# LukasHaas/PIGEON

Measured on AMD Instinct MI355X. Metric: images/sec end-to-end (ViT+head+refine), 4x336x336, higher is better.
Workload: dtype f16

## Files before the change

include/pigeon_hip.h:

```cpp
#ifndef PIGEON_HIP_H
#define PIGEON_HIP_H

#include <stddef.h>
#include <stdint.h>

#ifdef __cplusplus
extern "C" {
#endif

#define PG_OK            0
#define PG_EINVAL       -1
#define PG_ENOMEM       -2
#define PG_EHIP         -3
#define PG_ESTATE       -4

#define PG_DTYPE_F32     0
#define PG_DTYPE_BF16    1
#define PG_DTYPE_F16     2
#define PG_DTYPE_F64     3
#define PG_DTYPE_U8      4

#define PG_ABI_VERSION   7

const char* pg_last_error(void);
int pg_abi_version(void);
int pg_device_count(void);

typedef struct pg_vit pg_vit;

typedef struct pg_vit_cfg {
    int32_t layers;
    int32_t image_size;
    int32_t patch;
    int32_t hidden;
    int32_t heads;
    int32_t mlp;
    float   ln_eps;
    int32_t max_chunk;
    int32_t mma_dtype;
    int32_t precise;
} pg_vit_cfg;

int pg_vit_create(pg_vit** out, int device, const pg_vit_cfg* cfg);
int pg_vit_load_weight(pg_vit* h, const char* name, const void* data, int dtype,
                       const int64_t* shape, int ndim);
int pg_vit_finalize(pg_vit* h);
int pg_vit_workspace_bytes(const pg_vit* h, int n_images, size_t* bytes);
int pg_vit_forward(pg_vit* h, const void* pixels, int pix_dtype, int n_images, float* emb_out,
                   void* workspace, size_t workspace_bytes, void* stream);
int pg_vit_forward_hidden(pg_vit* h, const void* pixels, int pix_dtype, int n_images, float* emb_out,
                          float* hidden_out, void* workspace, size_t workspace_bytes, void* stream);
int pg_vit_precise_workspace_bytes(const pg_vit* h, int n_images, size_t* bytes);
int pg_vit_precise_plan(int n_images, int32_t out[8]);
int pg_vit_forward_precise(pg_vit* h, const void* pixels, int pix_dtype, int n_images, float* emb_out, float* hidden_out,
                           void* workspace, size_t workspace_bytes, void* stream);
int pg_vit_graph(pg_vit* h, int on, int64_t* replays, int64_t* captures);
int pg_vit_destroy(pg_vit* h);
int pg_vit_mma_dtype(const pg_vit* h);

int pg_fingerprint(const void* data, size_t bytes, uint64_t seed, uint64_t out[2], void* stream);
int pg_vit_fingerprint(const pg_vit* h, uint64_t out[2]);

#define PG_PROF_CLASSES 9
int pg_vit_profile_enable(pg_vit* h, int on);
int pg_vit_profile_read(pg_vit* h, int64_t* launches , double* ms );
int pg_vit_profile_reset(pg_vit* h);

int pg_tune_gemm_stagger(float fraction);
int pg_tune_gemm_tail_rows(int rows);
int pg_tune_gemm_tail_shape(int min_k, int min_n);
int pg_tune_gemm_raster(int gn);
int pg_tune_gemm_mid(int on);
int pg_gemm_plan(int variant, int epi, int M, int N, int K, int* kernel, int* rows_main, int* rest);
int pg_tune_exact_attention(int use_f32_mfma);
int pg_tune_exact_products(int n);
int pg_tune_exact_fusion(int on);
int pg_vit_saturation_check(pg_vit* h, int on);
int pg_vit_saturation_read(pg_vit* h, int64_t* count, int reset);
int pg_vit_range_alarm_read(pg_vit* h, int64_t* rows, int reset);

int pg_head_forward(const float* emb, int B, int P, const float* W, const float* bias,
                    const double* centroids, int C, int k, float* logits,
                    float* topk_val, int64_t* topk_idx, int64_t* argmax, double* pred_llh, void* stream);

int pg_head_margin(const float* logits, int B, int C, const float* emb, int P, const float* W, float* margin, float* sens,
                   int64_t* top2, void* stream);

int pg_head_certainty(const float* logits, int B, int C, const float* emb, int P, const float* W, const int64_t* topk_idx, int kx,
                      const float* beta, const float* wstats, float* tol, int32_t* code, float* margin, float* sens, void* stream);

int pg_aux_heads_forward(const float* emb, int B, int P, const float* W, const float* bias, int n_reg, int n_climate, int n_month,
                         const float* beta, float* preds, int64_t* cls, float* tol, int32_t* code, float* row_tol, void* stream);

typedef struct pg_bank {
    const float*   proto_emb;
    const int64_t* cell_off;
    const float*   proto_lnglat;
    const int32_t* proto_count;
    const int64_t* member_off;
    const int64_t* member_idx;
    const float*   train_emb;
    const float*   train_lnglat;
    int64_t num_cells;
    int64_t num_protos;
    int64_t num_train;
} pg_bank;

int pg_refine_forward(const pg_bank* bank, const float* q, int B, int P, const double* init_llh,
                      const int64_t* cand, const float* cand_prob, int k, int topk,
                      float temperature, double max_refine_km, float* scratch,
                      float* out_llh, int64_t* out_cell, int32_t* out_choice, void* stream);

int pg_refine_forward_ex(const pg_bank* bank, const float* q, int B, int P, const double* init_llh,
                         const int64_t* cand, const float* cand_prob, int k, int topk, int n_eval,
                         float temperature, double max_refine_km, float* scratch12,
                         float* out_llh, int64_t* out_cell, int32_t* out_choice, int32_t* out_refined, void* stream);

int pg_refine_certainty(const pg_bank* bank, const float* q, int B, int P, const int64_t* cand, const float* cand_prob, int k,
                        int topk, int n_eval, const float* scratch12, const float* W, int C, const float* beta,
                        const float* wstats, float temperature, const int32_t* refined, const int32_t* choice,
                        float* tol, int32_t* code, void* stream);

int pg_requeue_append(const float* head_tol, const float* refine_tol, const int32_t* refine_code, int B, float thr, int force_all,
                      int64_t dst_base, int64_t flushed, int64_t cap, int64_t* counters, int64_t* slot_dst, int32_t* row_slot,
                      uint8_t* certain, int32_t* cause, void* stream);
int pg_rows_to_slots(const void* src, int64_t row_bytes, const int32_t* row_slot, int B, void* dst, void* stream);
int pg_requeue_take(const int64_t* slot_dst, int64_t cap, int64_t head, int n_valid, int n_pad, int64_t* dst_out, void* stream);
int pg_scatter_rows(const void* src, int64_t row_bytes, const int64_t* dst_row, int n, void* dst, int64_t dst_rows,
                    int64_t remap_wb, int64_t remap_b, int64_t remap_off, void* stream);
// ... 37 lines not shown
int pg_allgather_many(void* comm, int count, const void* const* send, void* const* recv, const size_t* bytes_per_rank,
                      void* stream);
int pg_comm_destroy(void* comm);
int pg_comm_rccl_version(void);

int pg_proto_build(const float* train_emb, int panels, int64_t num_train, const int64_t* member_off,
                   const int64_t* member_idx, int64_t num_protos, float* proto_emb, void* stream);
int pg_haversine_matrix(const void* x, int x_dtype, const double* y, int N, int M, double* out, void* stream);
int pg_haversine_pairs(const double* x, const void* y, int y_dtype, int64_t N, double* out, void* stream);
int pg_smooth_labels(const double* distances, int N, int M, double constant, double* out, void* stream);

int pg_haversine_blocks(const double* pts, const int64_t* cell_off, const int64_t* mat_off, int C, double zero_as, double* out,
                        void* stream);
int pg_optics_graph(const double* dist, const int64_t* cell_off, const int64_t* mat_off, int C, int min_samples, int64_t* ordering,
                    double* core, double* reach, int64_t* pred, void* stream);
int pg_optics_plan(int64_t n, int min_samples, int32_t out[4]);
int pg_tune_optics_lds_points(int max_points);

typedef struct pg_region_bank {
    const int64_t* region_off;
    const int64_t* ring_off;
    const double*  xy;
    const double*  ring_bbox;
    const double*  region_bbox;
    const int64_t* region_off_host;
    const int64_t* ring_off_host;
    int64_t num_regions;
    int64_t num_rings;
    int64_t num_vertices;
} pg_region_bank;
#define PG_REGION_OUTSIDE   0
#define PG_REGION_INSIDE    1
#define PG_REGION_AMBIGUOUS 2
int pg_region_locate(const pg_region_bank* bank, const double* pts, const int32_t* start, int64_t N, int32_t* cover, uint8_t* state,
                     void* stream);
int pg_region_classify(const pg_region_bank* bank, const double* pts, const int32_t* region, int64_t N, uint8_t* state, void* stream);
int pg_region_nearest(const pg_region_bank* bank, const double* pts, int64_t N, int32_t* idx, double* dist, void* stream);
int pg_region_plan(const pg_region_bank* bank, int32_t out[4]);
int pg_tune_region_wave_edges(int max_edges);

int pg_op_gemm16(int dtype, const void* A, int64_t lda, const void* W, const float* bias, void* out, int64_t ldc,
                 int M, int N, int K, int epi, float qscale, int qcols, const float* aux,
                 int variant, void* stream);
int pg_op_gemm16_ld(int dtype, const void* A, int64_t lda, const void* W, int64_t ldw, const float* bias, void* out,
                    int64_t ldc, int M, int N, int K, int epi, float qscale, int qcols, const float* aux,
                    int variant, void* stream);
int pg_op_rowstat_cast(const float* x, void* x16, int dtype, float* rowstat, int64_t rows, float eps, void* stream);
int pg_op_gemm16_resid_stat(int dtype, const void* A, int64_t lda, const void* W, int64_t ldw, const float* bias, float* X,
                            int64_t ldc, void* x16, int64_t ldx, float* statpart, int M, int N, int K, int variant, void* stream);
int pg_op_rowstat_finalize(const float* statpart, int slots, float* rowstat, int64_t rows, float eps, void* stream);
int pg_op_gemm16_ln(int dtype, const void* A, int64_t lda, const void* W, int64_t ldw, const float* bias, const float* colsum,
                    const float* rowstat, void* out, int64_t ldc, int M, int N, int K, int epi, float qscale, int qcols,
                    int variant, void* stream);
int pg_op_layernorm(const float* x, const float* gamma, const float* beta, void* y, int out_dtype,
                    int64_t rows, float eps, void* stream);
int pg_op_attention(int dtype, const void* qkv, void* out, int n_images, void* stream);
int pg_op_im2col(const void* pixels, int pix_dtype, void* out, int out_dtype, int n_images, void* stream);
int pg_op_token_mean(const float* x, float* out, int n_images, void* stream);
int pg_op_cast_f32(const float* x, void* y, int out_dtype, int64_t n, void* stream);
int pg_op_preln(float* x, const float* cls, const float* pos0, const float* gamma, const float* beta, int64_t rows, float eps,
                void* x16, int x16_dtype, float* rowstat, void* stream);
int pg_op_gemm16_parts(int dtype, const void* A, int64_t lda, const void* W, int64_t ldw, const float* bias, float* parts,
                       int M, int N, int Kp, int S, void* stream);
int pg_op_x3_split(const float* x, void* y3, int64_t rows, int cols, int gelu, void* stream);
int pg_op_x3_layernorm(const float* x, const float* gamma, const float* beta, void* y3, int64_t rows, float eps, void* stream);
int pg_op_attention_f32(const float* qkv, float* out, int n_images, void* stream);
int pg_op_attention_x3(const float* qkv, void* out3, int n_images, void* stream);
int pg_op_x3_im2col(const void* pixels, int pix_dtype, void* out3, int n_images, void* stream);
int pg_op_sum_parts(const float* parts, int S, int64_t part_elems, float* dst, int64_t n, int resid, void* stream);

#ifdef __cplusplus
}
#endif
#endif
```

pigeon_amd/_lib.py:

```python
from __future__ import annotations

import ctypes as C
import os

_HERE = os.path.dirname(os.path.abspath(__file__))
LIB_PATH = os.environ.get("PIGEON_HIP_LIB") or os.path.join(_HERE, "libpigeon_hip.so")

PG_DTYPE_F32, PG_DTYPE_BF16, PG_DTYPE_F16, PG_DTYPE_F64, PG_DTYPE_U8 = 0, 1, 2, 3, 4
EPI_QKV, EPI_GELU, EPI_RESID, EPI_PATCH, EPI_F32, EPI_RESID_STAT, EPI_QKV_LN, EPI_GELU_LN, EPI_GELU_X3 = 0, 1, 2, 3, 4, 5, 6, 7, 8
PROF_CLASSES = ["gemm_qkv", "gemm_out", "gemm_fc1", "gemm_fc2", "gemm_patch", "attention", "layernorm",
                "im2col", "token_mean"]


class PigeonHipError(RuntimeError):
    pass


class VitCfg(C.Structure):
    _fields_ = [("layers", C.c_int32), ("image_size", C.c_int32), ("patch", C.c_int32), ("hidden", C.c_int32),
                ("heads", C.c_int32), ("mlp", C.c_int32), ("ln_eps", C.c_float), ("max_chunk", C.c_int32),
                ("mma_dtype", C.c_int32), ("precise", C.c_int32)]


class Bank(C.Structure):
    _fields_ = [("proto_emb", C.c_void_p), ("cell_off", C.c_void_p), ("proto_lnglat", C.c_void_p),
                ("proto_count", C.c_void_p), ("member_off", C.c_void_p), ("member_idx", C.c_void_p),
                ("train_emb", C.c_void_p), ("train_lnglat", C.c_void_p),
                ("num_cells", C.c_int64), ("num_protos", C.c_int64), ("num_train", C.c_int64)]


class RegionBankStruct(C.Structure):
    _fields_ = [("region_off", C.c_void_p), ("ring_off", C.c_void_p), ("xy", C.c_void_p), ("ring_bbox", C.c_void_p),
                ("region_bbox", C.c_void_p), ("region_off_host", C.c_void_p), ("ring_off_host", C.c_void_p),
                ("num_regions", C.c_int64), ("num_rings", C.c_int64), ("num_vertices", C.c_int64)]


class PrepItem(C.Structure):
    _fields_ = [("src_off", C.c_uint64), ("in_h", C.c_int32), ("in_w", C.c_int32), ("new_h", C.c_int32), ("new_w", C.c_int32),
                ("top", C.c_int32), ("left", C.c_int32), ("ksize_h", C.c_int32), ("ksize_v", C.c_int32), ("row0", C.c_int32),
                ("nrows", C.c_int32), ("tmp_row", C.c_int32), ("bounds_h_off", C.c_uint32), ("kk_h_off", C.c_uint32),
                ("bounds_v_off", C.c_uint32), ("kk_v_off", C.c_uint32), ("reserved", C.c_int32 * 3)]


PREP_ITEM_BYTES = 80
assert C.sizeof(PrepItem) == PREP_ITEM_BYTES


_P, _I, _I64, _F, _D, _SZ = C.c_void_p, C.c_int, C.c_int64, C.c_float, C.c_double, C.c_size_t
SIGNATURES = {
    "pg_last_error": (C.c_char_p, []),
    "pg_abi_version": (_I, []),
    "pg_device_count": (_I, []),
    "pg_vit_create": (_I, [C.POINTER(_P), _I, C.POINTER(VitCfg)]),
    "pg_vit_load_weight": (_I, [_P, C.c_char_p, _P, _I, C.POINTER(_I64), _I]),
    "pg_vit_finalize": (_I, [_P]),
    "pg_vit_workspace_bytes": (_I, [_P, _I, C.POINTER(_SZ)]),
    "pg_vit_forward": (_I, [_P, _P, _I, _I, _P, _P, _SZ, _P]),
    "pg_vit_forward_hidden": (_I, [_P, _P, _I, _I, _P, _P, _P, _SZ, _P]),
    "pg_vit_precise_workspace_bytes": (_I, [_P, _I, C.POINTER(_SZ)]),
    "pg_vit_forward_precise": (_I, [_P, _P, _I, _I, _P, _P, _P, _SZ, _P]),
    "pg_vit_graph": (_I, [_P, _I, C.POINTER(_I64), C.POINTER(_I64)]),
    "pg_vit_destroy": (_I, [_P]),
    "pg_vit_mma_dtype": (_I, [_P]),
    "pg_fingerprint": (_I, [_P, _SZ, C.c_uint64, C.POINTER(C.c_uint64), _P]),
    "pg_vit_fingerprint": (_I, [_P, C.POINTER(C.c_uint64)]),
    "pg_vit_profile_enable": (_I, [_P, _I]),
    "pg_vit_profile_read": (_I, [_P, C.POINTER(_I64), C.POINTER(_D)]),
    "pg_vit_profile_reset": (_I, [_P]),
    "pg_tune_gemm_stagger": (_I, [_F]),
    "pg_tune_gemm_tail_rows": (_I, [_I]),
    "pg_tune_gemm_tail_shape": (_I, [_I, _I]),
    "pg_tune_gemm_raster": (_I, [_I]),
    "pg_tune_gemm_mid": (_I, [_I]),
    "pg_tune_exact_attention": (_I, [_I]),
    "pg_tune_exact_products": (_I, [_I]),
    "pg_tune_exact_fusion": (_I, [_I]),
    "pg_gemm_plan": (_I, [_I, _I, _I, _I, _I, _P, _P, _P]),
    "pg_vit_saturation_check": (_I, [_P, _I]),
    "pg_vit_saturation_read": (_I, [_P, C.POINTER(_I64), _I]),
    "pg_vit_range_alarm_read": (_I, [_P, C.POINTER(_I64), _I]),
    "pg_comm_unique_id": (_I, [_P]),
    "pg_comm_init_rank": (_I, [C.POINTER(_P), _I, _P, _I]),
    "pg_comm_count": (_I, [_P, C.POINTER(_I)]),
    "pg_allgather": (_I, [_P, _P, _P, _SZ, _P]),
    "pg_allgather_many": (_I, [_P, _I, C.POINTER(_P), C.POINTER(_P), C.POINTER(_SZ), _P]),
    "pg_comm_destroy": (_I, [_P]),
    "pg_comm_rccl_version": (_I, []),
    "pg_prep_create": (_I, [C.POINTER(_P), _I, _I, _I]),
    "pg_prep_destroy": (_I, [_P]),
    "pg_prep_geometry": (_I, [_P, C.POINTER(C.c_int32)]),
    "pg_prep_workspace_bytes": (_I, [_P, _I, C.POINTER(_SZ)]),
    "pg_prep_norm_lut": (_I, [C.POINTER(_F)]),
    "pg_prep_forward": (_I, [_P, _P, _I, _P, _I, _P, _SZ, _P]),
    "pg_prep_ragged_plan": (_I, [_I, C.POINTER(C.c_int32), C.POINTER(PrepItem), C.POINTER(_SZ), C.POINTER(_SZ)]),
    "pg_prep_ragged_create": (_I, [C.POINTER(_P), _I]),
    "pg_prep_ragged_destroy": (_I, [_P]),
    "pg_prep_ragged_forward": (_I, [_P, _P, _SZ, C.POINTER(PrepItem), _I, _P, _I, _P, _SZ, _P]),
    "pg_proto_build": (_I, [_P, _I, _I64, _P, _P, _I64, _P, _P]),
    "pg_haversine_matrix": (_I, [_P, _I, _P, _I, _I, _P, _P]),
    "pg_haversine_pairs": (_I, [_P, _P, _I, _I64, _P, _P]),
    "pg_smooth_labels": (_I, [_P, _I, _I, _D, _P, _P]),
    "pg_haversine_blocks": (_I, [_P, _P, _P, _I, _D, _P, _P]),
    "pg_optics_graph": (_I, [_P, _P, _P, _I, _I, _P, _P, _P, _P, _P]),
    "pg_optics_plan": (_I, [_I64, _I, C.POINTER(C.c_int32)]),
    "pg_tune_optics_lds_points": (_I, [_I]),
    "pg_region_locate": (_I, [C.POINTER(RegionBankStruct), _P, _P, _I64, _P, _P, _P]),
    "pg_region_classify": (_I, [C.POINTER(RegionBankStruct), _P, _P, _I64, _P, _P]),
    "pg_region_nearest": (_I, [C.POINTER(RegionBankStruct), _P, _I64, _P, _P, _P]),
    "pg_region_plan": (_I, [C.POINTER(RegionBankStruct), C.POINTER(C.c_int32)]),
    "pg_tune_region_wave_edges": (_I, [_I]),
    "pg_head_forward": (_I, [_P, _I, _I, _P, _P, _P, _I, _I, _P, _P, _P, _P, _P, _P]),
    "pg_head_margin": (_I, [_P, _I, _I, _P, _I, _P, _P, _P, _P, _P]),
    "pg_head_certainty": (_I, [_P, _I, _I, _P, _I, _P, _P, _I, _P, _P, _P, _P, _P, _P, _P]),
    "pg_aux_heads_forward": (_I, [_P, _I, _I, _P, _P, _I, _I, _I, _P, _P, _P, _P, _P, _P, _P]),
    "pg_refine_forward": (_I, [C.POINTER(Bank), _P, _I, _I, _P, _P, _P, _I, _I, _F, _D, _P, _P, _P, _P, _P]),
    "pg_refine_forward_ex": (_I, [C.POINTER(Bank), _P, _I, _I, _P, _P, _P, _I, _I, _I, _F, _D, _P, _P, _P, _P, _P, _P]),
    "pg_refine_certainty": (_I, [C.POINTER(Bank), _P, _I, _I, _P, _P, _I, _I, _I, _P, _P, _I, _P, _P, _F, _P, _P, _P, _P, _P]),
    "pg_requeue_append": (_I, [_P, _P, _P, _I, _F, _I, _I64, _I64, _I64, _P, _P, _P, _P, _P, _P]),
    "pg_rows_to_slots": (_I, [_P, _I64, _P, _I, _P, _P]),
    "pg_requeue_take": (_I, [_P, _I64, _I64, _I, _I, _P, _P]),
    "pg_scatter_rows": (_I, [_P, _I64, _P, _I, _P, _I64, _I64, _I64, _I64, _P]),
    "pg_head_wstats": (_I, [_P, _I, _P, _P, _P]),
    "pg_embedding_debias": (_I, [_P, _I64, _I, _P, _P]),
    "pg_op_gemm16": (_I, [_I, _P, _I64, _P, _P, _P, _I64, _I, _I, _I, _I, _F, _I, _P, _I, _P]),
    "pg_op_gemm16_ld": (_I, [_I, _P, _I64, _P, _I64, _P, _P, _I64, _I, _I, _I, _I, _F, _I, _P, _I, _P]),
    "pg_op_rowstat_cast": (_I, [_P, _P, _I, _P, _I64, _F, _P]),
    "pg_op_gemm16_resid_stat": (_I, [_I, _P, _I64, _P, _I64, _P, _P, _I64, _P, _I64, _P, _I, _I, _I, _I, _P]),
    "pg_op_rowstat_finalize": (_I, [_P, _I, _P, _I64, _F, _P]),
    "pg_op_gemm16_ln": (_I, [_I, _P, _I64, _P, _I64, _P, _P, _P, _P, _I64, _I, _I, _I, _I, _F, _I, _I, _P]),
    "pg_op_layernorm": (_I, [_P, _P, _P, _P, _I, _I64, _F, _P]),
    "pg_op_attention": (_I, [_I, _P, _P, _I, _P]),
    "pg_op_im2col": (_I, [_P, _I, _P, _I, _I, _P]),
    "pg_op_token_mean": (_I, [_P, _P, _I, _P]),
    "pg_op_cast_f32": (_I, [_P, _P, _I, _I64, _P]),
    "pg_op_gemm16_parts": (_I, [_I, _P, _I64, _P, _I64, _P, _P, _I, _I, _I, _I, _P]),
    "pg_op_x3_split": (_I, [_P, _P, _I64, _I, _I, _P]),
    "pg_op_x3_layernorm": (_I, [_P, _P, _P, _P, _I64, _F, _P]),
    "pg_op_attention_f32": (_I, [_P, _P, _I, _P]),
    "pg_op_attention_x3": (_I, [_P, _P, _I, _P]),
    "pg_op_x3_im2col": (_I, [_P, _I, _P, _I, _P]),
    "pg_op_sum_parts": (_I, [_P, _I, _I64, _P, _I64, _I, _P]),
    "pg_op_preln": (_I, [_P, _P, _P, _P, _P, _I64, _F, _P, _I, _P, _P]),
    "pg_vit_precise_plan": (_I, [_I, C.POINTER(C.c_int32)]),
}

_lib = None


def load():
    global _lib
    if _lib is not None:
        return _lib
    if not os.path.exists(LIB_PATH):
        raise PigeonHipError(
            f"{LIB_PATH} not found: build it with `python -m pigeon_amd.build` (hipcc, gfx950). "
            "pigeon_amd has no CPU/PyTorch fallback for its hot path.")
    import torch
    lib = C.CDLL(LIB_PATH)
    for name, (res, args) in SIGNATURES.items():
        fn = getattr(lib, name)
        fn.restype = res
        fn.argtypes = args
    _lib = lib
    return lib


def check(rc: int, what: str = ""):
    if rc != 0:
        msg = load().pg_last_error()
        raise PigeonHipError(f"{what} failed (code {rc}): {msg.decode() if msg else ''}")


def require_gpu():
    lib = load()
    n = lib.pg_device_count()
    if n <= 0:
        raise PigeonHipError("pigeon_amd needs an AMD GPU (gfx950) visible to HIP; found none. "
                             "There is no CPU fallback for the hot path.")
    return n
```

pigeon_amd/csrc/abi.hip:

```cpp
#include "pigeon_internal.h"
#include <cstdarg>
#include <cstdio>

static thread_local char g_err[512] = "";

void pg_set_error(const char* fmt, ...) {
    va_list ap;
    va_start(ap, fmt);
    vsnprintf(g_err, sizeof(g_err), fmt, ap);
    va_end(ap);
}
int pg_check_launch(const char* what) {
    hipError_t e = hipGetLastError();
    if (e != hipSuccess) { pg_set_error("launch of %s failed: %s", what, hipGetErrorString(e)); return PG_EHIP; }
    return PG_OK;
}

extern "C" const char* pg_last_error(void) { return g_err; }
extern "C" int pg_abi_version(void) { return PG_ABI_VERSION; }
extern "C" int pg_device_count(void) {
    int n = 0;
    hipError_t e = hipGetDeviceCount(&n);
    if (e != hipSuccess) { pg_set_error("hipGetDeviceCount: %s", hipGetErrorString(e)); return PG_EHIP; }
    return n;
}

extern "C" int pg_op_gemm16(int dtype, const void* A, int64_t lda, const void* W, const float* bias, void* out, int64_t ldc,
                            int M, int N, int K, int epi, float qscale, int qcols, const float* aux, int variant,
                            void* stream) {
    if (!A || !W || !out) { pg_set_error("op_gemm16: null argument"); return PG_EINVAL; }
    return pg_gemm_launch(dtype, A, lda, W, K, bias, out, ldc, M, N, K, epi, qscale, qcols, aux, variant, (hipStream_t)stream);
}
extern "C" int pg_op_gemm16_ld(int dtype, const void* A, int64_t lda, const void* W, int64_t ldw, const float* bias, void* out,
                               int64_t ldc, int M, int N, int K, int epi, float qscale, int qcols, const float* aux,
                               int variant, void* stream) {
    if (!A || !W || !out) { pg_set_error("op_gemm16_ld: null argument"); return PG_EINVAL; }
    return pg_gemm_launch(dtype, A, lda, W, ldw, bias, out, ldc, M, N, K, epi, qscale, qcols, aux, variant, (hipStream_t)stream);
}
extern "C" int pg_op_rowstat_cast(const float* x, void* x16, int dtype, float* rowstat, int64_t rows, float eps, void* stream) {
    if (!x || !x16 || !rowstat) { pg_set_error("op_rowstat_cast: null argument"); return PG_EINVAL; }
    return pg_rowstat_cast_launch(x, x16, dtype, rowstat, rows, eps, (hipStream_t)stream);
}
extern "C" int pg_op_rowstat_finalize(const float* statpart, int slots, float* rowstat, int64_t rows, float eps, void* stream) {
    if (!statpart || !rowstat || slots <= 0) { pg_set_error("op_rowstat_finalize: bad argument"); return PG_EINVAL; }
    return pg_rowstat_finalize_launch(statpart, slots, rowstat, rows, eps, (hipStream_t)stream);
}
extern "C" int pg_op_gemm16_resid_stat(int dtype, const void* A, int64_t lda, const void* W, int64_t ldw, const float* bias, float* X,
                                       int64_t ldc, void* x16, int64_t ldx, float* statpart, int M, int N, int K, int variant,
                                       void* stream) {
    if (!A || !W || !X || !x16 || !statpart) { pg_set_error("op_gemm16_resid_stat: null argument"); return PG_EINVAL; }
    PgGemmExtra ex; ex.x16 = x16; ex.ldx = ldx; ex.statpart = statpart;
    return pg_gemm_launch(dtype, A, lda, W, ldw, bias, X, ldc, M, N, K, EPI_RESID_STAT, 1.f, 0, nullptr, variant ? variant : PG_GEMM_V_PP,
                          (hipStream_t)stream, &ex);
}
extern "C" int pg_op_gemm16_ln(int dtype, const void* A, int64_t lda, const void* W, int64_t ldw, const float* bias,
                               const float* colsum, const float* rowstat, void* out, int64_t ldc, int M, int N, int K, int epi,
                               float qscale, int qcols, int variant, void* stream) {
    if (!A || !W || !out || !colsum || !rowstat) { pg_set_error("op_gemm16_ln: null argument"); return PG_EINVAL; }
    if (epi != EPI_QKV_LN && epi != EPI_GELU_LN) { pg_set_error("op_gemm16_ln: epi must be 6 or 7"); return PG_EINVAL; }
    PgGemmExtra ex; ex.colsum = colsum; ex.rowstat = rowstat;
    return pg_gemm_launch(dtype, A, lda, W, ldw, bias, out, ldc, M, N, K, epi, qscale, qcols, nullptr, variant ? variant : PG_GEMM_V_PP,
                          (hipStream_t)stream, &ex);
}
extern "C" int pg_op_layernorm(const float* x, const float* gamma, const float* beta, void* y, int out_dtype,
                               int64_t rows, float eps, void* stream) {
    if (!x || !gamma || !beta || !y) { pg_set_error("op_layernorm: null argument"); return PG_EINVAL; }
    return pg_layernorm_launch(x, gamma, beta, y, out_dtype, rows, eps, (hipStream_t)stream);
}
extern "C" int pg_op_attention(int dtype, const void* qkv, void* out, int n_images, void* stream) {
    if (!qkv || !out) { pg_set_error("op_attention: null argument"); return PG_EINVAL; }
    return pg_attention_launch(dtype, qkv, out, n_images, (hipStream_t)stream);
}
extern "C" int pg_op_im2col(const void* pixels, int pix_dtype, void* out, int out_dtype, int n_images, void* stream) {
    if (!pixels || !out) { pg_set_error("op_im2col: null argument"); return PG_EINVAL; }
    if (out_dtype == PG_DTYPE_U8) { pg_set_error("op_im2col: PG_DTYPE_U8 is a pixel dtype, not an output dtype"); return PG_EINVAL; }
    const float* lut = nullptr;
    if (pix_dtype == PG_DTYPE_U8 && n_images > 0) { const int rc = pg_norm_lut_device(&lut); if (rc) return rc; }
    return pg_im2col_launch(pixels, pix_dtype, out, out_dtype, n_images, (hipStream_t)stream, lut);
}
extern "C" int pg_op_token_mean(const float* x, float* out, int n_images, void* stream) {
    if (!x || !out) { pg_set_error("op_token_mean: null argument"); return PG_EINVAL; }
    return pg_token_mean_launch(x, out, n_images, (hipStream_t)stream);
}
extern "C" int pg_op_cast_f32(const float* x, void* y, int out_dtype, int64_t n, void* stream) {
    if (!x || !y) { pg_set_error("op_cast_f32: null argument"); return PG_EINVAL; }
    return pg_cast_f32_launch(x, y, out_dtype, n, (hipStream_t)stream);
}

extern "C" int pg_op_gemm16_parts(int dtype, const void* A, int64_t lda, const void* W, int64_t ldw, const float* bias, float* parts,
                                  int M, int N, int Kp, int S, void* stream) {
    if (!A || !W || !parts) { pg_set_error("op_gemm16_parts: null argument"); return PG_EINVAL; }
    if (S < 1 || S > 8) { pg_set_error("op_gemm16_parts: 1 <= S <= 8"); return PG_EINVAL; }
    PgGemmExtra ex;
    ex.parts = S; ex.a_part = Kp; ex.w_part = Kp; ex.c_part = (int64_t)M * N;
    return pg_gemm_launch(dtype, A, lda, W, ldw, bias, parts, N, M, N, Kp, EPI_F32, 1.f, 0, nullptr, PG_GEMM_V_PP, (hipStream_t)stream, &ex);
}

extern "C" int pg_op_x3_split(const float* x, void* y3, int64_t rows, int cols, int gelu, void* stream) {
    if (!x || !y3) { pg_set_error("op_x3_split: null argument"); return PG_EINVAL; }
    return pg_x3_split_launch(x, y3, rows, cols, gelu, (hipStream_t)stream);
}
extern "C" int pg_op_x3_layernorm(const float* x, const float* gamma, const float* beta, void* y3, int64_t rows, float eps, void* stream) {
    if (!x || !gamma || !beta || !y3) { pg_set_error("op_x3_layernorm: null argument"); return PG_EINVAL; }
    return pg_x3_ln_launch(x, gamma, beta, y3, rows, eps, (hipStream_t)stream);
}
extern "C" int pg_op_attention_f32(const float* qkv, float* out, int n_images, void* stream) {
    if (!qkv || !out) { pg_set_error("op_attention_f32: null argument"); return PG_EINVAL; }
    return pg_attention_f32_launch(qkv, out, n_images, (hipStream_t)stream);
}
extern "C" int pg_op_x3_im2col(const void* pixels, int pix_dtype, void* out3, int n_images, void* stream) {
    if (!pixels || !out3 || n_images < 0) { pg_set_error("op_x3_im2col: bad argument"); return PG_EINVAL; }
    const float* lut = nullptr;
    if (pix_dtype == PG_DTYPE_U8 && n_images > 0) { const int rc = pg_norm_lut_device(&lut); if (rc) return rc; }
// ... 18 lines not shown
```

pigeon_amd/csrc/gemm_epi.h:

```cpp
#pragma once
#include "gemm_device.h"

__device__ __forceinline__ float quick_gelu(float v) {
    const float e = __builtin_amdgcn_exp2f(-2.4554669595930157f * v);
    return v * __builtin_amdgcn_rcpf(1.0f + e);
}

typedef float f32x2 __attribute__((ext_vector_type(2)));
__device__ __forceinline__ f32x2 pk_fma(f32x2 a, f32x2 b, f32x2 c) { return __builtin_elementwise_fma(a, b, c); }
__device__ __forceinline__ f32x2 quick_gelu2(f32x2 v) {
    const f32x2 t = v * -2.4554669595930157f;
    f32x2 e = {__builtin_amdgcn_exp2f(t[0]), __builtin_amdgcn_exp2f(t[1])};
    e = 1.0f + e;
    const f32x2 r = {__builtin_amdgcn_rcpf(e[0]), __builtin_amdgcn_rcpf(e[1])};
    return v * r;
}
__device__ __forceinline__ f32x4 ln_fold4(f32x4 acc, float rstd, float mrs, const f32x4& colsum, const f32x4& c) {
    const f32x2 r2 = {rstd, rstd}, m2 = {-mrs, -mrs};
    const f32x2 a0 = pk_fma(f32x2{acc[0], acc[1]}, r2, pk_fma(m2, f32x2{colsum[0], colsum[1]}, f32x2{c[0], c[1]}));
    const f32x2 a1 = pk_fma(f32x2{acc[2], acc[3]}, r2, pk_fma(m2, f32x2{colsum[2], colsum[3]}, f32x2{c[2], c[3]}));
    return f32x4{a0[0], a0[1], a1[0], a1[1]};
}
__device__ __forceinline__ f32x4 quick_gelu4(f32x4 v) {
    const f32x2 a0 = quick_gelu2(f32x2{v[0], v[1]}), a1 = quick_gelu2(f32x2{v[2], v[3]});
    return f32x4{a0[0], a0[1], a1[0], a1[1]};
}


template <typename T, int EPI>
__device__ __forceinline__ u32x4 epi16_finish(f32x4 lo, f32x4 hi, const f32x4& b_lo, const f32x4& b_hi, const f32x4& s_lo,
                                              const f32x4& s_hi, float rstd, float mrs, bool q_strip, float qsc) {
    if constexpr (epi_is_ln(EPI)) {
        lo = ln_fold4(lo, rstd, mrs, s_lo, b_lo);
        hi = ln_fold4(hi, rstd, mrs, s_hi, b_hi);
    } else {
        lo += b_lo; hi += b_hi;
    }
    if constexpr (epi_is_qkv(EPI)) {
        if (q_strip) { lo *= qsc; hi *= qsc; }
    } else {
        lo = quick_gelu4(lo); hi = quick_gelu4(hi);
    }
    u32x4 pk;
    pk[0] = pack16x2<T>(lo[0], lo[1]); pk[1] = pack16x2<T>(lo[2], lo[3]);
    pk[2] = pack16x2<T>(hi[0], hi[1]); pk[3] = pack16x2<T>(hi[2], hi[3]);
    return pk;
}

__device__ __forceinline__ f32x4 epi_resid4(f32x4 x, const f32x4& acc, const f32x4& b) {
    x += acc + b;
    return x;
}
template <typename T>
__device__ __forceinline__ u32x2 epi_copy16x4(const f32x4& x) {
    u32x2 h;
    h[0] = pack16x2<T>(x[0], x[1]); h[1] = pack16x2<T>(x[2], x[3]);
    return h;
}
__device__ __forceinline__ void epi_stat8(const f32x4& x, const f32x4& y, float& s1, float& s2) {
    s1 = ((x[0] + x[1]) + (x[2] + x[3])) + ((y[0] + y[1]) + (y[2] + y[3]));
    s2 = ((x[0] * x[0] + x[1] * x[1]) + (x[2] * x[2] + x[3] * x[3])) + ((y[0] * y[0] + y[1] * y[1]) + (y[2] * y[2] + y[3] * y[3]));
}
template <int CTRL>
__device__ __forceinline__ float epi_dpp_mov(float v) {
    return __builtin_bit_cast(float, __builtin_amdgcn_update_dpp(0, __builtin_bit_cast(int, v), CTRL, 0xF, 0xF, true));
}
__device__ __forceinline__ float row8_sum(float v) {
    v += epi_dpp_mov<0xB1>(v);
    v += epi_dpp_mov<0x4E>(v);
    v += epi_dpp_mov<0x141>(v);
    return v;
}

template <int EPI>
__device__ __forceinline__ void epi_store_f32x4(const GemmArgs& g, int row, int col, f32x4 v, const f32x4& b4) {
    if (EPI == EPI_RESID) {
        float* p = (float*)g.out + (int64_t)row * g.ldc + col;
        f32x4 x = *(const f32x4*)p;
        x += v + b4;
        *(f32x4*)p = x;
    } else if (EPI == EPI_PATCH) {
        const int img = row / VIT_PATCHES, p = row - img * VIT_PATCHES;
        float* o = (float*)g.out + ((int64_t)img * VIT_TOKENS + 1 + p) * g.ldc + col;
        const f32x4 pos = *(const f32x4*)(g.aux + (int64_t)(1 + p) * g.N + col);
        *(f32x4*)o = v + pos;
    } else {
        *(f32x4*)((float*)g.out + (int64_t)row * g.ldc + col) = v + b4;
    }
}

template <typename T, int EPI>
__device__ __forceinline__ void epi_store_bf16x8(const GemmArgs& g, int row, int col, f32x4 lo, f32x4 hi,
                                                 const f32x4& b_lo, const f32x4& b_hi) {
    lo += b_lo; hi += b_hi;
    if (EPI == EPI_QKV) {
        if (col < g.qcols) { lo *= g.qscale; hi *= g.qscale; }
    } else {
#pragma unroll
        for (int e = 0; e < 4; ++e) { lo[e] = quick_gelu(lo[e]); hi[e] = quick_gelu(hi[e]); }
    }
    u32x4 pk;
    pk[0] = pack16x2<T>(lo[0], lo[1]); pk[1] = pack16x2<T>(lo[2], lo[3]);
    pk[2] = pack16x2<T>(hi[0], hi[1]); pk[3] = pack16x2<T>(hi[2], hi[3]);
    *(u32x4*)((uint16_t*)g.out + (int64_t)row * g.ldc + col) = pk;
}

constexpr int EPI_SLAB_ROWPF = 64 + 4;
template <typename T, int EPI>
__device__ __forceinline__ void epi_slab32(const GemmArgs& g, float* slab, int lane, int row0, int col0, const f32x4 (&acc0)[4],
                                           const f32x4 (&acc1)[4]) {
    constexpr bool OUT16 = epi_is_out16(EPI);
    constexpr bool LN = epi_is_ln(EPI);
    constexpr bool STAT = (EPI == EPI_RESID_STAT);
    constexpr bool RESID = epi_is_resid(EPI);
    constexpr int ROWPF = EPI_SLAB_ROWPF;
    const int l15 = lane & 15, lq = lane >> 4;
#pragma unroll
    for (int ib = 0; ib < 2; ++ib)
#pragma unroll
        for (int j = 0; j < 4; ++j) *(f32x4*)(slab + (ib * 16 + l15) * ROWPF + j * 16 + 4 * lq) = (ib ? acc1 : acc0)[j];
    wave_lds_fence();

    constexpr int HOFF = STAT ? 32 : 4;
    const int rr = lane >> 3, cc = STAT ? (lane & 7) * 4 : (lane & 7) * 8;
    const int col = col0 + cc;
    const f32x4 zero4 = {0.f, 0.f, 0.f, 0.f};
    f32x4 b_lo = zero4, b_hi = zero4, s_lo = zero4, s_hi = zero4;
    if (g.bias) { b_lo = *(const f32x4*)(g.bias + col); b_hi = *(const f32x4*)(g.bias + col + HOFF); }
    if constexpr (LN) { s_lo = *(const f32x4*)(g.ex.colsum + col); s_hi = *(const f32x4*)(g.ex.colsum + col + 4); }
    const float qsc = (epi_is_qkv(EPI) && col < g.qcols) ? g.qscale : 1.f;

#pragma unroll
    for (int it = 0; it < 4; ++it) {
        const int r = it * 8 + rr;
        const int row = row0 + r;
        if (row >= g.M) continue;
        f32x4 lo = *(const f32x4*)(slab + r * ROWPF + cc);
        f32x4 hi = *(const f32x4*)(slab + r * ROWPF + cc + HOFF);
        if constexpr (OUT16) {
            float rstd = 0.f, mrs = 0.f;
            if constexpr (LN) {
                const u32x2 rs = *(const u32x2*)(g.ex.rowstat + (int64_t)row * 2);
                asm("v_mov_b32 %0, %1" : "=v"(rstd) : "v"(rs[0]));
                asm("v_mov_b32 %0, %1" : "=v"(mrs) : "v"(rs[1]));
            }
            *(u32x4*)((uint16_t*)g.out + (int64_t)row * g.ldc + col) =
                epi16_finish<T, EPI>(lo, hi, b_lo, b_hi, s_lo, s_hi, rstd, mrs, col0 < g.qcols, qsc);
        } else if constexpr (RESID) {
            float* p = (float*)g.out + (int64_t)row * g.ldc + col;
            const f32x4 x = epi_resid4(*(const f32x4*)p, lo, b_lo);
            const f32x4 y = epi_resid4(*(const f32x4*)(p + HOFF), hi, b_hi);
            *(f32x4*)p = x;
            *(f32x4*)(p + HOFF) = y;
            if constexpr (STAT) {
                uint16_t* p16 = (uint16_t*)g.ex.x16 + (int64_t)row * g.ldc + col;
                *(u32x2*)p16 = epi_copy16x4<T>(x);
                *(u32x2*)(p16 + HOFF) = epi_copy16x4<T>(y);
                float s1, s2;
                epi_stat8(x, y, s1, s2);
                s1 = row8_sum(s1);
                s2 = row8_sum(s2);
                if ((lane & 7) == 0) {
                    float* sp = g.ex.statpart + ((int64_t)(col0 / 64) * g.ex.stat_rows + row) * 2;
                    sp[0] = s1; sp[1] = s2;
                }
            }
        } else {
            float* p = (float*)g.out + (int64_t)row * g.ldc + col;
            *(f32x4*)p = lo + b_lo;
            *(f32x4*)(p + 4) = hi + b_hi;
        }
    }
}
```

pigeon_amd/csrc/gemm_mid.hip:

```cpp
#include "gemm_epi.h"

namespace {

constexpr int MD_BM = 128, MD_BN = 128;
#ifndef PG_MID_STAGES
#define PG_MID_STAGES 3
#endif
constexpr int MD_STAGES = PG_MID_STAGES;
#ifndef PG_MID_PRODUCER
#define PG_MID_PRODUCER 1
#endif
constexpr bool MD_PROD = PG_MID_PRODUCER != 0;
constexpr int MD_THREADS = MD_PROD ? 320 : 256;
constexpr int MD_STAGE = (MD_BM + MD_BN) * ROWB;
constexpr int MD_W_OFF = MD_BM * ROWB;
constexpr int MD_NDMA = (MD_BM + MD_BN) / 8 / 4;
constexpr int MD_LDS = MD_STAGES * MD_STAGE;
constexpr int MD_SLAB_BYTES = 32 * EPI_SLAB_ROWPF * 4;

__device__ __forceinline__ void md_issue(__amdgpu_buffer_rsrc_t ra, __amdgpu_buffer_rsrc_t rw, char* stage, int wave,
                                         const int (&voffA)[4], const int (&voffW)[4], int soff) {
#pragma unroll
    for (int d = 0; d < 4; ++d) dma16(ra, stage + (wave + 4 * d) * 8 * ROWB, voffA[d], soff);
#pragma unroll
// ... 17 lines not shown
    int voffA[4], voffW[4];
#pragma unroll
    for (int d = 0; d < 4; ++d) {
        const int r = (wave + 4 * d) * 8 + (lane >> 3);
        const int c = (lane & 7) ^ ((r >> 1) & 7);
        voffA[d] = r * (int)g.lda * 2 + c * 16;
        voffW[d] = r * (int)g.ldw * 2 + c * 16;
    }
    const int nt = g.K / BK;
    if constexpr (MD_PROD) {
        static_assert(!MD_PROD || MD_STAGES == 3, "the producer form is written for the three-stage ring");
        if (wave == 4) {
            int pvA[2], pvW[2];
#pragma unroll
            for (int d = 0; d < 2; ++d) {
                const int r = d * 8 + (lane >> 3);
                const int c = (lane & 7) ^ ((r >> 1) & 7);
                pvA[d] = r * (int)g.lda * 2 + c * 16;
                pvW[d] = r * (int)g.ldw * 2 + c * 16;
            }
            const int stepA = 16 * (int)g.lda * 2, stepW = 16 * (int)g.ldw * 2;
            auto issue = [&](int t, char* stage) {
#pragma unroll
                for (int gr = 0; gr < 16; ++gr) dma16(ra, stage + gr * 8 * ROWB, pvA[gr & 1] + (gr >> 1) * stepA, t * BK * 2);
#pragma unroll
                for (int gr = 0; gr < 16; ++gr) dma16(rw, stage + MD_W_OFF + gr * 8 * ROWB, pvW[gr & 1] + (gr >> 1) * stepW, t * BK * 2);
            };
            issue(0, smem);
            if (nt > 1) issue(1, smem + MD_STAGE);
            int freed = 2 * MD_STAGE;
            for (int t = 0; t < nt; ++t) {
                if (t + 1 < nt) asm volatile("s_waitcnt vmcnt(32)" ::: "memory");
                else asm volatile("s_waitcnt vmcnt(0)" ::: "memory");
                __builtin_amdgcn_sched_barrier(0);
                __builtin_amdgcn_s_barrier();
                __builtin_amdgcn_sched_barrier(0);
                if (t + 2 < nt) issue(t + 2, smem + freed);
                freed += MD_STAGE;
                if (freed >= MD_LDS) freed = 0;
            }
            __builtin_amdgcn_s_barrier();
            return;
        }
    } else {
#pragma unroll
        for (int t = 0; t < MD_STAGES - 1; ++t)
            if (t < nt) md_issue(ra, rw, smem + t * MD_STAGE, wave, voffA, voffW, t * BK * 2);
    }

    const int l15 = lane & 15, lq = lane >> 4;
    const int sw = (lane >> 1) & 7;
    const uint32_t lds0 = (uint32_t)(uintptr_t)(__attribute__((address_space(3))) char*)smem;
    const uint32_t a_base = lds0 + (wm * 64 + l15) * ROWB, b_base = lds0 + MD_W_OFF + (wn * 64 + l15) * ROWB;
    f32x4 acc[4][4];
#pragma unroll
    for (int i = 0; i < 4; ++i)
#pragma unroll
        for (int j = 0; j < 4; ++j) acc[i][j] = f32x4{0.f, 0.f, 0.f, 0.f};

    int cur = 0;
    for (int kt = 0; kt < nt; ++kt) {
        static_assert(MD_STAGES >= 3 && MD_STAGES <= 5, "the vmcnt ladder below covers 3 .. 5 stages");
        if constexpr (!MD_PROD) {
            const int ahead = min(MD_STAGES - 2, nt - 1 - kt);
            if (MD_STAGES >= 5 && ahead == 3) asm volatile("s_waitcnt vmcnt(%0)" ::"n"(3 * MD_NDMA) : "memory");
            else if (MD_STAGES >= 4 && ahead == 2) asm volatile("s_waitcnt vmcnt(%0)" ::"n"(2 * MD_NDMA) : "memory");
            else if (ahead == 1) asm volatile("s_waitcnt vmcnt(%0)" ::"n"(MD_NDMA) : "memory");
            else asm volatile("s_waitcnt vmcnt(0)" ::: "memory");
        }
        __builtin_amdgcn_sched_barrier(0);
        __builtin_amdgcn_s_barrier();
        __builtin_amdgcn_sched_barrier(0);
        if (!MD_PROD && kt + MD_STAGES - 1 < nt) {
            int nxt = cur - MD_STAGE;
            if (nxt < 0) nxt += MD_LDS;
            md_issue(ra, rw, smem + nxt, wave, voffA, voffW, (kt + MD_STAGES - 1) * BK * 2);
        }
#pragma unroll
        for (int ks = 0; ks < 2; ++ks) {
            const uint32_t xo = (uint32_t)(((ks * 4 + lq) ^ sw) << 4) + (uint32_t)cur;
            const uint32_t aa = a_base + xo, ab = b_base + xo;
            typename T::v8 a[4], b[4];
            lds_read_b128<0 * 16 * ROWB>(a[0], aa); lds_read_b128<1 * 16 * ROWB>(a[1], aa);
            lds_read_b128<2 * 16 * ROWB>(a[2], aa); lds_read_b128<3 * 16 * ROWB>(a[3], aa);
            lds_read_b128<0 * 16 * ROWB>(b[0], ab); lds_read_b128<1 * 16 * ROWB>(b[1], ab);
            lds_read_b128<2 * 16 * ROWB>(b[2], ab); lds_read_b128<3 * 16 * ROWB>(b[3], ab);
            wait_lgkm0();
#pragma unroll
            for (int i = 0; i < 4; ++i)
#pragma unroll
                for (int j = 0; j < 4; ++j) acc[i][j] = T::mfma16(b[j], a[i], acc[i][j]);
        }
        cur += MD_STAGE;
        if (cur >= MD_LDS) cur = 0;
    }
    if constexpr (MD_PROD) {
        asm volatile("s_waitcnt lgkmcnt(0)" ::: "memory");
        __builtin_amdgcn_s_barrier();
    } else {
        __syncthreads();
    }
    float* slab = (float*)(smem + wave * MD_SLAB_BYTES);
    const int row0 = m0 + wm * 64, col0 = n0 + wn * 64;
    epi_slab32<T, EPI>(g, slab, lane, row0, col0, acc[0], acc[1]);
    wave_lds_fence();
    epi_slab32<T, EPI>(g, slab, lane, row0 + 32, col0, acc[2], acc[3]);
    wave_lds_fence();
}

template <typename T, int EPI>
int launch_mid(const GemmArgs& g, int nblk, hipStream_t s) {
    static bool attr_set = false;
    return launch_kernel(gemm_mid_kernel<T, EPI>, attr_set, MD_LDS, dim3(nblk), dim3(MD_THREADS), g, s, "gemm_mid", "gemm_mid: set LDS attr");
}

template <typename T>
int dispatch_mid(const GemmArgs& g, int epi, int nblk, hipStream_t s) {
    switch (epi) {
        case EPI_QKV: return launch_mid<T, EPI_QKV>(g, nblk, s);
        case EPI_GELU: return launch_mid<T, EPI_GELU>(g, nblk, s);
        case EPI_RESID: return launch_mid<T, EPI_RESID>(g, nblk, s);
        case EPI_F32: return launch_mid<T, EPI_F32>(g, nblk, s);
        case EPI_RESID_STAT: return launch_mid<T, EPI_RESID_STAT>(g, nblk, s);
        case EPI_QKV_LN: return launch_mid<T, EPI_QKV_LN>(g, nblk, s);
        case EPI_GELU_LN: return launch_mid<T, EPI_GELU_LN>(g, nblk, s);
        default: pg_set_error("gemm_mid: epilogue %d not supported", epi); return PG_EINVAL;
    }
}

}

bool pg_gemm_mid_supported(int epi, int N, int K) {
    return epi != EPI_PATCH && epi >= EPI_QKV && epi <= EPI_GELU_LN && N % MD_BN == 0 && K % BK == 0 && K >= BK;
}

int pg_gemm_mid_launch(int dtype, GemmArgs g, int epi, hipStream_t s, int m_begin) {
    if (!pg_gemm_mid_supported(epi, g.N, g.K)) { pg_set_error("gemm_mid: unsupported epilogue / shape (epi=%d N=%d K=%d)", epi, g.N, g.K); return PG_EINVAL; }
    if (g.ex.parts > 1) { pg_set_error("gemm_mid: several products in one launch exist in gemm_pp.hip only"); return PG_EINVAL; }
    if (m_begin < 0 || m_begin >= g.M) return m_begin == g.M ? PG_OK : (pg_set_error("gemm_mid: m_begin = %d outside [0, %d)", m_begin, g.M), PG_EINVAL);
    if (m_begin > 0) {
        if (g.ex.stat_rows <= 0) g.ex.stat_rows = g.M;
        g.A += (int64_t)m_begin * g.lda;
        g.out = (char*)g.out + (int64_t)m_begin * g.ldc * (epi_is_out16(epi) ? 2 : 4);
        if (g.ex.rowstat) g.ex.rowstat += (int64_t)m_begin * 2;
        if (g.ex.x16) g.ex.x16 = (uint16_t*)g.ex.x16 + (int64_t)m_begin * g.ldc;
        if (g.ex.statpart) g.ex.statpart += (int64_t)m_begin * 2;
        g.M -= m_begin;
    }
    if (int rc = pg_gemm_panel_check("gemm_mid", g.lda, g.ldw, MD_BM, MD_BN)) return rc;
    g.tilesM = (g.M + MD_BM - 1) / MD_BM;
    g.tilesN = g.N / MD_BN;
    g.ntiles = g.tilesM * g.tilesN;
    g.gn = g.M >= g.N ? 1 : 0;
    if (dtype == PG_DTYPE_F16) return dispatch_mid<T_F16>(g, epi, g.ntiles, s);
    if (dtype == PG_DTYPE_BF16) return dispatch_mid<T_BF16>(g, epi, g.ntiles, s);
    pg_set_error("gemm_mid: operand dtype must be PG_DTYPE_F16 or PG_DTYPE_BF16 (got %d)", dtype);
    return PG_EINVAL;
}
```

pigeon_amd/csrc/gemm_plan.hip:

```cpp
#include "common.h"
#include "pigeon_internal.h"

#include "gemm_epi.h"

#include <cmath>
#include <cstdlib>
#include <type_traits>

#ifndef PG_DEFAULT_GEMM_STAGGER
#define PG_DEFAULT_GEMM_STAGGER 0.0f
#endif
#define PG_DEFAULT_GEMM_TAIL_ROWS 768
#define PG_DEFAULT_GEMM_TAIL_MIN_K 2048
#define PG_DEFAULT_GEMM_TAIL_MIN_N 4096
#ifndef PG_DEFAULT_GEMM_RESID6
#define PG_DEFAULT_GEMM_RESID6 1
#endif
#define PG_ROUTE_MAX_ROWS 40000
#ifndef PG_EXACT_MID_US_KT
#define PG_EXACT_MID_US_KT 0.6
#endif

static unsigned long long g_tune_epoch = 1;
unsigned long long pg_tune_epoch() { return g_tune_epoch; }
// ... 21 lines not shown
    return v;
}
static int route_max_rows() {
    static int v = -1;
    if (v < 0) { v = env_knob("PIGEON_GEMM_ROUTE_MAX_ROWS", PG_ROUTE_MAX_ROWS); if (v < 0) v = 0; }
    return v;
}
static bool resid6_enabled(int K) {
    static int mask = -1;
    if (mask < 0) { mask = env_knob("PIGEON_GEMM_RESID6", PG_DEFAULT_GEMM_RESID6); if (mask < 0) mask = 0; }
    return (mask & (K >= 2048 ? 1 : 2)) != 0;
}
static double precise_mid_us_kt() {
    static double v = -1.0;
    if (v < 0.0) { v = env_knob("PIGEON_EXACT_MID_US", PG_EXACT_MID_US_KT); if (!(v > 0.0)) v = PG_EXACT_MID_US_KT; }
    return v;
}

static int g_raster_gn = -2;
int pg_gemm_raster_gn() {
    if (g_raster_gn == -2) { g_raster_gn = env_knob("PIGEON_GEMM_RASTER_GN", 0); if (g_raster_gn < -1) g_raster_gn = 0; }
    return g_raster_gn;
}
extern "C" int pg_tune_gemm_raster(int gn) {
    if (gn < -1 || gn > 64) { pg_set_error("tune_gemm_raster: gn must be -1 (all N tiles), 0 (default) or 1..64"); return PG_EINVAL; }
    g_raster_gn = gn; ++g_tune_epoch;
    return PG_OK;
}

static int g_tail_rows = -1, g_tail_min_k = -1, g_tail_min_n = -1;
static int env_count(const char* name, int dflt) { const int v = env_knob(name, dflt); return v < 0 ? 0 : v; }
static int tail_rows() { if (g_tail_rows < 0) g_tail_rows = env_count("PIGEON_GEMM_TAIL_ROWS", PG_DEFAULT_GEMM_TAIL_ROWS); return g_tail_rows; }
static int tail_min_k() { if (g_tail_min_k < 0) g_tail_min_k = env_count("PIGEON_GEMM_TAIL_MIN_K", PG_DEFAULT_GEMM_TAIL_MIN_K); return g_tail_min_k; }
static int tail_min_n() { if (g_tail_min_n < 0) g_tail_min_n = env_count("PIGEON_GEMM_TAIL_MIN_N", PG_DEFAULT_GEMM_TAIL_MIN_N); return g_tail_min_n; }
extern "C" int pg_tune_gemm_tail_rows(int rows) {
    if (rows < 0 || rows > (1 << 20)) { pg_set_error("tune_gemm_tail_rows: rows must be in [0, 2^20]"); return PG_EINVAL; }
    g_tail_rows = rows; ++g_tune_epoch;
    return PG_OK;
}
extern "C" int pg_tune_gemm_tail_shape(int min_k, int min_n) {
    if (min_k < 0 || min_n < 0) { pg_set_error("tune_gemm_tail_shape: negative threshold"); return PG_EINVAL; }
    g_tail_min_k = min_k; g_tail_min_n = min_n; ++g_tune_epoch;
    return PG_OK;
}

static int g_gemm_mid = -1;
static bool mid_on() {
    if (g_gemm_mid < 0) { const char* e = env_knob<const char*>("PIGEON_GEMM_MID", "1"); g_gemm_mid = e[0] == '0' ? 0 : (e[0] == '2' ? 2 : 1); }
    return g_gemm_mid != 0;
}
static bool route_pp256() { return mid_on() && g_gemm_mid != 2; }
extern "C" int pg_tune_gemm_mid(int on) {
    g_gemm_mid = on == 2 ? 2 : (on ? 1 : 0); ++g_tune_epoch;
    return PG_OK;
}

static float g_stagger = -1.f;
static float stagger_fraction() {
    if (g_stagger < 0.f) {
        g_stagger = env_knob("PIGEON_GEMM_STAGGER", PG_DEFAULT_GEMM_STAGGER);
        if (!(g_stagger >= 0.f && g_stagger <= 4.f)) g_stagger = 0.f;
    }
    return g_stagger;
}
extern "C" int pg_tune_gemm_stagger(float fraction) {
    if (!(fraction >= 0.f && fraction <= 4.f)) { pg_set_error("tune_gemm_stagger: fraction must be in [0, 4]"); return PG_EINVAL; }
    g_stagger = fraction; ++g_tune_epoch;
    return PG_OK;
}

static int num_cus() {
    static int n = 0;
    if (n == 0) {
        int dev = 0;
        hipDeviceProp_t p;
        if (hipGetDevice(&dev) == hipSuccess && hipGetDeviceProperties(&p, dev) == hipSuccess) n = p.multiProcessorCount;
        if (n <= 0) n = 256;
    }
    return n;
}
int pg_gemm_grid_cus() {
    const int ncu = num_cus(), cap = block_cap();
    return cap > 0 && cap < ncu ? cap : ncu;
}


struct PersistentFit { double ci, cf, e1_resid, e1_gelu, e1_other, e2; };
constexpr PersistentFit SMALL_PP6 = {1.6, 3.0, 7.0, 9.0, 6.0, 3.0};
constexpr PersistentFit SMALL_PP = {1.1, 1.8, 12.0, 9.0, 7.0, 6.0};
constexpr double SMALL_MID_US_KT = 0.44;
constexpr double SMALL_MID_EPI_RESID = 8.0, SMALL_MID_EPI = 5.5;
constexpr double SMALL_PP_MARGIN = 0.90;

static double gemm_model_us(int kernel, int M, int N, int K, int epi, int ncu) {
    const bool resid = epi == EPI_RESID || epi == EPI_RESID_STAT;
    const bool gelu = epi == EPI_GELU || epi == EPI_GELU_LN;
    const double kt = K / 64;
    if (kernel == PG_GK_MID) {
        const int64_t tiles = (int64_t)((M + 127) / 128) * (N / 128);
        return (double)((tiles + ncu - 1) / ncu) * (kt * SMALL_MID_US_KT + (resid ? SMALL_MID_EPI_RESID : SMALL_MID_EPI));
    }
    const PersistentFit& c = kernel == PG_GK_PP6 ? SMALL_PP6 : SMALL_PP;
    const int bm = kernel == PG_GK_PP6 ? 384 : 256;
    const double e1 = resid ? c.e1_resid : (gelu ? c.e1_gelu : c.e1_other);
    const int64_t tiles = (int64_t)((M + bm - 1) / bm) * (N / 256);
    const int64_t full = tiles / ncu;
// ... 93 lines not shown
    if (!by_mid && !by_tail) return false;
    p.rows = (int)m_main;
    p.rest = by_mid ? PG_GK_MID : PG_GK_TAIL;
    return true;
}

static int stagger_ticks(bool six, int epi, int M, int K) {
    const float f = stagger_fraction();
    if (!(f > 0.f && M >= 256 * 64)) return 0;
    const float period_us = six ? ((epi == EPI_GELU || epi == EPI_GELU_LN ? STAGGER_PP6_EPI_GELU : STAGGER_PP6_EPI) + STAGGER_PP6_US_KT * (K / 64))
                                : ((epi == EPI_RESID || epi == EPI_RESID_STAT ? STAGGER_PP_EPI_RESID : STAGGER_PP_EPI) + STAGGER_PP_US_KT * (K / 64));
    return (int)(f * period_us * TICKS_PER_US);
}

static int gemm_plan(int variant, int epi, int M, int N, int K, GemmPlan& p) {
    if (epi < EPI_QKV || epi > EPI_GELU_X3) { pg_set_error("gemm: bad epilogue %d", epi); return PG_EINVAL; }
    if (variant == 0) variant = pg_default_gemm_variant();
    const bool six = use_pp6(variant, epi, N, K);
    const bool pp = !six && (variant == PG_GEMM_V_PP6 || is_pp_variant(variant)) && N % 256 == 0 && K % 128 == 0;
    const int own = six ? PG_GK_PP6 : PG_GK_PP;
    const int pp_variant = variant == PG_GEMM_V_PP6 ? PG_GEMM_V_PP : variant;
    p = GemmPlan{own, pp_variant, M, PG_GK_NONE, stagger_ticks(six, epi, M, K)};
    if (variant == PG_GEMM_V_MID || variant == PG_GEMM_V_TAIL) {
        const bool mid = variant == PG_GEMM_V_MID;
        if (!(mid ? pg_gemm_mid_supported(epi, N, K) : pg_gemm_tail_supported(epi, N, K))) {
            pg_set_error("gemm: variant %d (%s) does not support epi=%d N=%d K=%d", variant, mid ? "gemm_mid" : "gemm_tail", epi, N, K);
            return PG_EINVAL;
        }
        p.kernel = mid ? PG_GK_MID : PG_GK_TAIL;
        return PG_OK;
    }
    if (six || pp) {
        const int kind = small_batch_route(own, epi, M, N, K);
        if (kind != own) {
            p.kernel = kind;
            p.variant = PG_GEMM_V_PP;
            return PG_OK;
        }
        tail_split(own, epi, M, N, K, p);
        return PG_OK;
    }
    if (epi >= EPI_RESID_STAT) { pg_set_error("gemm: epilogue %d exists only in the persistent kernels (variants 33, 36, 56, N %% 256 == 0, K %% 128 == 0)", epi); return PG_EINVAL; }
    p.kernel = PG_GK_ONE_TILE;
    p.variant = (variant == PG_GEMM_V_PP6 || is_pp_variant(variant)) ? PG_GEMM_V_ONE_TILE : variant;
    const int bn = pg_gemm_one_tile_bn(p.variant);
    if (bn == 0) {
        pg_set_error("gemm: variant %d does not exist (variants: 8, 33, 36, 56, 70, 71)", p.variant);
        return PG_EINVAL;
    }
    if (N % bn != 0 || K % BK != 0) { pg_set_error("gemm: N %% %d or K %% 64 != 0 (N=%d K=%d)", bn, N, K); return PG_EINVAL; }
    return PG_OK;
}

extern "C" int pg_gemm_plan(int variant, int epi, int M, int N, int K, int* kernel, int* rows_main, int* rest) {
    if (!kernel || !rows_main || !rest || M <= 0 || N <= 0 || K <= 0) { pg_set_error("gemm_plan: bad argument"); return PG_EINVAL; }
    GemmPlan p;
    const int rc = gemm_plan(variant, epi, M, N, K, p);
    if (rc != PG_OK) return rc;
    *kernel = p.kernel; *rows_main = p.rows; *rest = p.rest;
    return PG_OK;
}

#ifdef PIGEON_PROBES
static void* g_dbg_ts = nullptr;
extern "C" int pg_dbg_timestamps(void* buf) { g_dbg_ts = buf; return PG_OK; }
#endif

static int launch_one(int kernel, int variant, int dtype, const GemmArgs& g, int epi, int m_begin, hipStream_t s) {
    switch (kernel) {
        case PG_GK_PP6: return pg_gemm_pp6_launch(dtype, g, epi, s);
        case PG_GK_PP: return pg_gemm_pp_launch(dtype, g, epi, variant, s);
        case PG_GK_MID: return pg_gemm_mid_launch(dtype, g, epi, s, m_begin);
        case PG_GK_TAIL: return pg_gemm_tail_launch(dtype, g, epi, m_begin, s);
        default: return pg_gemm_one_tile_launch(dtype, g, epi, variant, s);
    }
}

int pg_gemm_launch(int dtype, const void* A, int64_t lda, const void* W, int64_t ldw, const float* bias, void* out, int64_t ldc,
                   int M, int N, int K, int epi, float qscale, int qcols, const float* aux, int variant,
                   hipStream_t s, const PgGemmExtra* extra) {
    if (M <= 0) return PG_OK;
    GemmArgs g;
    g.A = (const uint16_t*)A; g.lda = lda; g.W = (const uint16_t*)W; g.ldw = ldw > 0 ? ldw : K; g.bias = bias; g.out = out; g.ldc = ldc;
    g.M = M; g.N = N; g.K = K; g.qscale = qscale; g.qcols = qcols; g.aux = aux;
    g.tilesM = 0; g.tilesN = 0; g.ntiles = 0; g.part_tiles = 0; g.gn = 0; g.stagger = 0; g.xcd_stagger_ticks = 0;
    if (extra) g.ex = *extra;
    if (g.ex.parts > 1) {
        if (epi != EPI_F32 || N % 256 != 0 || K % 128 != 0) { pg_set_error("gemm: parts > 1 needs EPI_F32, N %% 256 == 0, K %% 128 == 0"); return PG_EINVAL; }
        return pg_gemm_pp_launch(dtype, g, epi, PG_GEMM_V_PP, s);
    }
    if ((epi == EPI_GELU || epi == EPI_RESID || epi >= EPI_RESID_STAT) && !bias) { pg_set_error("gemm: epilogue %d needs a bias", epi); return PG_EINVAL; }
    if (epi == EPI_RESID_STAT && (!g.ex.x16 || !g.ex.statpart || g.ex.ldx != ldc)) { pg_set_error("gemm: EPI_RESID_STAT needs x16 / statpart and ldx == ldc"); return PG_EINVAL; }
    if (epi_is_ln(epi) && (!g.ex.colsum || !g.ex.rowstat)) { pg_set_error("gemm: LN epilogue needs colsum / rowstat"); return PG_EINVAL; }
    if (epi == EPI_PATCH && !aux) { pg_set_error("gemm: patch epilogue needs aux"); return PG_EINVAL; }
    if (epi == EPI_GELU_X3 && (ldc != 3 * (int64_t)N || dtype != PG_DTYPE_F16 || N % 256 != 0 || K % 128 != 0)) {
        pg_set_error("gemm: EPI_GELU_X3 writes the fp16 triple [M][3N]: ldc == 3 N, fp16 operands, N %% 256 == 0, K %% 128 == 0 (ldc=%lld N=%d K=%d)",
                     (long long)ldc, N, K);
        return PG_EINVAL;
    }
    if ((lda % 8) || (ldc % 8) || (qcols % 8) || (g.ldw % 8) || g.ldw < K) { pg_set_error("gemm: lda/ldw/ldc/qcols must be multiples of 8, ldw >= K"); return PG_EINVAL; }
    GemmPlan p;
    const int rc = gemm_plan(variant, epi, M, N, K, p);
    if (rc != PG_OK) return rc;
    g.xcd_stagger_ticks = p.stagger_ticks;
    if (g.ex.stat_rows <= 0) g.ex.stat_rows = M;
#ifdef PIGEON_PROBES
    if (g_dbg_ts && epi != EPI_PATCH) { g.aux = (const float*)g_dbg_ts; g.stagger = -7; }
#endif
    GemmArgs gm = g;
    gm.M = p.rows;
    const int rc_main = launch_one(p.kernel, p.variant, dtype, gm, epi, 0, s);
    if (rc_main != PG_OK || p.rest == PG_GK_NONE) return rc_main;
    return launch_one(p.rest, 0, dtype, g, epi, p.rows, s);
}
```

pigeon_amd/csrc/gemm_pp.hip:

```cpp
#include "gemm_epi.h"
#include "x3.h"
#include <type_traits>

namespace {

constexpr int PP_BM = 256, PP_BN = 256;
constexpr int PP_STAGE = (PP_BM + PP_BN) * ROWB;
constexpr int PP_W_OFF = PP_BM * ROWB;
constexpr int PP_SLAB_OFF = PP_STAGE;
constexpr int PP_SLAB_ROWF = 64 + 4;
constexpr int PP_SLAB_BYTES = 32 * PP_SLAB_ROWF * 4;
constexpr int PP_LDS = 160 * 1024;

struct TileCtx {
    __amdgpu_buffer_rsrc_t ra, rw;
    int m0, n0;
    int part;
};

template <bool PARTS = false>
__device__ __forceinline__ TileCtx make_tile(const GemmArgs& g, int L) {
    TileCtx c;
    c.part = 0;
    const uint16_t* Ab = g.A;
    const uint16_t* Wb = g.W;
    if constexpr (PARTS) {
        c.part = L / g.part_tiles;
        L -= c.part * g.part_tiles;
        Ab += (int64_t)c.part * g.ex.a_part;
        Wb += (int64_t)c.part * g.ex.w_part;
    }
    const int gmax = g.gn >= 32 ? 1 : 32 / g.gn;
    const int band_sz = gmax * g.tilesN;
    const int band = L / band_sz, rem = L - band * band_sz;
    const int gm = min(gmax, g.tilesM - band * gmax);
    const int sup = rem / (gm * g.gn), rem2 = rem - sup * gm * g.gn;
    const int im = rem2 / g.gn, in = rem2 - im * g.gn;
    const int tm = band * gmax + im, tn = sup * g.gn + in;
    c.m0 = tm * PP_BM; c.n0 = tn * PP_BN;
    const int rows = min(PP_BM, g.M - c.m0);
    c.ra = make_rsrc(Ab + (int64_t)c.m0 * g.lda, (uint32_t)rows * (uint32_t)g.lda * 2u);
    c.rw = make_rsrc(Wb + (int64_t)c.n0 * g.ldw, (uint32_t)PP_BN * (uint32_t)g.ldw * 2u);
    return c;
}

template <int FROM, int CNT>
__device__ __forceinline__ void issue_dma(const TileCtx& c, char* stage, int wave, const int (&voffA)[4], const int (&voffW)[4],
                                          int soff) {
#pragma unroll
    for (int d = 0; d < 8; ++d) {
        if (d < FROM || d >= FROM + CNT) continue;
        if (d < 4) dma16(c.ra, stage + (wave + 8 * d) * 8 * ROWB, voffA[d], soff);
        else dma16(c.rw, stage + PP_W_OFF + (wave + 8 * (d - 4)) * 8 * ROWB, voffW[d - 4], soff);
    }
}

typedef f32x4 AccPP[8][4];
template <typename T> struct Frag { typename T::v8 a[4], b[4]; };

template <typename T, bool WITH_B>
__device__ __forceinline__ void load_frag(Frag<T>& f, const char* sa, const char* sb, int xo) {
#pragma unroll
    for (int i = 0; i < 4; ++i) f.a[i] = *(const typename T::v8*)(sa + i * 16 * ROWB + xo);
    if constexpr (WITH_B) {
#pragma unroll
// ... 214 lines not shown
                const int r = it * RPI + rr;
                f32x4 lo = *(const f32x4*)(slab + r * ROWPF + cc);
                f32x4 hi = lo;
                if constexpr (WIDE) hi = *(const f32x4*)(slab + r * ROWPF + cc + HOFF);
                const int ooff = voff + (i * sstep + it * rstep);
                if constexpr (OUT16) {
                    float rstd = 0.f, mrs = 0.f;
                    if constexpr (LN) {
                        asm("v_mov_b32 %0, %1" : "=v"(rstd) : "v"(rs[i][it][0]));
                        asm("v_mov_b32 %0, %1" : "=v"(mrs) : "v"(rs[i][it][1]));
                    }
                    const u32x4 pk = epi16_finish<T, EPI>(lo, hi, bias.lo, bias.hi, bias.slo, bias.shi, rstd, mrs, col0 < g.qcols, qsc);
                    __builtin_amdgcn_raw_buffer_store_b128(pk, ro, ooff, 0, 0);
                } else if constexpr (RESID) {
                    const f32x4 x = epi_resid4(__builtin_bit_cast(f32x4, XEARLY == 1 ? xq[i][it] : xr[i & 1][it][0]), lo, bias.lo);
                    __builtin_amdgcn_raw_buffer_store_b128(__builtin_bit_cast(u32x4, x), ro, ooff, 0, 0);
                    if constexpr (STAT) {
                        const f32x4 y = epi_resid4(__builtin_bit_cast(f32x4, xr[i & 1][it][1]), hi, bias.hi);
                        __builtin_amdgcn_raw_buffer_store_b128(__builtin_bit_cast(u32x4, y), ro, ooff + HOFF * 4, 0, 0);
                        __builtin_amdgcn_raw_buffer_store_b64(epi_copy16x4<T>(x), rx16, ooff >> 1, 0, 0);
                        __builtin_amdgcn_raw_buffer_store_b64(epi_copy16x4<T>(y), rx16, (ooff >> 1) + HOFF * 2, 0, 0);
                        float s1, s2;
                        epi_stat8(x, y, s1, s2);
                        s1 = row8_sum(s1);
                        s2 = row8_sum(s2);
                        if ((lane & 7) == 0) { slab[r * ROWPF + 64] = s1; slab[r * ROWPF + 65] = s2; }
                    }
                } else if constexpr (X3) {
                    f32x4 v = lo + bias.lo;
#pragma unroll
                    for (int e = 0; e < 4; ++e) v[e] = x3_quick_gelu(v[e]);
                    u32x2 ph, pl, ps;
                    x3_pack4(v, ph, pl, ps);
                    const int nb = g.N * 2;
                    __builtin_amdgcn_raw_buffer_store_b64(ph, ro, ooff, 0, 0);
                    __builtin_amdgcn_raw_buffer_store_b64(pl, ro, ooff + nb, 0, 0);
                    __builtin_amdgcn_raw_buffer_store_b64(ps, ro, ooff + 2 * nb, 0, 0);
                } else {
                    __builtin_amdgcn_raw_buffer_store_b128(__builtin_bit_cast(u32x4, lo + bias.lo), ro, ooff, 0, 0);
                }
            }
            wave_lds_fence();
            if constexpr (STAT) {
                if (lane < 32 && i * 32 + lane < rv)
                    *(u32x2*)(stat_base + (i * 32 + lane) * 2) = *(const u32x2*)(slab + lane * ROWPF + 64);
                wave_lds_fence();
            }
            PG_TS(g, dbg_iter, wave, 3 + i);
            if constexpr (LN) { if (i == 0) prefetch_next(); }
        }
    }
}

template <typename T, int EPI>
__global__ __launch_bounds__(512) void gemm_pp_kernel(GemmArgs g) {
    extern __shared__ __attribute__((aligned(16))) char smem[];
    const int tid = threadIdx.x;
    const int lane = tid & 63;
    const int wave = __builtin_amdgcn_readfirstlane(tid >> 6);
    const int wm = wave >> 2, wn = wave & 3;
    const bool follower = (wm == 1);

    int voffA[4], voffW[4];
#pragma unroll
    for (int i = 0; i < 4; ++i) {
        const int r = (wave + 8 * i) * 8 + (lane >> 3);
        const int c = (lane & 7) ^ ((r >> 1) & 7);
        voffA[i] = r * (int)g.lda * 2 + c * 16;
        voffW[i] = r * (int)g.ldw * 2 + c * 16;
    }
    const int l15 = lane & 15, lq = lane >> 4;
    const int sw = (lane >> 1) & 7;
    int xoff[2];
#pragma unroll
    for (int ks = 0; ks < 2; ++ks) xoff[ks] = ((ks * 4 + lq) ^ sw) << 4;
    const int a_base = (wm * 128 + l15) * ROWB;
    const int b_base = PP_W_OFF + (wn * 64 + l15) * ROWB;

    constexpr int ECPL = epi_wide<EPI>() ? 8 : 4;
    const int ecc = EPI == EPI_RESID_STAT ? (lane & 7) * 4 : (lane % (64 / ECPL)) * ECPL;
    const int nt = g.K / BK;
    const int nblk = gridDim.x;
    constexpr bool PARTS = (EPI == EPI_F32);
    int L = xcd_remap(blockIdx.x, nblk);
    if (L >= g.ntiles) return;
    xcd_stagger_wait(g.xcd_stagger_ticks);
    if (g.stagger > 0) {
        const int slot = (blockIdx.x >> 3) & 31;
        const long long until = (long long)__builtin_readcyclecounter() + (long long)g.stagger * slot / 32;
        while ((long long)__builtin_readcyclecounter() < until) __builtin_amdgcn_s_sleep(8);
    }
    TileCtx c = make_tile<PARTS>(g, L);
    issue_dma<0, 8>(c, smem, wave, voffA, voffW, 0);
    EpiBias<EPI> bias;
    const int err = lane / (64 / ECPL);
    load_bias<EPI>(bias, g, c.n0 + wn * 64 + ecc);
    if constexpr (PARTS) { if (c.part > 0) zero_bias<EPI>(bias); }
    pin_bias<EPI>(bias);
    constexpr int NST = (EPI == EPI_PATCH) ? 0 : (EPI == EPI_F32 ? 32 : (EPI == EPI_GELU_X3 ? 63 : (epi_is_ln(EPI) ? 12 : 16)));
    bool first = true;
    int dbg_iter = 0;

    while (true) {
        AccPP acc;

        if (first || NST == 0) {
            wait_vm0();
        } else {
            asm volatile("s_waitcnt vmcnt(%0)" ::"n"(NST) : "memory");
            __builtin_amdgcn_sched_barrier(0);
        }
        wait_lgkm0();
        raw_barrier();
        PG_TS(g, dbg_iter, wave, 0);
        u32x2 rs[4][4];
        if constexpr (epi_is_ln(EPI)) load_rowstat<EPI>(rs, g, c.m0 + wm * 128, err);
        constexpr int XEARLY = EPI == EPI_RESID ? 1 : (EPI == EPI_RESID_STAT ? 2 : 0);
        XCtx xc;
        u32x4 xq[4][8];
        if (follower) raw_barrier();
        int t0 = 0;
        if (nt > 2) {
            ktile_pp<T, 0, true>(acc, smem, smem + PP_STAGE, a_base, b_base, xoff, c, wave, voffA, voffW, ROWB, true, false, xc, xq);
            ktile_pp<T, 0>(acc, smem + PP_STAGE, smem, a_base, b_base, xoff, c, wave, voffA, voffW, 2 * ROWB, true, false, xc, xq);
            t0 = 2;
        } else {
#pragma unroll
            for (int i = 0; i < 8; ++i)
#pragma unroll
                for (int j = 0; j < 4; ++j)
#pragma unroll
                    for (int r = 0; r < 4; ++r) acc[i][j][r] = 0.f;
        }
        for (int t = t0; t < nt; t += 2) {
            const bool xf = XEARLY != 0 && (t + 2 == nt);
            if (XEARLY != 0 && xf) xc = make_xctx<XEARLY == 2>(g, c.m0 + wm * 128, c.n0 + wn * 64, lane);
            ktile_pp<T, XEARLY>(acc, smem, smem + PP_STAGE, a_base, b_base, xoff, c, wave, voffA, voffW, (t + 1) * ROWB, true, xf, xc, xq);
            ktile_pp<T, 0>(acc, smem + PP_STAGE, smem, a_base, b_base, xoff, c, wave, voffA, voffW, (t + 2) * ROWB, t + 2 < nt, false,
                           xc, xq);
        }
        PG_TS(g, dbg_iter, wave, 1);
        if (!follower) raw_barrier();

        asm volatile("s_nop 7\n\ts_nop 7" ::: "memory");
        PG_TS(g, dbg_iter, wave, 2);
        const int row0 = c.m0 + wm * 128, col0 = c.n0 + wn * 64;
        const int part_now = c.part;
        L += nblk;
        const bool more = L < g.ntiles;
        EpiBias<EPI> bias_next = bias;
        auto prefetch_next = [&]() {
            c = make_tile<PARTS>(g, more ? L : L - nblk);
            issue_dma<0, 8>(c, smem, wave, voffA, voffW, 0);
            load_bias<EPI>(bias_next, g, c.n0 + wn * 64 + ecc);
            if constexpr (PARTS) { if (c.part > 0) zero_bias<EPI>(bias_next); }
        };
        if constexpr (PARTS) {
            GemmArgs ge = g;
            ge.out = (float*)g.out + (int64_t)part_now * g.ex.c_part;
            pp_epilogue<T, EPI, XEARLY>(acc, ge, smem, wave, lane, row0, col0, bias, rs, prefetch_next, xc, xq, dbg_iter);
        } else {
            pp_epilogue<T, EPI, XEARLY>(acc, g, smem, wave, lane, row0, col0, bias, rs, prefetch_next, xc, xq, dbg_iter);
        }
        PG_TS(g, dbg_iter, wave, 9);
        ++dbg_iter;
        if (!more) break;
        pin_bias<EPI>(bias_next);
        bias = bias_next;
        first = false;
    }
}

template <typename T, int EPI>
int launch_pp(const GemmArgs& g, int nblk, hipStream_t s) {
    static bool attr_set = false;
    return launch_kernel(gemm_pp_kernel<T, EPI>, attr_set, PP_LDS, dim3(nblk), dim3(512), g, s, "gemm_pp", "gemm_pp: set LDS attr");
}

template <typename T>
int launch_pp_epi(const GemmArgs& g, int epi, int nblk, hipStream_t s) {
    switch (epi) {
        case EPI_QKV: return launch_pp<T, EPI_QKV>(g, nblk, s);
        case EPI_GELU: return launch_pp<T, EPI_GELU>(g, nblk, s);
        case EPI_RESID: return launch_pp<T, EPI_RESID>(g, nblk, s);
        case EPI_PATCH: return launch_pp<T, EPI_PATCH>(g, nblk, s);
        case EPI_F32: return launch_pp<T, EPI_F32>(g, nblk, s);
        case EPI_RESID_STAT: return launch_pp<T, EPI_RESID_STAT>(g, nblk, s);
        case EPI_QKV_LN: return launch_pp<T, EPI_QKV_LN>(g, nblk, s);
        case EPI_GELU_LN: return launch_pp<T, EPI_GELU_LN>(g, nblk, s);
        case EPI_GELU_X3:
            if constexpr (std::is_same<T, T_F16>::value) return launch_pp<T, EPI_GELU_X3>(g, nblk, s);
            else { pg_set_error("gemm_pp: EPI_GELU_X3 exists for fp16 operands only (the exact mode)"); return PG_EINVAL; }
        default: pg_set_error("gemm_pp: bad epilogue %d", epi); return PG_EINVAL;
    }
}

template <typename T>
int dispatch_pp(GemmArgs& g, int epi, int variant, int nblk, hipStream_t s) {
    g.gn = g.tilesN;
    switch (variant) {
        case 33: return launch_pp_epi<T>(g, epi, nblk, s);
        case 36: if (g.tilesN % 4 == 0) g.gn = 4; return launch_pp_epi<T>(g, epi, nblk, s);
        default: pg_set_error("gemm_pp: variant %d is not a persistent schedule (33, 36)", variant); return PG_EINVAL;
    }
}

}

int pg_gemm_pp_launch(int dtype, GemmArgs g, int epi, int variant, hipStream_t s) {
    if (g.N % PP_BN != 0 || g.K % (2 * BK) != 0) {
        pg_set_error("gemm_pp: N %% 256 or K %% 128 != 0 (N=%d K=%d)", g.N, g.K);
        return PG_EINVAL;
    }
    if (int rc = pg_gemm_panel_check("gemm_pp", g.lda, g.ldw, PP_BM, PP_BN)) return rc;
    g.tilesM = (g.M + PP_BM - 1) / PP_BM;
    g.tilesN = g.N / PP_BN;
    g.part_tiles = g.tilesM * g.tilesN;
    if (g.ex.parts < 1) g.ex.parts = 1;
    if (g.ex.parts > 1 && epi != EPI_F32) { pg_set_error("gemm_pp: parts > 1 exists for EPI_F32 only (epi = %d)", epi); return PG_EINVAL; }
    if ((int64_t)g.part_tiles * g.ex.parts >= (1ll << 30)) { pg_set_error("gemm_pp: too many tiles"); return PG_EINVAL; }
    g.ntiles = g.part_tiles * g.ex.parts;
    const int cap = pg_gemm_grid_cus();
    const int nblk = g.ntiles < cap ? g.ntiles : cap;
    if (dtype == PG_DTYPE_F16) return dispatch_pp<T_F16>(g, epi, variant, nblk, s);
    if (dtype == PG_DTYPE_BF16) return dispatch_pp<T_BF16>(g, epi, variant, nblk, s);
    pg_set_error("gemm_pp: operand dtype must be PG_DTYPE_F16 or PG_DTYPE_BF16 (got %d)", dtype);
    return PG_EINVAL;
}
```

pigeon_amd/csrc/gemm_pp6.hip:

```cpp
#include "gemm_epi.h"

namespace {

constexpr int P6_TM = 6;
constexpr int P6_BM = 2 * P6_TM * 32, P6_BN = 256;
constexpr int P6_STAGE = (P6_BM + P6_BN) * ROWB;
constexpr int P6_W_OFF = P6_BM * ROWB;
constexpr int P6_SLAB_OFF = P6_STAGE;
constexpr int P6_SLAB_ROWF = 64 + 4;
constexpr int P6_SLAB_BYTES = 32 * P6_SLAB_ROWF * 4;
constexpr int P6_LDS = 2 * P6_STAGE;
constexpr int P6_NDMA = P6_TM + 4;
static_assert(8 * P6_SLAB_BYTES <= P6_STAGE, "slabs must fit into stage 1");

struct Tile6 {
    __amdgpu_buffer_rsrc_t ra, rw;
    int m0, n0;
    int sa, sw;
};

__device__ __forceinline__ Tile6 make_tile6(const GemmArgs& g, int L) {
    Tile6 c;
    const int gmax = g.gn >= 32 ? 1 : 32 / g.gn;
    const int band_sz = gmax * g.tilesN;
    const int band = L / band_sz, rem = L - band * band_sz;
    const int gm = min(gmax, g.tilesM - band * gmax);
    const int sup = rem / (gm * g.gn), rem2 = rem - sup * gm * g.gn;
    const int im = rem2 / g.gn, in = rem2 - im * g.gn;
    const int tm = band * gmax + im, tn = sup * g.gn + in;
    c.m0 = tm * P6_BM; c.n0 = tn * P6_BN;
    const int rows = min(P6_BM, g.M - c.m0);
    c.ra = make_rsrc(g.A + (int64_t)c.m0 * g.lda, (uint32_t)rows * (uint32_t)g.lda * 2u);
    c.rw = make_rsrc(g.W + (int64_t)c.n0 * g.ldw, (uint32_t)P6_BN * (uint32_t)g.ldw * 2u);
    c.sa = 64 * (int)g.lda * 2; c.sw = 64 * (int)g.ldw * 2;
    return c;
}

template <int FROM, int CNT>
__device__ __forceinline__ void issue_dma6(const Tile6& c, char* stage, int wave, int voffA, int voffW, int soff) {
    asm volatile("" : "+s"(soff));
#pragma unroll
    for (int d = 0; d < P6_NDMA; ++d) {
        if (d < FROM || d >= FROM + CNT) continue;
        if (d < P6_TM) dma16(c.ra, stage + (wave + 8 * d) * 8 * ROWB, voffA + (soff + d * c.sa), 0);
        else dma16(c.rw, stage + P6_W_OFF + (wave + 8 * (d - P6_TM)) * 8 * ROWB, voffW + (soff + (d - P6_TM) * c.sw), 0);
    }
}

constexpr int P6_RB = 2 * P6_TM;
typedef f32x4 Acc6[P6_RB][4];
template <typename T> struct Frag6 { typename T::v8 a[P6_TM], b[4]; };

template <typename T, bool WITH_B>
__device__ __forceinline__ void load_frag6(Frag6<T>& f, uint32_t aA, uint32_t aB) {
    lds_read_b128<0 * 16 * ROWB>(f.a[0], aA); lds_read_b128<1 * 16 * ROWB>(f.a[1], aA); lds_read_b128<2 * 16 * ROWB>(f.a[2], aA);
    lds_read_b128<3 * 16 * ROWB>(f.a[3], aA); lds_read_b128<4 * 16 * ROWB>(f.a[4], aA);
    if constexpr (P6_TM > 5) lds_read_b128<5 * 16 * ROWB>(f.a[P6_TM > 5 ? 5 : 0], aA);
    if constexpr (WITH_B) {
        lds_read_b128<0 * 16 * ROWB>(f.b[0], aB); lds_read_b128<1 * 16 * ROWB>(f.b[1], aB);
        lds_read_b128<2 * 16 * ROWB>(f.b[2], aB); lds_read_b128<3 * 16 * ROWB>(f.b[3], aB);
    }
}

template <typename T, bool ZERO, int HALF>
__device__ __forceinline__ void mma24(Acc6& acc, const Frag6<T>& f) {
#pragma unroll
// ... 64 lines not shown
        wait_lgkm0();
#ifdef PIGEON_PROBES
        if (probe) t1 = __builtin_amdgcn_s_memrealtime();
#endif
        raw_barrier();
#ifdef PIGEON_PROBES
        if (probe) t2 = __builtin_amdgcn_s_memrealtime();
#endif
        __builtin_amdgcn_s_setprio(1);
        if (kk == 0) mma24<T, ZERO, 0>(acc, f);
        if (kk == 1) mma24<T, ZERO, 1>(acc, f);
        if (kk == 2) mma24<T, false, 0>(acc, f);
        if (kk == 3) mma24<T, false, 1>(acc, f);
        __builtin_amdgcn_s_setprio(0);
#ifdef PIGEON_PROBES
        if (probe) t3 = __builtin_amdgcn_s_memrealtime();
#endif
        raw_barrier();
#ifdef PIGEON_PROBES
        if (probe && (threadIdx.x & 63) == 0) {
            const unsigned long long t4 = __builtin_amdgcn_s_memrealtime();
            unsigned long long* d = pg_dbg_phase[wave >> 2];
            d[0] += t1 - t0; d[1] += t2 - t1; d[2] += t3 - t2; d[3] += t4 - t3; d[4] += 1;
        }
#endif
    }
}

struct Bias6 { f32x4 lo, hi; };

template <int HOFF = 4>
__device__ __forceinline__ void load_bias6(Bias6& b, const GemmArgs& g, int col) {
    const f32x4 z = {0.f, 0.f, 0.f, 0.f};
    b.lo = z; b.hi = z;
    if (g.bias) {
        b.lo = *(const f32x4*)(g.bias + col);
        b.hi = *(const f32x4*)(g.bias + col + HOFF);
    }
}
__device__ __forceinline__ void pin_bias6(Bias6& b) { asm volatile("" : "+v"(b.lo), "+v"(b.hi)); }

__device__ __forceinline__ __amdgpu_buffer_rsrc_t rowstat_rsrc6(const GemmArgs& g, int row0) {
    const int rvs = wave_valid_rows(g.M - row0, P6_TM * 32);
    return make_rsrc((const char*)g.ex.rowstat + (int64_t)row0 * 8, (uint32_t)rvs * 8u);
}

constexpr int P6_P16_ROWB = 128 + 16;
static_assert(32 * P6_P16_ROWB <= P6_SLAB_BYTES, "16-bit slab must fit into the wave's slab");
struct RowStatP { u32x2 v[2]; };
__device__ __forceinline__ void load_rowstat_p(RowStatP& rs, __amdgpu_buffer_rsrc_t rrs, int l15, int slab) {
    rs.v[0] = __builtin_amdgcn_raw_buffer_load_b64(rrs, (slab * 32 + l15) * 8, 0, 0);
    rs.v[1] = __builtin_amdgcn_raw_buffer_load_b64(rrs, (slab * 32 + 16 + l15) * 8, 0, 0);
}
template <typename T, int EPI, typename PREFETCH_DMA, typename PREFETCH_BIAS>
__device__ __forceinline__ void epilogue6_park16(Acc6& acc, const GemmArgs& g, char* smem, int wave, int lane, int row0, int col0,
                                                 const Bias6& b01, const Bias6& b23, const Bias6& s01, const Bias6& s23,
                                                 const RowStatP& rs0, __amdgpu_buffer_rsrc_t rrs,
                                                 PREFETCH_DMA&& prefetch_dma, PREFETCH_BIAS&& prefetch_bias, int dbg_iter = 0) {
    constexpr bool LN = epi_is_ln(EPI);
    const int l15 = lane & 15, lq = lane >> 4;
    char* slab = smem + P6_SLAB_OFF + wave * P6_SLAB_BYTES;
    const int rr = lane >> 3, c8 = lane & 7;
    const bool q_strip = col0 < g.qcols;
    const float qsc = (epi_is_qkv(EPI) && q_strip) ? g.qscale : 1.f;
    const int rv = wave_valid_rows(g.M - row0, P6_TM * 32);
    const uint32_t nbytes = rv > 0 ? (uint32_t)(((int64_t)(rv - 1) * g.ldc + 64) * 2) : 0u;
    __amdgpu_buffer_rsrc_t ro = make_rsrc((const char*)g.out + ((int64_t)row0 * g.ldc + col0) * 2, nbytes);
    const int voff = (rr * (int)g.ldc + c8 * 8) * 2;
    int rstep = 8 * (int)g.ldc * 2;
    int sstep = 32 * (int)g.ldc * 2;
    asm volatile("" : "+s"(rstep), "+s"(sstep));
    prefetch_dma();
    RowStatP rs[2];
    rs[0] = rs0;
    char* wr = slab + l15 * P6_P16_ROWB + 8 * lq;
#pragma unroll
    for (int i = 0; i < P6_TM; ++i) {
        if constexpr (LN) { if (i + 1 < P6_TM) load_rowstat_p(rs[(i + 1) & 1], rrs, l15, i + 1); }
#pragma unroll
        for (int ib = 0; ib < 2; ++ib) {
            float rstd = 0.f, mrs = 0.f;
            if constexpr (LN) {
                asm("v_mov_b32 %0, %1" : "=v"(rstd) : "v"(rs[i & 1].v[ib][0]));
                asm("v_mov_b32 %0, %1" : "=v"(mrs) : "v"(rs[i & 1].v[ib][1]));
            }
#pragma unroll
            for (int jp = 0; jp < 2; ++jp) {
                const Bias6& bb = jp ? b23 : b01;
                const Bias6& ss = jp ? s23 : s01;
                const u32x4 pk = epi16_finish<T, EPI>(acc[2 * i + ib][2 * jp], acc[2 * i + ib][2 * jp + 1], bb.lo, bb.hi, ss.lo, ss.hi,
                                                      rstd, mrs, q_strip, qsc);
                u32x2 h0, h1;
                h0[0] = pk[0]; h0[1] = pk[1]; h1[0] = pk[2]; h1[1] = pk[3];
                *(u32x2*)(wr + ib * 16 * P6_P16_ROWB + (2 * jp) * 32) = h0;
                *(u32x2*)(wr + ib * 16 * P6_P16_ROWB + (2 * jp + 1) * 32) = h1;
            }
        }
        wave_lds_fence();
#pragma unroll
        for (int it = 0; it < 4; ++it) {
            const u32x4 v = *(const u32x4*)(slab + (it * 8 + rr) * P6_P16_ROWB + c8 * 16);
            __builtin_amdgcn_raw_buffer_store_b128(v, ro, voff + (i * sstep + it * rstep), 0, 0);
        }
        wave_lds_fence();
        PG_TS(g, dbg_iter, wave, 3 + i);
        if (i == 0) prefetch_bias();
    }
}

struct XRows6 { u32x4 v[4][2]; };
template <int IT0 = 0, int IT1 = 4>
__device__ __forceinline__ void fetch_xrows6(XRows6& x, __amdgpu_buffer_rsrc_t ro, int voff, int slab_off, int rstep) {
#pragma unroll
    for (int it = IT0; it < IT1; ++it)
#pragma unroll
        for (int h = 0; h < 2; ++h)
            x.v[it][h] =
                __builtin_amdgcn_raw_buffer_load_b128(ro, voff + 128 * h, __builtin_amdgcn_readfirstlane(slab_off + it * rstep), 0);
}
constexpr int P6_X0_EARLY = 2;
struct ResidCtx6 {
    __amdgpu_buffer_rsrc_t ro, rx16, rstat;
    int voff;
};
__device__ __forceinline__ ResidCtx6 make_resid6(const GemmArgs& g, int row0, int col0, int lane) {
    ResidCtx6 r;
    const int rv = wave_valid_rows(g.M - row0, P6_TM * 32);
    const uint32_t nel = rv > 0 ? (uint32_t)((int64_t)(rv - 1) * g.ldc + 64) : 0u;
    r.ro = make_rsrc((const char*)g.out + ((int64_t)row0 * g.ldc + col0) * 4, nel * 4u);
    r.rx16 = make_rsrc((const char*)g.ex.x16 + ((int64_t)row0 * g.ldc + col0) * 2, nel * 2u);
    r.rstat = make_rsrc((const char*)(g.ex.statpart + ((int64_t)(col0 / 64) * g.ex.stat_rows + row0) * 2), (uint32_t)rv * 8u);
    r.voff = ((lane >> 3) * (int)g.ldc + (lane & 7) * 4) * 4;
    return r;
}
template <typename T, typename PREFETCH_DMA, typename PREFETCH_BIAS>
__device__ __forceinline__ void epilogue6_resid(Acc6& acc, const GemmArgs& g, char* smem, int wave, int lane, int row0, int col0,
                                                const Bias6& bias, const XRows6& x0, const ResidCtx6& rc,
                                                PREFETCH_DMA&& prefetch_dma, PREFETCH_BIAS&& prefetch_bias, int dbg_iter = 0) {
    constexpr int ROWPF = P6_SLAB_ROWF;
    const int l15 = lane & 15, lq = lane >> 4;
    float* slab = (float*)(smem + P6_SLAB_OFF + wave * P6_SLAB_BYTES);
    const int rr = lane >> 3, cc = (lane & 7) * 4;
    int rstep = 8 * (int)g.ldc * 4;
    int sstep = 32 * (int)g.ldc * 4;
    asm volatile("" : "+s"(rstep), "+s"(sstep));
    prefetch_dma();
    XRows6 xr[2];
#pragma unroll
    for (int it = 0; it < P6_X0_EARLY; ++it) { xr[0].v[it][0] = x0.v[it][0]; xr[0].v[it][1] = x0.v[it][1]; }
    auto process = [&](int i, int it) {
        const int r = it * 8 + rr;
        const f32x4 lo = *(const f32x4*)(slab + r * ROWPF + cc);
        const f32x4 hi = *(const f32x4*)(slab + r * ROWPF + cc + 32);
        const int ooff = rc.voff + (i * sstep + it * rstep);
        const f32x4 x = epi_resid4(__builtin_bit_cast(f32x4, xr[i & 1].v[it][0]), lo, bias.lo);
        const f32x4 y = epi_resid4(__builtin_bit_cast(f32x4, xr[i & 1].v[it][1]), hi, bias.hi);
        __builtin_amdgcn_raw_buffer_store_b128(__builtin_bit_cast(u32x4, x), rc.ro, ooff, 0, 0);
        __builtin_amdgcn_raw_buffer_store_b128(__builtin_bit_cast(u32x4, y), rc.ro, ooff + 128, 0, 0);
        __builtin_amdgcn_raw_buffer_store_b64(epi_copy16x4<T>(x), rc.rx16, ooff >> 1, 0, 0);
        __builtin_amdgcn_raw_buffer_store_b64(epi_copy16x4<T>(y), rc.rx16, (ooff >> 1) + 64, 0, 0);
        float s1, s2;
        epi_stat8(x, y, s1, s2);
        s1 = row8_sum(s1);
        s2 = row8_sum(s2);
        if ((lane & 7) == 0) { slab[r * ROWPF + 64] = s1; slab[r * ROWPF + 65] = s2; }
    };
#pragma unroll
    for (int i = 0; i < P6_TM; ++i) {
#pragma unroll
        for (int ib = 0; ib < 2; ++ib)
#pragma unroll
            for (int j = 0; j < 4; ++j) *(f32x4*)(slab + (ib * 16 + l15) * ROWPF + j * 16 + 4 * lq) = acc[2 * i + ib][j];
        if (i == 0) fetch_xrows6<P6_X0_EARLY, 4>(xr[0], rc.ro, rc.voff, 0, rstep);
        if (i + 1 < P6_TM) fetch_xrows6<0, 2>(xr[(i + 1) & 1], rc.ro, rc.voff, (i + 1) * sstep, rstep);
        wave_lds_fence();
        process(i, 0);
        process(i, 1);
        if (i + 1 < P6_TM) fetch_xrows6<2, 4>(xr[(i + 1) & 1], rc.ro, rc.voff, (i + 1) * sstep, rstep);
        process(i, 2);
        process(i, 3);
        wave_lds_fence();
        if (lane < 32)
            __builtin_amdgcn_raw_buffer_store_b64(*(const u32x2*)(slab + lane * ROWPF + 64), rc.rstat, lane * 8 + i * 256, 0, 0);
        wave_lds_fence();
        PG_TS(g, dbg_iter, wave, 3 + i);
        if (i == 0) prefetch_bias();
    }
}

template <typename T, int EPI>
__global__ __launch_bounds__(512) void gemm_pp6_kernel(GemmArgs g) {
    extern __shared__ __attribute__((aligned(16))) char smem[];
    const int tid = threadIdx.x;
    const int lane = tid & 63;
    const int wave = __builtin_amdgcn_readfirstlane(tid >> 6);
    const int wm = wave >> 2, wn = wave & 3;
    const bool follower = (wm == 1);

    const int r0 = wave * 8 + (lane >> 3);
    const int ch = (lane & 7) ^ ((r0 >> 1) & 7);
    const int voffA = r0 * (int)g.lda * 2 + ch * 16;
    const int voffW = r0 * (int)g.ldw * 2 + ch * 16;
    const int l15 = lane & 15;
    const int xo0 = ((lane >> 4) ^ ((lane >> 1) & 7)) << 4;
    const uint32_t smem0 = (uint32_t)(uintptr_t)(__attribute__((address_space(3))) char*)smem;
    const uint32_t baseA = smem0 + (wm * (P6_TM * 32) + l15) * ROWB + xo0;
    const uint32_t baseB = smem0 + P6_W_OFF + (wn * 64 + l15) * ROWB + xo0;
    constexpr bool RSTAT = (EPI == EPI_RESID_STAT);
    constexpr int BHOFF = RSTAT ? 32 : 16;
    const int ecc = RSTAT ? (lane & 7) * 4 : (lane >> 4) * 4;

    const int nt = g.K / BK;
    const int nblk = gridDim.x;
    int L = xcd_remap(blockIdx.x, nblk);
    if (L >= g.ntiles) return;
    xcd_stagger_wait(g.xcd_stagger_ticks);
    Tile6 c = make_tile6(g, L);
    issue_dma6<0, P6_NDMA>(c, smem, wave, voffA, voffW, 0);
    Bias6 bias;
    load_bias6<BHOFF>(bias, g, c.n0 + wn * 64 + ecc);
    pin_bias6(bias);
    constexpr int NST = (P6_TM - 1) * 4;
    bool first = true;
    int dbg_iter = 0;

    while (true) {
        Acc6 acc;
        if (first) {
            wait_vm0();
        } else {
            asm volatile("s_waitcnt vmcnt(%0)" ::"n"(NST) : "memory");
            __builtin_amdgcn_sched_barrier(0);
        }
        wait_lgkm0();
        raw_barrier();
        PG_TS(g, dbg_iter, wave, 0);
        if (follower) raw_barrier();
        ktile6<T, true, 0>(acc, smem, baseA, baseB, c, wave, voffA, voffW, ROWB, true);
        ktile6<T, false, 1>(acc, smem, baseA, baseB, c, wave, voffA, voffW, 2 * ROWB, true);
        for (int t = 2; t < nt; t += 2) {
            ktile6<T, false, 0>(acc, smem, baseA, baseB, c, wave, voffA, voffW, (t + 1) * ROWB, true);
            ktile6<T, false, 1>(acc, smem, baseA, baseB, c, wave, voffA, voffW, (t + 2) * ROWB, t + 2 < nt);
        }
        PG_TS(g, dbg_iter, wave, 1);
        const int row0 = c.m0 + wm * (P6_TM * 32), col0 = c.n0 + wn * 64;
        Bias6 cs;
        Bias6 b23, cs23;
        RowStatP rsp;
        __amdgpu_buffer_rsrc_t rrs = c.ra;
        if constexpr (!RSTAT) load_bias6<16>(b23, g, col0 + 32 + ecc);
        if constexpr (epi_is_ln(EPI)) {
            cs.lo = *(const f32x4*)(g.ex.colsum + col0 + ecc);
            cs.hi = *(const f32x4*)(g.ex.colsum + col0 + ecc + BHOFF);
            rrs = rowstat_rsrc6(g, row0);
            cs23.lo = *(const f32x4*)(g.ex.colsum + col0 + 32 + ecc);
            cs23.hi = *(const f32x4*)(g.ex.colsum + col0 + 48 + ecc);
            load_rowstat_p(rsp, rrs, l15, 0);
        }
        ResidCtx6 rc;
        XRows6 x0;
        if constexpr (RSTAT) {
            rc = make_resid6(g, row0, col0, lane);
            fetch_xrows6<0, P6_X0_EARLY>(x0, rc.ro, rc.voff, 0, 8 * (int)g.ldc * 4);
        }
        if (!follower) raw_barrier();
        asm volatile("s_nop 7\n\ts_nop 7" ::: "memory");
        PG_TS(g, dbg_iter, wave, 2);

        L += nblk;
        const bool more = L < g.ntiles;
        Bias6 bias_next = bias;
        auto prefetch_dma = [&]() {
            c = make_tile6(g, more ? L : L - nblk);
            issue_dma6<0, P6_NDMA>(c, smem, wave, voffA, voffW, 0);
        };
        auto prefetch_bias = [&]() { load_bias6<BHOFF>(bias_next, g, c.n0 + wn * 64 + ecc); };
        if constexpr (RSTAT) epilogue6_resid<T>(acc, g, smem, wave, lane, row0, col0, bias, x0, rc, prefetch_dma, prefetch_bias, dbg_iter);
        else epilogue6_park16<T, EPI>(acc, g, smem, wave, lane, row0, col0, bias, b23, cs, cs23, rsp, rrs, prefetch_dma, prefetch_bias, dbg_iter);
        PG_TS(g, dbg_iter, wave, 9);
        ++dbg_iter;
        if (!more) break;
        pin_bias6(bias_next);
        bias = bias_next;
        first = false;
    }
}

template <typename T, int EPI>
int launch_pp6(const GemmArgs& g, int nblk, hipStream_t s) {
    static bool attr_set = false;
    return launch_kernel(gemm_pp6_kernel<T, EPI>, attr_set, P6_LDS, dim3(nblk), dim3(512), g, s, "gemm_pp6", "gemm_pp6: set LDS attr");
}

}

bool pg_gemm_pp6_supported(int epi, int N, int K) {
    return (epi_is_out16(epi) || epi == EPI_RESID_STAT) && N % P6_BN == 0 &&
           K % (2 * BK) == 0 && K >= 4 * BK;
}

int pg_gemm_pp6_launch(int dtype, GemmArgs g, int epi, hipStream_t s) {
    if (!pg_gemm_pp6_supported(epi, g.N, g.K)) { pg_set_error("gemm_pp6: unsupported epilogue / shape (epi=%d N=%d K=%d)", epi, g.N, g.K); return PG_EINVAL; }
    if (int rc = pg_gemm_panel_check("gemm_pp6", g.lda, g.ldw, P6_BM, P6_BN)) return rc;
    g.tilesM = (g.M + P6_BM - 1) / P6_BM;
    g.tilesN = g.N / P6_BN;
    g.ntiles = g.tilesM * g.tilesN;
    g.gn = (g.tilesN % 4 == 0) ? 4 : g.tilesN;
    {
        const int rg = pg_gemm_raster_gn();
        if (rg == -1 || rg >= g.tilesN) g.gn = g.tilesN;
        else if (rg > 0 && g.tilesN % rg == 0) g.gn = rg;
    }
    const int cap = pg_gemm_grid_cus();
    const int nblk = g.ntiles < cap ? g.ntiles : cap;
    if (epi_is_ln(epi) && (!g.ex.colsum || !g.ex.rowstat)) { pg_set_error("gemm_pp6: LN epilogue needs colsum / rowstat"); return PG_EINVAL; }
    if (epi == EPI_RESID_STAT && (!g.ex.x16 || !g.ex.statpart || g.ex.ldx != g.ldc || !g.bias)) { pg_set_error("gemm_pp6: EPI_RESID_STAT needs bias, x16 / statpart and ldx == ldc"); return PG_EINVAL; }
#define P6_DISPATCH(TT)                                                          \
    switch (epi) {                                                               \
        case EPI_QKV: return launch_pp6<TT, EPI_QKV>(g, nblk, s);                \
        case EPI_GELU: return launch_pp6<TT, EPI_GELU>(g, nblk, s);              \
        case EPI_QKV_LN: return launch_pp6<TT, EPI_QKV_LN>(g, nblk, s);          \
        case EPI_RESID_STAT: return launch_pp6<TT, EPI_RESID_STAT>(g, nblk, s);  \
        default: return launch_pp6<TT, EPI_GELU_LN>(g, nblk, s);                 \
    }
    if (dtype == PG_DTYPE_F16) { P6_DISPATCH(T_F16) }
    if (dtype == PG_DTYPE_BF16) { P6_DISPATCH(T_BF16) }
#undef P6_DISPATCH
    pg_set_error("gemm_pp6: operand dtype must be PG_DTYPE_F16 or PG_DTYPE_BF16 (got %d)", dtype);
    return PG_EINVAL;
}
```

pigeon_amd/csrc/gemm_tail.hip:

```cpp
#include "gemm_epi.h"

namespace {

constexpr int TL_BM = 32, TL_BN = 64;
constexpr int TL_DEPTH = 8;

template <typename T> struct FragTL { typename T::v8 a[2], b[4]; };

template <typename T>
__device__ __forceinline__ void load_frag_tl(FragTL<T>& f, __amdgpu_buffer_rsrc_t ra, __amdgpu_buffer_rsrc_t rw,
                                             const int (&va)[2], const int (&vw)[4], int kbytes) {
#pragma unroll
    for (int i = 0; i < 2; ++i) f.a[i] = __builtin_bit_cast(typename T::v8, __builtin_amdgcn_raw_buffer_load_b128(ra, va[i], kbytes, 0));
#pragma unroll
    for (int j = 0; j < 4; ++j) f.b[j] = __builtin_bit_cast(typename T::v8, __builtin_amdgcn_raw_buffer_load_b128(rw, vw[j], kbytes, 0));
}

template <typename T, int EPI>
__global__ __launch_bounds__(64) void gemm_tail_kernel(GemmArgs g, int m_begin) {
    __shared__ __attribute__((aligned(16))) float slab[TL_BM * EPI_SLAB_ROWPF];
    const int lane = threadIdx.x;
    int tn, tm;
    if (g.tilesN % 8 == 0) {
        const int xcd = blockIdx.x & 7, idx = blockIdx.x >> 3, per = g.tilesN >> 3;
        tn = xcd + 8 * (idx % per); tm = idx / per;
    } else {
        tn = blockIdx.x % g.tilesN; tm = blockIdx.x / g.tilesN;
    }
    const int row0 = m_begin + tm * TL_BM, col0 = tn * TL_BN;
    const int l15 = lane & 15, lq = lane >> 4;
    const int rows = min(TL_BM, g.M - row0);
    const __amdgpu_buffer_rsrc_t ra = make_rsrc(g.A + (int64_t)row0 * g.lda, (uint32_t)rows * (uint32_t)g.lda * 2u);
    const __amdgpu_buffer_rsrc_t rw = make_rsrc(g.W + (int64_t)col0 * g.ldw, (uint32_t)TL_BN * (uint32_t)g.ldw * 2u);
    int va[2], vw[4];
#pragma unroll
    for (int i = 0; i < 2; ++i) va[i] = (i * 16 + l15) * (int)g.lda * 2 + lq * 16;
#pragma unroll
    for (int j = 0; j < 4; ++j) vw[j] = (j * 16 + l15) * (int)g.ldw * 2 + lq * 16;

    const int nks = g.K / 32;
    FragTL<T> fr[TL_DEPTH];
#pragma unroll
    for (int d = 0; d < TL_DEPTH; ++d) {
        load_frag_tl<T>(fr[d], ra, rw, va, vw, d * 64);
        __builtin_amdgcn_sched_barrier(0);
    }
    f32x4 acc[2][4];
#pragma unroll
    for (int i = 0; i < 2; ++i)
#pragma unroll
        for (int j = 0; j < 4; ++j) acc[i][j] = f32x4{0.f, 0.f, 0.f, 0.f};
    for (int ks = 0; ks < nks; ks += TL_DEPTH) {
#pragma unroll
        for (int d = 0; d < TL_DEPTH; ++d) {
#pragma unroll
            for (int i = 0; i < 2; ++i)
#pragma unroll
                for (int j = 0; j < 4; ++j) acc[i][j] = T::mfma16(fr[d].b[j], fr[d].a[i], acc[i][j]);
            const int kn = min(ks + d + TL_DEPTH, nks - 1);
            load_frag_tl<T>(fr[d], ra, rw, va, vw, kn * 64);
            __builtin_amdgcn_sched_barrier(0);
        }
    }

    constexpr bool OUT16 = epi_is_out16(EPI);
    constexpr bool LN = epi_is_ln(EPI);
    constexpr bool STAT = (EPI == EPI_RESID_STAT);
    constexpr bool RESID = epi_is_resid(EPI);
#pragma unroll
    for (int ib = 0; ib < 2; ++ib)
#pragma unroll
        for (int j = 0; j < 4; ++j) *(f32x4*)(slab + (ib * 16 + l15) * EPI_SLAB_ROWPF + j * 16 + 4 * lq) = acc[ib][j];
    wave_lds_fence();

    constexpr int HOFF = STAT ? 32 : 4;
    const int rr = lane >> 3, cc = STAT ? (lane & 7) * 4 : (lane & 7) * 8;
    const int col = col0 + cc;
    const f32x4 zero4 = {0.f, 0.f, 0.f, 0.f};
    f32x4 b_lo = zero4, b_hi = zero4, s_lo = zero4, s_hi = zero4;
    if (g.bias) { b_lo = *(const f32x4*)(g.bias + col); b_hi = *(const f32x4*)(g.bias + col + HOFF); }
    if constexpr (LN) { s_lo = *(const f32x4*)(g.ex.colsum + col); s_hi = *(const f32x4*)(g.ex.colsum + col + 4); }
    const float qsc = (epi_is_qkv(EPI) && col < g.qcols) ? g.qscale : 1.f;

#pragma unroll
    for (int it = 0; it < 4; ++it) {
        const int r = it * 8 + rr;
        const int row = row0 + r;
        if (row >= g.M) continue;
        f32x4 lo = *(const f32x4*)(slab + r * EPI_SLAB_ROWPF + cc);
        f32x4 hi = *(const f32x4*)(slab + r * EPI_SLAB_ROWPF + cc + HOFF);
        if constexpr (OUT16) {
            float rstd = 0.f, mrs = 0.f;
            if constexpr (LN) {
                const u32x2 rs = *(const u32x2*)(g.ex.rowstat + (int64_t)row * 2);
                asm("v_mov_b32 %0, %1" : "=v"(rstd) : "v"(rs[0]));
                asm("v_mov_b32 %0, %1" : "=v"(mrs) : "v"(rs[1]));
            }
            *(u32x4*)((uint16_t*)g.out + (int64_t)row * g.ldc + col) =
                epi16_finish<T, EPI>(lo, hi, b_lo, b_hi, s_lo, s_hi, rstd, mrs, col0 < g.qcols, qsc);
        } else if constexpr (RESID) {
            float* p = (float*)g.out + (int64_t)row * g.ldc + col;
            const f32x4 x = epi_resid4(*(const f32x4*)p, lo, b_lo);
            const f32x4 y = epi_resid4(*(const f32x4*)(p + HOFF), hi, b_hi);
            *(f32x4*)p = x;
            *(f32x4*)(p + HOFF) = y;
            if constexpr (STAT) {
                uint16_t* p16 = (uint16_t*)g.ex.x16 + (int64_t)row * g.ldc + col;
                *(u32x2*)p16 = epi_copy16x4<T>(x);
                *(u32x2*)(p16 + HOFF) = epi_copy16x4<T>(y);
                float s1, s2;
                epi_stat8(x, y, s1, s2);
                s1 = row8_sum(s1);
                s2 = row8_sum(s2);
                if ((lane & 7) == 0) {
                    float* sp = g.ex.statpart + ((int64_t)(col0 / 64) * g.ex.stat_rows + row) * 2;
                    sp[0] = s1; sp[1] = s2;
                }
            }
        } else {
            float* p = (float*)g.out + (int64_t)row * g.ldc + col;
            *(f32x4*)p = lo + b_lo;
            *(f32x4*)(p + 4) = hi + b_hi;
        }
    }
}

template <typename T, int EPI>
int launch_tail(const GemmArgs& g, int m_begin, int nblk, hipStream_t s) {
    hipLaunchKernelGGL((gemm_tail_kernel<T, EPI>), dim3(nblk), dim3(64), 0, s, g, m_begin);
    return pg_check_launch("gemm_tail");
}

template <typename T>
int dispatch_tail(const GemmArgs& g, int epi, int m_begin, int nblk, hipStream_t s) {
    switch (epi) {
        case EPI_QKV: return launch_tail<T, EPI_QKV>(g, m_begin, nblk, s);
        case EPI_GELU: return launch_tail<T, EPI_GELU>(g, m_begin, nblk, s);
        case EPI_RESID: return launch_tail<T, EPI_RESID>(g, m_begin, nblk, s);
        case EPI_F32: return launch_tail<T, EPI_F32>(g, m_begin, nblk, s);
        case EPI_RESID_STAT: return launch_tail<T, EPI_RESID_STAT>(g, m_begin, nblk, s);
        case EPI_QKV_LN: return launch_tail<T, EPI_QKV_LN>(g, m_begin, nblk, s);
        case EPI_GELU_LN: return launch_tail<T, EPI_GELU_LN>(g, m_begin, nblk, s);
        default: pg_set_error("gemm_tail: epilogue %d not supported", epi); return PG_EINVAL;
    }
}

}
// ... 18 lines not shown
```

pigeon_amd/csrc/pigeon_internal.h:

```cpp
#pragma once
#include <hip/hip_runtime.h>
#include <stdint.h>
#include "../../include/pigeon_hip.h"

enum { EPI_QKV = 0, EPI_GELU = 1, EPI_RESID = 2, EPI_PATCH = 3, EPI_F32 = 4, EPI_RESID_STAT = 5, EPI_QKV_LN = 6, EPI_GELU_LN = 7,
       EPI_GELU_X3 = 8 };

struct PgGemmExtra {
    const float* colsum = nullptr;
    const float* rowstat = nullptr;
    void* x16 = nullptr;
    int64_t ldx = 0;
    float* statpart = nullptr;
    int64_t stat_rows = 0;
    int parts = 1;
    int64_t a_part = 0, w_part = 0, c_part = 0;
};

void pg_set_error(const char* fmt, ...) __attribute__((format(printf, 1, 2)));
int pg_check_launch(const char* what);
int pg_default_gemm_variant();
int pg_gemm_grid_cus();
int pg_gemm_raster_gn();
unsigned long long pg_tune_epoch();
int pg_gemm_precise_route(int M, int N, int Ktot, bool resid, const int* cand, int ncand);

enum { PG_GEMM_V_ONE_TILE = 8, PG_GEMM_V_PP = 36, PG_GEMM_V_PP6 = 56, PG_GEMM_V_TAIL = 70, PG_GEMM_V_MID = 71 };
enum PgGemmKernel { PG_GK_NONE = -1, PG_GK_PP6 = 0, PG_GK_PP = 1, PG_GK_MID = 2, PG_GK_TAIL = 3, PG_GK_ONE_TILE = 4 };

#define PG_HIP(call)                                                                          \
    do {                                                                                      \
        hipError_t e__ = (call);                                                              \
        if (e__ != hipSuccess) {                                                              \
            pg_set_error("%s failed: %s (%s:%d)", #call, hipGetErrorString(e__), __FILE__, __LINE__); \
            return PG_EHIP;                                                                   \
        }                                                                                     \
    } while (0)

struct PgFpBuf { const void* data; size_t bytes; uint64_t seed; };
int pg_fingerprint_many(const PgFpBuf* bufs, int n, uint64_t* out, hipStream_t stream);
void pg_fingerprint_host(const void* data, size_t bytes, uint64_t seed, uint64_t out[2]);

#define PG_NORM_LUT_SIZE (3 * 256)
void pg_norm_lut_fill(float* lut);
int pg_norm_lut_device(const float** lut);

int pg_gemm_launch(int dtype, const void* A, int64_t lda, const void* W, int64_t ldw, const float* bias, void* out, int64_t ldc,
                   int M, int N, int K, int epi, float qscale, int qcols, const float* aux, int variant,
                   hipStream_t s, const PgGemmExtra* extra = nullptr);
int pg_layernorm_launch(const float* x, const float* gamma, const float* beta, void* y, int out_dtype,
                        int64_t rows, float eps, hipStream_t s);
int pg_preln_launch(float* x, const float* cls, const float* pos0, const float* gamma, const float* beta,
                    int64_t rows, float eps, hipStream_t s, void* x16 = nullptr, int x16_dtype = 0, float* rowstat = nullptr);
int pg_im2col_launch(const void* pixels, int pix_dtype, void* out, int out_dtype, int n_images, hipStream_t s, const float* norm_lut = nullptr);
int pg_token_mean_launch(const float* x, float* out, int n_images, hipStream_t s);
int pg_cast_f32_launch(const float* x, void* y, int out_dtype, int64_t n, hipStream_t s);
int pg_rowstat_cast_launch(const float* x, void* x16, int out_dtype, float* rowstat, int64_t rows, float eps, hipStream_t s);
int pg_rowstat_finalize_launch(const float* statpart, int slots, float* rowstat, int64_t rows, float eps, hipStream_t s,
                               unsigned long long* alarm = nullptr, float alarm_sumsq = 0.f);
int pg_count_sat16_launch(const void* buf, int64_t rows, int cols, int64_t ld, int dtype, unsigned long long* counter, hipStream_t s);
int pg_attention_launch(int dtype, const void* qkv, void* out, int n_images, hipStream_t s);
int pg_x3_ln_launch(const float* x, const float* gamma, const float* beta, void* y3, int64_t rows, float eps, hipStream_t s);
int pg_x3_split_launch(const float* x, void* y3, int64_t rows, int C, int gelu, hipStream_t s);
int pg_x3_im2col_launch(const void* pixels, int pix_dtype, void* out3, int n_images, hipStream_t s, const float* norm_lut = nullptr);
int pg_attention_f32_launch(const float* qkv, float* out, int n_images, hipStream_t s);
bool pg_attention_x3out_available();
int pg_attention_x3out_launch(const float* qkv, void* out3, int n_images, hipStream_t s);
int pg_sum_parts_launch(const float* parts, int S, int64_t part_elems, float* dst, int64_t n, int resid, hipStream_t s);
```

pigeon_amd/csrc/rowops.hip:

```cpp
#include "common.h"
#include "pigeon_internal.h"

template <int OUT>
__global__ __launch_bounds__(256) void layernorm_kernel(const float* __restrict__ x, const float* __restrict__ gamma,
                                                        const float* __restrict__ beta, void* __restrict__ y,
                                                        int64_t rows, float eps) {
    const int lane = threadIdx.x & 63;
    const int64_t row = (int64_t)blockIdx.x * 4 + (threadIdx.x >> 6);
    if (row >= rows) return;
    const float* xr = x + row * VIT_HIDDEN;
    f32x4 v[4];
#pragma unroll
    for (int i = 0; i < 4; ++i) v[i] = *(const f32x4*)(xr + i * 256 + lane * 4);
    float s = 0.f;
#pragma unroll
    for (int i = 0; i < 4; ++i) s += (v[i][0] + v[i][1]) + (v[i][2] + v[i][3]);
    const float mean = wave_sum(s) * (1.0f / VIT_HIDDEN);
    float q = 0.f;
#pragma unroll
    for (int i = 0; i < 4; ++i)
#pragma unroll
        for (int e = 0; e < 4; ++e) { const float d = v[i][e] - mean; q += d * d; }
    const float var = wave_sum(q) * (1.0f / VIT_HIDDEN);
    const float rstd = 1.0f / sqrtf(var + eps);
#pragma unroll
    for (int i = 0; i < 4; ++i) {
        const int c = i * 256 + lane * 4;
        const f32x4 g4 = *(const f32x4*)(gamma + c);
        const f32x4 b4 = *(const f32x4*)(beta + c);
        f32x4 o;
#pragma unroll
        for (int e = 0; e < 4; ++e) o[e] = (v[i][e] - mean) * rstd * g4[e] + b4[e];
        if (OUT != 0) {
            u32x2 pk;
            if (OUT == 1) { pk[0] = pack16x2<T_BF16>(o[0], o[1]); pk[1] = pack16x2<T_BF16>(o[2], o[3]); }
            else { pk[0] = pack16x2<T_F16>(o[0], o[1]); pk[1] = pack16x2<T_F16>(o[2], o[3]); }
            *(u32x2*)((uint16_t*)y + row * VIT_HIDDEN + c) = pk;
        } else {
            *(f32x4*)((float*)y + row * VIT_HIDDEN + c) = o;
        }
    }
}

int pg_layernorm_launch(const float* x, const float* gamma, const float* beta, void* y, int out_dtype,
                        int64_t rows, float eps, hipStream_t s) {
    if (rows <= 0) return PG_OK;
    dim3 grid((unsigned)((rows + 3) / 4)), block(256);
    if (out_dtype == PG_DTYPE_BF16) hipLaunchKernelGGL(layernorm_kernel<1>, grid, block, 0, s, x, gamma, beta, y, rows, eps);
    else if (out_dtype == PG_DTYPE_F16) hipLaunchKernelGGL(layernorm_kernel<2>, grid, block, 0, s, x, gamma, beta, y, rows, eps);
    else if (out_dtype == PG_DTYPE_F32) hipLaunchKernelGGL(layernorm_kernel<0>, grid, block, 0, s, x, gamma, beta, y, rows, eps);
    else { pg_set_error("layernorm: bad output dtype %d", out_dtype); return PG_EINVAL; }
    return pg_check_launch("layernorm");
}

// ... 62 lines not shown
    dim3 grid((unsigned)((rows + 3) / 4)), block(256);
    if (!x16) hipLaunchKernelGGL((preln_kernel<T_F16, false>), grid, block, 0, s, x, cls, pos0, gamma, beta, rows, eps, nullptr, nullptr);
    else if (!rowstat) { pg_set_error("pre_layernorm: x16 without rowstat"); return PG_EINVAL; }
    else if (x16_dtype == PG_DTYPE_F16) hipLaunchKernelGGL((preln_kernel<T_F16, true>), grid, block, 0, s, x, cls, pos0, gamma, beta, rows, eps, (uint16_t*)x16, rowstat);
    else if (x16_dtype == PG_DTYPE_BF16) hipLaunchKernelGGL((preln_kernel<T_BF16, true>), grid, block, 0, s, x, cls, pos0, gamma, beta, rows, eps, (uint16_t*)x16, rowstat);
    else { pg_set_error("pre_layernorm: bad 16-bit dtype %d", x16_dtype); return PG_EINVAL; }
    return pg_check_launch("pre_layernorm");
}

template <typename T>
__global__ __launch_bounds__(256) void rowstat_cast_kernel(const float* __restrict__ x, uint16_t* __restrict__ x16,
                                                           float* __restrict__ rowstat, int64_t rows, float eps) {
    const int lane = threadIdx.x & 63;
    const int64_t row = (int64_t)blockIdx.x * 4 + (threadIdx.x >> 6);
    if (row >= rows) return;
    const float* xr = x + row * VIT_HIDDEN;
    f32x4 v[4];
#pragma unroll
    for (int i = 0; i < 4; ++i) v[i] = *(const f32x4*)(xr + i * 256 + lane * 4);
    float s = 0.f;
#pragma unroll
    for (int i = 0; i < 4; ++i) s += (v[i][0] + v[i][1]) + (v[i][2] + v[i][3]);
    const float mean = wave_sum(s) * (1.0f / VIT_HIDDEN);
    float q = 0.f;
#pragma unroll
    for (int i = 0; i < 4; ++i)
#pragma unroll
        for (int e = 0; e < 4; ++e) { const float d = v[i][e] - mean; q += d * d; }
    const float rstd = 1.0f / sqrtf(wave_sum(q) * (1.0f / VIT_HIDDEN) + eps);
#pragma unroll
    for (int i = 0; i < 4; ++i) {
        u32x2 pk;
        pk[0] = pack16x2<T>(v[i][0], v[i][1]); pk[1] = pack16x2<T>(v[i][2], v[i][3]);
        *(u32x2*)(x16 + row * VIT_HIDDEN + i * 256 + lane * 4) = pk;
    }
    if (lane == 0) { rowstat[2 * row] = rstd; rowstat[2 * row + 1] = mean * rstd; }
}

int pg_rowstat_cast_launch(const float* x, void* x16, int out_dtype, float* rowstat, int64_t rows, float eps, hipStream_t s) {
    if (rows <= 0) return PG_OK;
    dim3 grid((unsigned)((rows + 3) / 4)), block(256);
    if (out_dtype == PG_DTYPE_F16) hipLaunchKernelGGL(rowstat_cast_kernel<T_F16>, grid, block, 0, s, x, (uint16_t*)x16, rowstat, rows, eps);
    else if (out_dtype == PG_DTYPE_BF16) hipLaunchKernelGGL(rowstat_cast_kernel<T_BF16>, grid, block, 0, s, x, (uint16_t*)x16, rowstat, rows, eps);
    else { pg_set_error("rowstat_cast: bad dtype %d", out_dtype); return PG_EINVAL; }
    return pg_check_launch("rowstat_cast");
}

__global__ __launch_bounds__(256) void rowstat_finalize_kernel(const float* __restrict__ part, int slots, float* __restrict__ rowstat,
                                                               int64_t rows, float eps, unsigned long long* __restrict__ alarm,
                                                               float alarm_sumsq) {
    const int64_t row = (int64_t)blockIdx.x * 256 + threadIdx.x;
    if (row >= rows) return;
    float s1 = 0.f, s2 = 0.f;
    for (int i = 0; i < slots; ++i) {
        const f32x2 v = *(const f32x2*)(part + ((int64_t)i * rows + row) * 2);
        s1 += v[0]; s2 += v[1];
    }
    const float mean = s1 * (1.0f / VIT_HIDDEN);
    const float var = fmaxf(s2 * (1.0f / VIT_HIDDEN) - mean * mean, 0.f);
    const float rstd = 1.0f / sqrtf(var + eps);
    rowstat[2 * row] = rstd;
    rowstat[2 * row + 1] = mean * rstd;
    if (alarm && !(s2 < alarm_sumsq)) atomicAdd(alarm, 1ull);
}

int pg_rowstat_finalize_launch(const float* statpart, int slots, float* rowstat, int64_t rows, float eps, hipStream_t s,
                               unsigned long long* alarm, float alarm_sumsq) {
    if (rows <= 0) return PG_OK;
    hipLaunchKernelGGL(rowstat_finalize_kernel, dim3((unsigned)((rows + 255) / 256)), dim3(256), 0, s, statpart, slots, rowstat, rows, eps,
                       alarm, alarm_sumsq);
    return pg_check_launch("rowstat_finalize");
}

template <typename PIX, typename T, bool PIX_F16 = false>
__global__ __launch_bounds__(256) void im2col_kernel(const PIX* __restrict__ pix, uint16_t* __restrict__ out) {
    const int img = blockIdx.x / 24, py = blockIdx.x % 24;
    const PIX* src = pix + (int64_t)img * 3 * VIT_IMG * VIT_IMG;
    uint16_t* dst = out + ((int64_t)img * VIT_PATCHES + py * 24) * VIT_PATCH_KPAD;
    for (int idx = threadIdx.x; idx < 42 * VIT_IMG; idx += 256) {
        const int line = idx / VIT_IMG, xcol = idx - line * VIT_IMG;
        const int c = line / 14, ky = line - c * 14;
        const int px = xcol / 14, kx = xcol - px * 14;
        float v;
        if (sizeof(PIX) == 4) v = (float)src[((int64_t)c * VIT_IMG + py * 14 + ky) * VIT_IMG + xcol];
        else if (PIX_F16) v = f16_bits_to_f32((uint16_t)src[((int64_t)c * VIT_IMG + py * 14 + ky) * VIT_IMG + xcol]);
        else v = bf16_bits_to_f32((uint16_t)src[((int64_t)c * VIT_IMG + py * 14 + ky) * VIT_IMG + xcol]);
        dst[px * VIT_PATCH_KPAD + c * 196 + ky * 14 + kx] = T::bits(v);
    }
    for (int idx = threadIdx.x; idx < 24 * (VIT_PATCH_KPAD - VIT_PATCH_K); idx += 256) {
        const int px = idx / (VIT_PATCH_KPAD - VIT_PATCH_K), k = idx % (VIT_PATCH_KPAD - VIT_PATCH_K);
        dst[px * VIT_PATCH_KPAD + VIT_PATCH_K + k] = 0;
    }
}

template <typename T>
__global__ __launch_bounds__(256) void im2col_u8_kernel(const uint8_t* __restrict__ pix, uint16_t* __restrict__ out,
                                                        const float* __restrict__ lut) {
    __shared__ float slut[PG_NORM_LUT_SIZE];
    for (int i = threadIdx.x; i < PG_NORM_LUT_SIZE; i += 256) slut[i] = lut[i];
    __syncthreads();
    const int img = blockIdx.x / 24, py = blockIdx.x % 24;
    const uint8_t* src = pix + (int64_t)img * 3 * VIT_IMG * VIT_IMG;
    uint16_t* dst = out + ((int64_t)img * VIT_PATCHES + py * 24) * VIT_PATCH_KPAD;
    constexpr int WORDS = VIT_IMG / 4;
    static_assert(VIT_IMG % 4 == 0, "a pixel line is a whole number of 4-byte words");
    for (int idx = threadIdx.x; idx < 42 * WORDS; idx += 256) {
        const int line = idx / WORDS, w = idx - line * WORDS;
        const int c = line / 14, ky = line - c * 14;
        const uint32_t word = *(const uint32_t*)(src + ((int64_t)c * VIT_IMG + py * 14 + ky) * VIT_IMG + w * 4);
#pragma unroll
        for (int b = 0; b < 4; b += 2) {
            const int xcol = w * 4 + b;
            const int px = xcol / 14, kx = xcol - px * 14;
            const uint32_t lo = T::bits(slut[c * 256 + ((word >> (8 * b)) & 0xffu)]);
            const uint32_t hi = T::bits(slut[c * 256 + ((word >> (8 * b + 8)) & 0xffu)]);
            *(uint32_t*)(dst + px * VIT_PATCH_KPAD + c * 196 + ky * 14 + kx) = lo | (hi << 16);
// ... 113 lines not shown
```

pigeon_amd/csrc/vit.hip:

```cpp
#include "vit_handle.h"

static const float kQScale = 0.125f * 1.4426950408889634f;
static size_t ws_bytes_for(int chunk, bool ln_fold) { return fast_ws((size_t)chunk * VIT_TOKENS, ln_fold).total; }
static size_t part_ws_bytes(const pg_vit* h, int n_images, int* parts) {
    *parts = (h->streams > 1 && n_images >= 32 * h->streams) ? h->streams : 1;
    const int per = (n_images + *parts - 1) / *parts;
    const int chunk = per < h->cfg.max_chunk ? per : h->cfg.max_chunk;
    return align_up(ws_bytes_for(chunk > 0 ? chunk : 1, h->ln_fold), 256);
}
extern "C" int pg_vit_workspace_bytes(const pg_vit* h, int n_images, size_t* bytes) {
    if (!h || !bytes || n_images < 0) { pg_set_error("vit_workspace_bytes: bad argument"); return PG_EINVAL; }
    int parts = 1;
    const size_t per_part = part_ws_bytes(h, n_images, &parts);
    *bytes = (size_t)parts * per_part;
    return PG_OK;
}
#define SAT(buf, rows, cols, ld) do { if (h->sat_check) RC(pg_count_sat16_launch((buf), (rows), (cols), (ld), dt, h->sat_counter, s)); } while (0)

static int vit_forward_body(pg_vit* h, int n, char* ws, hipStream_t s) {
    const int64_t M = (int64_t)n * VIT_TOKENS;
    const FastWs w = fast_ws((size_t)M, h->ln_fold);
    float* X = (float*)(ws + w.X);
    uint16_t *Xn = (uint16_t*)(ws + w.Xn), *big = (uint16_t*)(ws + w.big);
    const float eps = h->cfg.ln_eps;
    const int dt = h->cfg.mma_dtype, D = VIT_HIDDEN, F = VIT_MLP;
    auto gemm = [&](const void* A, const uint16_t* W, const float* bias, void* out, int N, int K, int epi, const PgGemmExtra* ex = nullptr) -> int {
        const bool qkv = epi == EPI_QKV || epi == EPI_QKV_LN;
        return pg_gemm_launch(dt, A, K, W, K, bias, out, N, (int)M, N, K, epi, qkv ? kQScale : 1.f, qkv ? D : 0, nullptr, 0, s, ex);
    };
    SAT(big, (int64_t)n * VIT_PATCHES, VIT_PATCH_KPAD, VIT_PATCH_KPAD);
    { ProfScope p(h, s, PROF_GEMM_PATCH);
      RC(pg_gemm_launch(dt, big, VIT_PATCH_KPAD, h->wpatch, VIT_PATCH_KPAD, nullptr, X, VIT_HIDDEN, n * VIT_PATCHES, VIT_HIDDEN, VIT_PATCH_KPAD,
                        EPI_PATCH, 1.f, 0, h->pos, 0, s)); }
    if (!h->ln_fold) { ProfScope p(h, s, PROF_LAYERNORM); RC(pg_preln_launch(X, h->cls, h->pos, h->preg, h->preb, M, eps, s)); }
    if (h->ln_fold) {
        uint16_t* Xn2 = (uint16_t*)(ws + w.Xn2);
        float *statpart = (float*)(ws + w.statpart), *rsA = (float*)(ws + w.rsA), *rsB = (float*)(ws + w.rsB);
        const int slots = VIT_HIDDEN / 64;
        { ProfScope p(h, s, PROF_LAYERNORM); RC(pg_preln_launch(X, h->cls, h->pos, h->preg, h->preb, M, eps, s, Xn, dt, rsA)); }
        SAT(Xn, M, VIT_HIDDEN, VIT_HIDDEN);
        for (int l = 0; l < h->cfg.layers; ++l) {
            const LayerW& L = h->layers[l];
            const bool last = l + 1 == h->cfg.layers;
            PgGemmExtra ex;
            { ProfScope p(h, s, PROF_GEMM_QKV); ex = PgGemmExtra(); ex.colsum = L.sqkv; ex.rowstat = rsA;
              RC(gemm(Xn, L.wqkv, L.bqkv, big, 3 * D, D, EPI_QKV_LN, &ex)); }
            SAT(big, M, 3 * VIT_HIDDEN, 3 * VIT_HIDDEN);
            { ProfScope p(h, s, PROF_ATTENTION); RC(pg_attention_launch(dt, big, Xn, n, s)); }
            SAT(Xn, M, VIT_HIDDEN, VIT_HIDDEN);
            { ProfScope p(h, s, PROF_GEMM_OUT); ex = PgGemmExtra(); ex.x16 = Xn2; ex.ldx = VIT_HIDDEN; ex.statpart = statpart;
              RC(gemm(Xn, L.wo, L.bo, X, D, D, EPI_RESID_STAT, &ex)); }
            SAT(Xn2, M, VIT_HIDDEN, VIT_HIDDEN);
            { ProfScope p(h, s, PROF_LAYERNORM); RC(pg_rowstat_finalize_launch(statpart, slots, rsB, M, eps, s, h->range_alarm, h->range_alarm_sumsq)); }
            { ProfScope p(h, s, PROF_GEMM_FC1); ex = PgGemmExtra(); ex.colsum = L.s1; ex.rowstat = rsB;
              RC(gemm(Xn2, L.w1, L.b1, big, F, D, EPI_GELU_LN, &ex)); }
            SAT(big, M, VIT_MLP, VIT_MLP);
            { ProfScope p(h, s, PROF_GEMM_FC2);
              if (last) RC(gemm(big, L.w2, L.b2, X, D, F, EPI_RESID));
              else { ex = PgGemmExtra(); ex.x16 = Xn; ex.ldx = VIT_HIDDEN; ex.statpart = statpart;
                     RC(gemm(big, L.w2, L.b2, X, D, F, EPI_RESID_STAT, &ex)); } }
            if (!last) SAT(Xn, M, VIT_HIDDEN, VIT_HIDDEN);
            if (!last) { ProfScope p(h, s, PROF_LAYERNORM); RC(pg_rowstat_finalize_launch(statpart, slots, rsA, M, eps, s, h->range_alarm, h->range_alarm_sumsq)); }
        }
    } else
    for (int l = 0; l < h->cfg.layers; ++l) {
        const LayerW& L = h->layers[l];
        { ProfScope p(h, s, PROF_LAYERNORM); RC(pg_layernorm_launch(X, L.ln1g, L.ln1b, Xn, dt, M, eps, s)); }
        SAT(Xn, M, VIT_HIDDEN, VIT_HIDDEN);
        { ProfScope p(h, s, PROF_GEMM_QKV); RC(gemm(Xn, L.wqkv, L.bqkv, big, 3 * D, D, EPI_QKV)); }
        SAT(big, M, 3 * VIT_HIDDEN, 3 * VIT_HIDDEN);
        { ProfScope p(h, s, PROF_ATTENTION); RC(pg_attention_launch(dt, big, Xn, n, s)); }
        SAT(Xn, M, VIT_HIDDEN, VIT_HIDDEN);
        { ProfScope p(h, s, PROF_GEMM_OUT); RC(gemm(Xn, L.wo, L.bo, X, D, D, EPI_RESID)); }
        { ProfScope p(h, s, PROF_LAYERNORM); RC(pg_layernorm_launch(X, L.ln2g, L.ln2b, Xn, dt, M, eps, s)); }
        SAT(Xn, M, VIT_HIDDEN, VIT_HIDDEN);
        { ProfScope p(h, s, PROF_GEMM_FC1); RC(gemm(Xn, L.w1, L.b1, big, F, D, EPI_GELU)); }
        SAT(big, M, VIT_MLP, VIT_MLP);
        { ProfScope p(h, s, PROF_GEMM_FC2); RC(gemm(big, L.w2, L.b2, X, D, F, EPI_RESID)); }
    }
    return PG_OK;
}

void vit_graph_entry_free(pg_vit::GraphEntry& e) {
    if (e.done) { (void)hipEventSynchronize(e.done); (void)hipEventDestroy(e.done); }
    if (e.exec) (void)hipGraphExecDestroy(e.exec);
    if (e.graph) (void)hipGraphDestroy(e.graph);
    e.exec = nullptr; e.graph = nullptr; e.done = nullptr;
}
static int graph_replay(pg_vit* h, pg_vit::GraphEntry* ent, hipStream_t s) {
    PG_HIP(hipGraphLaunch(ent->exec, s));
    if (ent->done) (void)hipEventRecord(ent->done, s);
    ++h->graph_replays;
    return PG_OK;
}
static int vit_forward_body_graphed(pg_vit* h, int n, char* ws, hipStream_t s) {
    const bool ok = h->use_graph && !h->prof && !h->sat_check && h->streams == 1;
    if (!ok) return vit_forward_body(h, n, ws, s);
    pg_vit::GraphEntry* ent = nullptr;
    for (auto& e : h->graphs) if (e.ws == ws && e.n == n) { ent = &e; break; }
    if (!ent) {
        if (h->graphs.size() >= 8) {
            size_t lru = 0;
            for (size_t i = 1; i < h->graphs.size(); ++i) if (h->graphs[i].last_use < h->graphs[lru].last_use) lru = i;
            vit_graph_entry_free(h->graphs[lru]);
            h->graphs.erase(h->graphs.begin() + lru);
        }
        h->graphs.push_back({ws, n, 0, nullptr, nullptr, 0, pg_tune_epoch(), nullptr});
        ent = &h->graphs.back();
    }
    ent->last_use = ++h->graph_clock;
    if (ent->exec && ent->epoch != pg_tune_epoch()) {
        vit_graph_entry_free(*ent);
        ent->seen = 1;
    }
    if (ent->exec) return graph_replay(h, ent, s);
// ... 144 lines not shown
```

pigeon_amd/hip_ops.py:

```python
from __future__ import annotations

import ctypes as C
from typing import Dict, Optional

import torch

from . import _lib
from ._lib import Bank, VitCfg, check, load

TOKENS, HIDDEN, MLP, PATCHES, KPAD = 577, 1024, 4096, 576, 640


def _p(t: Optional[torch.Tensor]):
    return C.c_void_p(0) if t is None else C.c_void_p(t.data_ptr())


def _stream():
    return C.c_void_p(torch.cuda.current_stream().cuda_stream)


_T16 = {torch.float16: _lib.PG_DTYPE_F16, torch.bfloat16: _lib.PG_DTYPE_BF16}
_PIXDT = {torch.float32: _lib.PG_DTYPE_F32, torch.float16: _lib.PG_DTYPE_F16, torch.bfloat16: _lib.PG_DTYPE_BF16}
_PIXIN = {**_PIXDT, torch.uint8: _lib.PG_DTYPE_U8}
_PREP_OUT = {torch.float32: _lib.PG_DTYPE_F32, torch.float16: _lib.PG_DTYPE_F16, torch.uint8: _lib.PG_DTYPE_U8}
# ... 46 lines not shown
        out.copy_(dst)
    return out


def tune_gemm_tail_rows(rows: int) -> None:
    check(load().pg_tune_gemm_tail_rows(int(rows)), "pg_tune_gemm_tail_rows")


def tune_gemm_tail_shape(min_k: int, min_n: int) -> None:
    check(load().pg_tune_gemm_tail_shape(int(min_k), int(min_n)), "pg_tune_gemm_tail_shape")


def rowstat_cast(x: torch.Tensor, out_dtype: torch.dtype = torch.float16, eps: float = 1e-5):
    _dev(x, torch.float32)
    rows = x.numel() // HIDDEN
    x16 = torch.empty(x.shape, dtype=out_dtype, device=x.device)
    rs = torch.empty((rows, 2), dtype=torch.float32, device=x.device)
    check(load().pg_op_rowstat_cast(_p(x), _p(x16), _dt16(x16), _p(rs), rows, float(eps), _stream()), "pg_op_rowstat_cast")
    return x16, rs


def gemm16_resid_stat(A: torch.Tensor, W: torch.Tensor, bias: torch.Tensor, X: torch.Tensor, variant: int = 0):
    M, K = A.shape
    N = W.shape[0]
    x16 = torch.empty((M, N), dtype=A.dtype, device=A.device)
    part = torch.empty((N // 64, M, 2), dtype=torch.float32, device=A.device)
    have = X.untyped_storage().nbytes() - X.storage_offset() * X.element_size()
    Xr = X
    if have < (M + 384) * X.stride(0) * X.element_size():
        Xr = torch.zeros((M + 384, N), dtype=X.dtype, device=X.device)[:M]
        Xr.copy_(X)
    check(load().pg_op_gemm16_resid_stat(_dt16(A), _p(A), A.stride(0), _p(W), W.stride(0), _p(bias), _p(Xr), Xr.stride(0), _p(x16),
                                         x16.stride(0), _p(part), M, N, K, variant, _stream()), "pg_op_gemm16_resid_stat")
    if Xr is not X:
        X.copy_(Xr)
    return x16, part


def rowstat_finalize(part: torch.Tensor, eps: float = 1e-5) -> torch.Tensor:
    slots, rows = part.shape[0], part.shape[1]
    rs = torch.empty((rows, 2), dtype=torch.float32, device=part.device)
    check(load().pg_op_rowstat_finalize(_p(part), slots, _p(rs), rows, float(eps), _stream()), "pg_op_rowstat_finalize")
    return rs


def gemm16_ln(A: torch.Tensor, W: torch.Tensor, bias: torch.Tensor, colsum: torch.Tensor, rowstat: torch.Tensor, epi: int,
              qscale: float = 1.0, qcols: int = 0, variant: int = 0) -> torch.Tensor:
    M, K = A.shape
    N = W.shape[0]
    out = torch.empty((M, N), dtype=A.dtype, device=A.device)
    check(load().pg_op_gemm16_ln(_dt16(A), _p(A), A.stride(0), _p(W), W.stride(0), _p(bias), _p(colsum), _p(rowstat), _p(out),
                                 out.stride(0), M, N, K, epi, float(qscale), int(qcols), variant, _stream()), "pg_op_gemm16_ln")
    return out


def layernorm(x: torch.Tensor, gamma: torch.Tensor, beta: torch.Tensor, eps: float = 1e-5,
              out_dtype: torch.dtype = torch.float16, out: Optional[torch.Tensor] = None) -> torch.Tensor:
    _dev(x, torch.float32)
    rows = x.numel() // HIDDEN
    if out is None:
        out = torch.empty(x.shape, dtype=out_dtype, device=x.device)
    pg = _lib.PG_DTYPE_F32 if out.dtype == torch.float32 else _dt16(out)
    check(load().pg_op_layernorm(_p(x), _p(gamma), _p(beta), _p(out), pg, rows, float(eps), _stream()), "pg_op_layernorm")
    return out


def attention(qkv: torch.Tensor, n_images: int) -> torch.Tensor:
    _dev(qkv)
    out = torch.empty((n_images * TOKENS, HIDDEN), dtype=qkv.dtype, device=qkv.device)
    check(load().pg_op_attention(_dt16(qkv), _p(qkv), _p(out), n_images, _stream()), "pg_op_attention")
    return out


def im2col(pixels: torch.Tensor, out_dtype: torch.dtype = torch.float16) -> torch.Tensor:
    _dev(pixels)
    _shape(pixels, "pixels", None, 3, 336, 336)
    n = pixels.shape[0]
    dt = _PIXIN[pixels.dtype]
    out = torch.empty((n * PATCHES, KPAD), dtype=out_dtype, device=pixels.device)
    check(load().pg_op_im2col(_p(pixels), dt, _p(out), _dt16(out), n, _stream()), "pg_op_im2col")
    return out


def token_mean(x: torch.Tensor) -> torch.Tensor:
    _dev(x, torch.float32)
    n = x.shape[0]
    out = torch.empty((n, HIDDEN), dtype=torch.float32, device=x.device)
    check(load().pg_op_token_mean(_p(x), _p(out), n, _stream()), "pg_op_token_mean")
    return out


def cast_f32(x: torch.Tensor, out_dtype: torch.dtype = torch.float16) -> torch.Tensor:
    _dev(x, torch.float32)
    y = torch.empty(x.shape, dtype=out_dtype, device=x.device)
    check(load().pg_op_cast_f32(_p(x), _p(y), _dt16(y), x.numel(), _stream()), "pg_op_cast_f32")
    return y


def proto_build(train_emb: torch.Tensor, member_off: torch.Tensor, member_idx: torch.Tensor) -> torch.Tensor:
    _dev(train_emb, torch.float32); _dev(member_off, torch.int64); _dev(member_idx, torch.int64)
    if train_emb.dim() not in (2, 3) or train_emb.shape[-1] != HIDDEN:
        raise _lib.PigeonHipError(f"proto_build: embeddings must be (Ntr,{HIDDEN}) or (Ntr,panels,{HIDDEN}), got {tuple(train_emb.shape)}")
    panels = 1 if train_emb.dim() == 2 else int(train_emb.shape[1])
    if member_off.dim() != 1 or member_off.numel() < 1 or member_idx.dim() != 1:
        raise _lib.PigeonHipError("proto_build: member_off (P+1,) and member_idx (n,) expected")
    P = member_off.numel() - 1
# ... 833 lines not shown
```

Measured before the change: 2519.

## Fold rowstat finalize into LN-epilogue GEMMs reading partial sums directly

The LN-folded GEMMs (QKV and FC1) can now read the per-slot row-stat partials, sum them, and compute rstd and mean*rstd inside the kernel. This removes the separate rowstat finalize launch that used to run twice per layer. The range alarm moves into the first column tile. A planner enables the fold only when the GEMM grid fits within one wave of CUs, where the extra partial loads are likely hidden, and it adds an LDS exchange plus a barrier in the pp/pp6 kernels.

Result: no change. 2519, median of 3 (+0.0%).

```diff
diff --git a/include/pigeon_hip.h b/include/pigeon_hip.h
--- a/include/pigeon_hip.h
+++ b/include/pigeon_hip.h
@@ -75,6 +75,8 @@
 int pg_tune_exact_attention(int use_f32_mfma);
 int pg_tune_exact_products(int n);
 int pg_tune_exact_fusion(int on);
+int pg_tune_rowstat_fold(int mode);
+int pg_rowstat_fold_plan(int rows, int* qkv, int* fc1);
 int pg_vit_saturation_check(pg_vit* h, int on);
 int pg_vit_saturation_read(pg_vit* h, int64_t* count, int reset);
 int pg_vit_range_alarm_read(pg_vit* h, int64_t* rows, int reset);
@@ -218,6 +220,12 @@
 int pg_op_gemm16_ln(int dtype, const void* A, int64_t lda, const void* W, int64_t ldw, const float* bias, const float* colsum,
                     const float* rowstat, void* out, int64_t ldc, int M, int N, int K, int epi, float qscale, int qcols,
                     int variant, void* stream);
+int pg_op_gemm16_ln_part(int dtype, const void* A, int64_t lda, const void* W, int64_t ldw, const float* bias, const float* colsum,
+                         const float* rowstat, const float* statpart_in, int slots, int64_t stat_rows, float eps,
+                         unsigned long long* alarm, float alarm_sumsq, void* out, int64_t ldc, int M, int N, int K, int epi,
+                         float qscale, int qcols, int variant, void* stream);
+int pg_op_rowstat_finalize_alarm(const float* statpart, int slots, float* rowstat, int64_t rows, float eps, unsigned long long* alarm,
+                                 float alarm_sumsq, void* stream);
 int pg_op_layernorm(const float* x, const float* gamma, const float* beta, void* y, int out_dtype,
                     int64_t rows, float eps, void* stream);
 int pg_op_attention(int dtype, const void* qkv, void* out, int n_images, void* stream);
diff --git a/pigeon_amd/_lib.py b/pigeon_amd/_lib.py
--- a/pigeon_amd/_lib.py
+++ b/pigeon_amd/_lib.py
@@ -75,6 +75,8 @@
     "pg_tune_exact_attention": (_I, [_I]),
     "pg_tune_exact_products": (_I, [_I]),
     "pg_tune_exact_fusion": (_I, [_I]),
+    "pg_tune_rowstat_fold": (_I, [_I]),
+    "pg_rowstat_fold_plan": (_I, [_I, _P, _P]),
     "pg_gemm_plan": (_I, [_I, _I, _I, _I, _I, _P, _P, _P]),
     "pg_vit_saturation_check": (_I, [_P, _I]),
     "pg_vit_saturation_read": (_I, [_P, C.POINTER(_I64), _I]),
@@ -128,6 +130,8 @@
     "pg_op_gemm16_resid_stat": (_I, [_I, _P, _I64, _P, _I64, _P, _P, _I64, _P, _I64, _P, _I, _I, _I, _I, _P]),
     "pg_op_rowstat_finalize": (_I, [_P, _I, _P, _I64, _F, _P]),
     "pg_op_gemm16_ln": (_I, [_I, _P, _I64, _P, _I64, _P, _P, _P, _P, _I64, _I, _I, _I, _I, _F, _I, _I, _P]),
+    "pg_op_gemm16_ln_part": (_I, [_I, _P, _I64, _P, _I64, _P, _P, _P, _P, _I, _I64, _F, _P, _F, _P, _I64, _I, _I, _I, _I, _F, _I, _I, _P]),
+    "pg_op_rowstat_finalize_alarm": (_I, [_P, _I, _P, _I64, _F, _P, _F, _P]),
     "pg_op_layernorm": (_I, [_P, _P, _P, _P, _I, _I64, _F, _P]),
     "pg_op_attention": (_I, [_I, _P, _P, _I, _P]),
     "pg_op_im2col": (_I, [_P, _I, _P, _I, _I, _P]),
diff --git a/pigeon_amd/csrc/abi.hip b/pigeon_amd/csrc/abi.hip
--- a/pigeon_amd/csrc/abi.hip
+++ b/pigeon_amd/csrc/abi.hip
@@ -59,6 +59,22 @@
     if (!A || !W || !out || !colsum || !rowstat) { pg_set_error("op_gemm16_ln: null argument"); return PG_EINVAL; }
     if (epi != EPI_QKV_LN && epi != EPI_GELU_LN) { pg_set_error("op_gemm16_ln: epi must be 6 or 7"); return PG_EINVAL; }
     PgGemmExtra ex; ex.colsum = colsum; ex.rowstat = rowstat;
+    return pg_gemm_launch(dtype, A, lda, W, ldw, bias, out, ldc, M, N, K, epi, qscale, qcols, nullptr, variant ? variant : PG_GEMM_V_PP,
+                          (hipStream_t)stream, &ex);
+}
+extern "C" int pg_op_rowstat_finalize_alarm(const float* statpart, int slots, float* rowstat, int64_t rows, float eps,
+                                            unsigned long long* alarm, float alarm_sumsq, void* stream) {
+    if (!statpart || !rowstat || slots <= 0) { pg_set_error("op_rowstat_finalize_alarm: bad argument"); return PG_EINVAL; }
+    return pg_rowstat_finalize_launch(statpart, slots, rowstat, rows, eps, (hipStream_t)stream, alarm, alarm_sumsq);
+}
+extern "C" int pg_op_gemm16_ln_part(int dtype, const void* A, int64_t lda, const void* W, int64_t ldw, const float* bias,
+                                    const float* colsum, const float* rowstat, const float* statpart_in, int slots, int64_t stat_rows,
+                                    float eps, unsigned long long* alarm, float alarm_sumsq, void* out, int64_t ldc, int M, int N, int K,
+                                    int epi, float qscale, int qcols, int variant, void* stream) {
+    if (!A || !W || !out) { pg_set_error("op_gemm16_ln_part: null argument"); return PG_EINVAL; }
+    if (epi != EPI_QKV_LN && epi != EPI_GELU_LN) { pg_set_error("op_gemm16_ln_part: epi must be 6 or 7"); return PG_EINVAL; }
+    PgGemmExtra ex; ex.colsum = colsum; ex.rowstat = rowstat; ex.statpart_in = statpart_in; ex.stat_slots = slots; ex.stat_rows = stat_rows;
+    ex.ln_eps = eps; ex.alarm = alarm; ex.alarm_sumsq = alarm_sumsq;
     return pg_gemm_launch(dtype, A, lda, W, ldw, bias, out, ldc, M, N, K, epi, qscale, qcols, nullptr, variant ? variant : PG_GEMM_V_PP,
                           (hipStream_t)stream, &ex);
 }
diff --git a/pigeon_amd/csrc/gemm_epi.h b/pigeon_amd/csrc/gemm_epi.h
--- a/pigeon_amd/csrc/gemm_epi.h
+++ b/pigeon_amd/csrc/gemm_epi.h
@@ -1,5 +1,6 @@
 #pragma once
 #include "gemm_device.h"
+#include "rowstat.h"
 
 __device__ __forceinline__ float quick_gelu(float v) {
     const float e = __builtin_amdgcn_exp2f(-2.4554669595930157f * v);
@@ -106,9 +107,21 @@
 }
 
 constexpr int EPI_SLAB_ROWPF = 64 + 4;
+struct RowPair { float rstd, mrs; };
+__device__ __forceinline__ RowPair tile_rowpair(const GemmArgs& g, int row, bool valid_lane, bool alarm_tile) {
+    RowstatPartials pp;
+    const int rc = row < g.M ? row : g.M - 1;
+    pp.issue(g.ex.statpart_in, g.ex.stat_slots, g.ex.stat_rows, rc);
+    float s1, s2;
+    pp.sum(g.ex.stat_slots, s1, s2);
+    RowPair o;
+    rowstat_pair(s1, s2, g.ex.ln_eps, o.rstd, o.mrs);
+    if (alarm_tile && valid_lane && row < g.M) rowstat_alarm(g.ex.alarm, g.ex.alarm_sumsq, s2);
+    return o;
+}
 template <typename T, int EPI>
 __device__ __forceinline__ void epi_slab32(const GemmArgs& g, float* slab, int lane, int row0, int col0, const f32x4 (&acc0)[4],
-                                           const f32x4 (&acc1)[4]) {
+                                           const f32x4 (&acc1)[4], RowPair own = RowPair{0.f, 0.f}, int own_lane0 = 0) {
     constexpr bool OUT16 = epi_is_out16(EPI);
     constexpr bool LN = epi_is_ln(EPI);
     constexpr bool STAT = (EPI == EPI_RESID_STAT);
@@ -119,6 +132,11 @@
     for (int ib = 0; ib < 2; ++ib)
 #pragma unroll
         for (int j = 0; j < 4; ++j) *(f32x4*)(slab + (ib * 16 + l15) * ROWPF + j * 16 + 4 * lq) = (ib ? acc1 : acc0)[j];
+    if constexpr (LN) {
+        if (g.ex.statpart_in && (unsigned)(lane - own_lane0) < 32u) {
+            slab[(lane - own_lane0) * ROWPF + 64] = own.rstd; slab[(lane - own_lane0) * ROWPF + 65] = own.mrs;
+        }
+    }
     wave_lds_fence();
 
     constexpr int HOFF = STAT ? 32 : 4;
@@ -140,7 +158,7 @@
         if constexpr (OUT16) {
             float rstd = 0.f, mrs = 0.f;
             if constexpr (LN) {
-                const u32x2 rs = *(const u32x2*)(g.ex.rowstat + (int64_t)row * 2);
+                const u32x2 rs = g.ex.statpart_in ? *(const u32x2*)(slab + r * ROWPF + 64) : *(const u32x2*)(g.ex.rowstat + (int64_t)row * 2);
                 asm("v_mov_b32 %0, %1" : "=v"(rstd) : "v"(rs[0]));
                 asm("v_mov_b32 %0, %1" : "=v"(mrs) : "v"(rs[1]));
             }
diff --git a/pigeon_amd/csrc/gemm_mid.hip b/pigeon_amd/csrc/gemm_mid.hip
--- a/pigeon_amd/csrc/gemm_mid.hip
+++ b/pigeon_amd/csrc/gemm_mid.hip
@@ -93,6 +93,10 @@
     const int sw = (lane >> 1) & 7;
     const uint32_t lds0 = (uint32_t)(uintptr_t)(__attribute__((address_space(3))) char*)smem;
     const uint32_t a_base = lds0 + (wm * 64 + l15) * ROWB, b_base = lds0 + MD_W_OFF + (wn * 64 + l15) * ROWB;
+    RowPair own = {0.f, 0.f};
+    if constexpr (epi_is_ln(EPI)) {
+        if (g.ex.statpart_in) own = tile_rowpair(g, m0 + wm * 64 + lane, true, n0 + wn * 64 == 0);
+    }
     f32x4 acc[4][4];
 #pragma unroll
     for (int i = 0; i < 4; ++i)
@@ -143,9 +147,9 @@
     }
     float* slab = (float*)(smem + wave * MD_SLAB_BYTES);
     const int row0 = m0 + wm * 64, col0 = n0 + wn * 64;
-    epi_slab32<T, EPI>(g, slab, lane, row0, col0, acc[0], acc[1]);
+    epi_slab32<T, EPI>(g, slab, lane, row0, col0, acc[0], acc[1], own, 0);
     wave_lds_fence();
-    epi_slab32<T, EPI>(g, slab, lane, row0 + 32, col0, acc[2], acc[3]);
+    epi_slab32<T, EPI>(g, slab, lane, row0 + 32, col0, acc[2], acc[3], own, 32);
     wave_lds_fence();
 }
 
@@ -186,6 +190,7 @@
         if (g.ex.rowstat) g.ex.rowstat += (int64_t)m_begin * 2;
         if (g.ex.x16) g.ex.x16 = (uint16_t*)g.ex.x16 + (int64_t)m_begin * g.ldc;
         if (g.ex.statpart) g.ex.statpart += (int64_t)m_begin * 2;
+        if (g.ex.statpart_in) g.ex.statpart_in += (int64_t)m_begin * 2;
         g.M -= m_begin;
     }
     if (int rc = pg_gemm_panel_check("gemm_mid", g.lda, g.ldw, MD_BM, MD_BN)) return rc;
diff --git a/pigeon_amd/csrc/gemm_plan.hip b/pigeon_amd/csrc/gemm_plan.hip
--- a/pigeon_amd/csrc/gemm_plan.hip
+++ b/pigeon_amd/csrc/gemm_plan.hip
@@ -97,6 +97,16 @@
 static bool route_pp256() { return mid_on() && g_gemm_mid != 2; }
 extern "C" int pg_tune_gemm_mid(int on) {
     g_gemm_mid = on == 2 ? 2 : (on ? 1 : 0); ++g_tune_epoch;
+    return PG_OK;
+}
+
+static int g_rowstat_fold = -1;
+static int rowstat_fold_mode() {
+    if (g_rowstat_fold < 0) { const char* e = env_knob<const char*>("PIGEON_ROWSTAT_FOLD", "1"); g_rowstat_fold = e[0] == '0' ? 0 : (e[0] == '2' ? 2 : 1); }
+    return g_rowstat_fold;
+}
+extern "C" int pg_tune_rowstat_fold(int on) {
+    g_rowstat_fold = on == 2 ? 2 : (on ? 1 : 0); ++g_tune_epoch;
     return PG_OK;
 }
 
@@ -296,6 +306,24 @@
     return PG_OK;
 }
 
+bool pg_rowstat_fold_pays(int epi, int M, int N, int K) {
+    const int mode = rowstat_fold_mode();
+    if (mode != 1) return mode == 2;
+    GemmPlan p;
+    if (gemm_plan(0, epi, M, N, K, p) != PG_OK) return false;
+    if (p.kernel == PG_GK_MID || p.kernel == PG_GK_TAIL) return true;
+    if (p.kernel != PG_GK_PP6 && p.kernel != PG_GK_PP) return false;
+    const int bm = p.kernel == PG_GK_PP6 ? 384 : 256;
+    return (int64_t)((p.rows + bm - 1) / bm) * (N / 256) <= pg_gemm_grid_cus();
+}
+
+extern "C" int pg_rowstat_fold_plan(int rows, int* qkv, int* fc1) {
+    if (!qkv || !fc1 || rows <= 0) { pg_set_error("rowstat_fold_plan: bad argument"); return PG_EINVAL; }
+    *qkv = pg_rowstat_fold_pays(EPI_QKV_LN, rows, 3 * VIT_HIDDEN, VIT_HIDDEN) ? 1 : 0;
+    *fc1 = pg_rowstat_fold_pays(EPI_GELU_LN, rows, VIT_MLP, VIT_HIDDEN) ? 1 : 0;
+    return PG_OK;
+}
+
 extern "C" int pg_gemm_plan(int variant, int epi, int M, int N, int K, int* kernel, int* rows_main, int* rest) {
     if (!kernel || !rows_main || !rest || M <= 0 || N <= 0 || K <= 0) { pg_set_error("gemm_plan: bad argument"); return PG_EINVAL; }
     GemmPlan p;
@@ -335,7 +363,16 @@
     }
     if ((epi == EPI_GELU || epi == EPI_RESID || epi >= EPI_RESID_STAT) && !bias) { pg_set_error("gemm: epilogue %d needs a bias", epi); return PG_EINVAL; }
     if (epi == EPI_RESID_STAT && (!g.ex.x16 || !g.ex.statpart || g.ex.ldx != ldc)) { pg_set_error("gemm: EPI_RESID_STAT needs x16 / statpart and ldx == ldc"); return PG_EINVAL; }
-    if (epi_is_ln(epi) && (!g.ex.colsum || !g.ex.rowstat)) { pg_set_error("gemm: LN epilogue needs colsum / rowstat"); return PG_EINVAL; }
+    if (epi_is_ln(epi)) {
+        if (!g.ex.colsum) { pg_set_error("gemm: LN epilogue needs colsum"); return PG_EINVAL; }
+        if (!g.ex.rowstat && !g.ex.statpart_in) { pg_set_error("gemm: LN epilogue needs rowstat or statpart_in"); return PG_EINVAL; }
+        if (g.ex.rowstat && g.ex.statpart_in) { pg_set_error("gemm: LN epilogue takes rowstat or statpart_in, not both"); return PG_EINVAL; }
+        if (g.ex.statpart_in && (g.ex.stat_slots < 1 || g.ex.stat_slots > ROWSTAT_MAX_SLOTS)) {
+            pg_set_error("gemm: statpart_in needs its slot count, 1 .. %d (stat_slots = %d)", ROWSTAT_MAX_SLOTS, g.ex.stat_slots);
+            return PG_EINVAL;
+        }
+        if (g.ex.statpart_in && g.ex.stat_rows > 0 && g.ex.stat_rows < M) { pg_set_error("gemm: statpart_in has fewer rows per slot than the problem (stat_rows = %lld, M = %d)", (long long)g.ex.stat_rows, M); return PG_EINVAL; }
+    } else if (g.ex.statpart_in) { pg_set_error("gemm: statpart_in goes with the LN epilogues only (epi = %d)", epi); return PG_EINVAL; }
     if (epi == EPI_PATCH && !aux) { pg_set_error("gemm: patch epilogue needs aux"); return PG_EINVAL; }
     if (epi == EPI_GELU_X3 && (ldc != 3 * (int64_t)N || dtype != PG_DTYPE_F16 || N % 256 != 0 || K % 128 != 0)) {
         pg_set_error("gemm: EPI_GELU_X3 writes the fp16 triple [M][3N]: ldc == 3 N, fp16 operands, N %% 256 == 0, K %% 128 == 0 (ldc=%lld N=%d K=%d)",
diff --git a/pigeon_amd/csrc/gemm_pp.hip b/pigeon_amd/csrc/gemm_pp.hip
--- a/pigeon_amd/csrc/gemm_pp.hip
+++ b/pigeon_amd/csrc/gemm_pp.hip
@@ -11,6 +11,8 @@
 constexpr int PP_SLAB_ROWF = 64 + 4;
 constexpr int PP_SLAB_BYTES = 32 * PP_SLAB_ROWF * 4;
 constexpr int PP_LDS = 160 * 1024;
+constexpr int PP_EXCH_OFF = PP_SLAB_OFF + 8 * PP_SLAB_BYTES;
+static_assert(PP_EXCH_OFF + PP_BM * 8 <= PP_LDS, "the row-pair exchange must fit behind the slabs");
 
 struct TileCtx {
     __amdgpu_buffer_rsrc_t ra, rw;
@@ -331,8 +333,9 @@
     }
 }
 
-template <typename T, int EPI>
+template <typename T, int EPI, bool FOLD = false>
 __global__ __launch_bounds__(512) void gemm_pp_kernel(GemmArgs g) {
+    static_assert(!FOLD || epi_is_ln(EPI), "only the LN epilogues take the partials");
     extern __shared__ __attribute__((aligned(16))) char smem[];
     const int tid = threadIdx.x;
     const int lane = tid & 63;
@@ -393,7 +396,9 @@
         raw_barrier();
         PG_TS(g, dbg_iter, wave, 0);
         u32x2 rs[4][4];
-        if constexpr (epi_is_ln(EPI)) load_rowstat<EPI>(rs, g, c.m0 + wm * 128, err);
+        RowstatPartials sp;
+        if constexpr (FOLD) sp.issue(g.ex.statpart_in, g.ex.stat_slots, g.ex.stat_rows, min(c.m0 + (tid & (PP_BM - 1)), g.M - 1));
+        else if constexpr (epi_is_ln(EPI)) load_rowstat<EPI>(rs, g, c.m0 + wm * 128, err);
         constexpr int XEARLY = EPI == EPI_RESID ? 1 : (EPI == EPI_RESID_STAT ? 2 : 0);
         XCtx xc;
         u32x4 xq[4][8];
@@ -423,6 +428,22 @@
 
         asm volatile("s_nop 7\n\ts_nop 7" ::: "memory");
         PG_TS(g, dbg_iter, wave, 2);
+        if constexpr (FOLD) {
+            float s1, s2;
+            sp.sum(g.ex.stat_slots, s1, s2);
+            RowPair own;
+            rowstat_pair(s1, s2, g.ex.ln_eps, own.rstd, own.mrs);
+            if (tid < PP_BM) {
+                *(f32x2*)(smem + PP_EXCH_OFF + tid * 8) = f32x2{own.rstd, own.mrs};
+                if (c.n0 == 0 && c.m0 + tid < g.M) rowstat_alarm(g.ex.alarm, g.ex.alarm_sumsq, s2);
+            }
+            wait_lgkm0();
+            raw_barrier();
+#pragma unroll
+            for (int i = 0; i < 4; ++i)
+#pragma unroll
+                for (int it = 0; it < 4; ++it) rs[i][it] = *(const u32x2*)(smem + PP_EXCH_OFF + (wm * 128 + i * 32 + it * 8 + err) * 8);
+        }
         const int row0 = c.m0 + wm * 128, col0 = c.n0 + wn * 64;
         const int part_now = c.part;
         L += nblk;
@@ -450,10 +471,10 @@
     }
 }
 
-template <typename T, int EPI>
+template <typename T, int EPI, bool FOLD = false>
 int launch_pp(const GemmArgs& g, int nblk, hipStream_t s) {
     static bool attr_set = false;
-    return launch_kernel(gemm_pp_kernel<T, EPI>, attr_set, PP_LDS, dim3(nblk), dim3(512), g, s, "gemm_pp", "gemm_pp: set LDS attr");
+    return launch_kernel(gemm_pp_kernel<T, EPI, FOLD>, attr_set, PP_LDS, dim3(nblk), dim3(512), g, s, "gemm_pp", "gemm_pp: set LDS attr");
 }
 
 template <typename T>
@@ -465,8 +486,8 @@
         case EPI_PATCH: return launch_pp<T, EPI_PATCH>(g, nblk, s);
         case EPI_F32: return launch_pp<T, EPI_F32>(g, nblk, s);
         case EPI_RESID_STAT: return launch_pp<T, EPI_RESID_STAT>(g, nblk, s);
-        case EPI_QKV_LN: return launch_pp<T, EPI_QKV_LN>(g, nblk, s);
-        case EPI_GELU_LN: return launch_pp<T, EPI_GELU_LN>(g, nblk, s);
+        case EPI_QKV_LN: return g.ex.statpart_in ? launch_pp<T, EPI_QKV_LN, true>(g, nblk, s) : launch_pp<T, EPI_QKV_LN>(g, nblk, s);
+        case EPI_GELU_LN: return g.ex.statpart_in ? launch_pp<T, EPI_GELU_LN, true>(g, nblk, s) : launch_pp<T, EPI_GELU_LN>(g, nblk, s);
         case EPI_GELU_X3:
             if constexpr (std::is_same<T, T_F16>::value) return launch_pp<T, EPI_GELU_X3>(g, nblk, s);
             else { pg_set_error("gemm_pp: EPI_GELU_X3 exists for fp16 operands only (the exact mode)"); return PG_EINVAL; }
diff --git a/pigeon_amd/csrc/gemm_pp6.hip b/pigeon_amd/csrc/gemm_pp6.hip
--- a/pigeon_amd/csrc/gemm_pp6.hip
+++ b/pigeon_amd/csrc/gemm_pp6.hip
@@ -11,7 +11,8 @@
 constexpr int P6_SLAB_BYTES = 32 * P6_SLAB_ROWF * 4;
 constexpr int P6_LDS = 2 * P6_STAGE;
 constexpr int P6_NDMA = P6_TM + 4;
-static_assert(8 * P6_SLAB_BYTES <= P6_STAGE, "slabs must fit into stage 1");
+constexpr int P6_EXCH_OFF = P6_SLAB_OFF + 8 * P6_SLAB_BYTES;
+static_assert(P6_EXCH_OFF + P6_BM * 8 <= P6_LDS, "slabs and the row-pair exchange must fit into stage 1");
 
 struct Tile6 {
     __amdgpu_buffer_rsrc_t ra, rw;
@@ -182,11 +183,16 @@
     rs.v[0] = __builtin_amdgcn_raw_buffer_load_b64(rrs, (slab * 32 + l15) * 8, 0, 0);
     rs.v[1] = __builtin_amdgcn_raw_buffer_load_b64(rrs, (slab * 32 + 16 + l15) * 8, 0, 0);
 }
-template <typename T, int EPI, typename PREFETCH_DMA, typename PREFETCH_BIAS>
+__device__ __forceinline__ void read_rowpair_p(RowStatP& rs, const char* xrows, int l15, int slab) {
+    rs.v[0] = *(const u32x2*)(xrows + (slab * 32 + l15) * 8);
+    rs.v[1] = *(const u32x2*)(xrows + (slab * 32 + 16 + l15) * 8);
+}
+template <typename T, int EPI, bool FOLD, typename PREFETCH_DMA, typename PREFETCH_BIAS, typename PREFETCH_STAT>
 __device__ __forceinline__ void epilogue6_park16(Acc6& acc, const GemmArgs& g, char* smem, int wave, int lane, int row0, int col0,
                                                  const Bias6& b01, const Bias6& b23, const Bias6& s01, const Bias6& s23,
-                                                 const RowStatP& rs0, __amdgpu_buffer_rsrc_t rrs,
-                                                 PREFETCH_DMA&& prefetch_dma, PREFETCH_BIAS&& prefetch_bias, int dbg_iter = 0) {
+                                                 const RowStatP& rs0, __amdgpu_buffer_rsrc_t rrs, const char* xrows,
+                                                 PREFETCH_DMA&& prefetch_dma, PREFETCH_BIAS&& prefetch_bias,
+                                                 PREFETCH_STAT&& prefetch_stat, int dbg_iter = 0) {
     constexpr bool LN = epi_is_ln(EPI);
     const int l15 = lane & 15, lq = lane >> 4;
     char* slab = smem + P6_SLAB_OFF + wave * P6_SLAB_BYTES;
@@ -206,7 +212,12 @@
     char* wr = slab + l15 * P6_P16_ROWB + 8 * lq;
 #pragma unroll
     for (int i = 0; i < P6_TM; ++i) {
-        if constexpr (LN) { if (i + 1 < P6_TM) load_rowstat_p(rs[(i + 1) & 1], rrs, l15, i + 1); }
+        if constexpr (LN) {
+            if (i + 1 < P6_TM) {
+                if constexpr (FOLD) read_rowpair_p(rs[(i + 1) & 1], xrows, l15, i + 1);
+                else load_rowstat_p(rs[(i + 1) & 1], rrs, l15, i + 1);
+            }
+        }
 #pragma unroll
         for (int ib = 0; ib < 2; ++ib) {
             float rstd = 0.f, mrs = 0.f;
@@ -227,6 +238,7 @@
             }
         }
         wave_lds_fence();
+        if constexpr (FOLD) { if (i == 0) prefetch_stat(0); if (i == 1) prefetch_stat(1); }
 #pragma unroll
         for (int it = 0; it < 4; ++it) {
             const u32x4 v = *(const u32x4*)(slab + (it * 8 + rr) * P6_P16_ROWB + c8 * 16);
@@ -318,8 +330,9 @@
     }
 }
 
-template <typename T, int EPI>
+template <typename T, int EPI, bool FOLD = false>
 __global__ __launch_bounds__(512) void gemm_pp6_kernel(GemmArgs g) {
+    static_assert(!FOLD || epi_is_ln(EPI), "only the LN epilogues take the partials");
     extern __shared__ __attribute__((aligned(16))) char smem[];
     const int tid = threadIdx.x;
     const int lane = tid & 63;
@@ -348,10 +361,15 @@
     Tile6 c = make_tile6(g, L);
     issue_dma6<0, P6_NDMA>(c, smem, wave, voffA, voffW, 0);
     Bias6 bias;
-    load_bias6<BHOFF>(bias, g, c.n0 + wn * 64 + ecc);
-    pin_bias6(bias);
+    if constexpr (!FOLD) {
+        load_bias6<BHOFF>(bias, g, c.n0 + wn * 64 + ecc);
+        pin_bias6(bias);
+    }
     constexpr int NST = (P6_TM - 1) * 4;
     bool first = true;
+    const int xrow = tid < P6_BM ? tid : P6_BM - 1;
+    RowPair own = {0.f, 0.f};
+    if constexpr (FOLD) own = tile_rowpair(g, c.m0 + xrow, tid < P6_BM, c.n0 == 0);
     int dbg_iter = 0;
 
     while (true) {
@@ -378,14 +396,15 @@
         Bias6 b23, cs23;
         RowStatP rsp;
         __amdgpu_buffer_rsrc_t rrs = c.ra;
+        if constexpr (FOLD) load_bias6<BHOFF>(bias, g, col0 + ecc);
         if constexpr (!RSTAT) load_bias6<16>(b23, g, col0 + 32 + ecc);
         if constexpr (epi_is_ln(EPI)) {
             cs.lo = *(const f32x4*)(g.ex.colsum + col0 + ecc);
             cs.hi = *(const f32x4*)(g.ex.colsum + col0 + ecc + BHOFF);
-            rrs = rowstat_rsrc6(g, row0);
+            if constexpr (!FOLD) rrs = rowstat_rsrc6(g, row0);
             cs23.lo = *(const f32x4*)(g.ex.colsum + col0 + 32 + ecc);
             cs23.hi = *(const f32x4*)(g.ex.colsum + col0 + 48 + ecc);
-            load_rowstat_p(rsp, rrs, l15, 0);
+            if constexpr (!FOLD) load_rowstat_p(rsp, rrs, l15, 0);
         }
         ResidCtx6 rc;
         XRows6 x0;
@@ -396,6 +415,13 @@
         if (!follower) raw_barrier();
         asm volatile("s_nop 7\n\ts_nop 7" ::: "memory");
         PG_TS(g, dbg_iter, wave, 2);
+        const char* xrows = smem + P6_EXCH_OFF + wm * (P6_TM * 32) * 8;
+        if constexpr (FOLD) {
+            if (tid < P6_BM) *(f32x2*)(smem + P6_EXCH_OFF + tid * 8) = f32x2{own.rstd, own.mrs};
+            wait_lgkm0();
+            raw_barrier();
+            read_rowpair_p(rsp, xrows, l15, 0);
+        }
 
         L += nblk;
         const bool more = L < g.ntiles;
@@ -404,22 +430,39 @@
             c = make_tile6(g, more ? L : L - nblk);
             issue_dma6<0, P6_NDMA>(c, smem, wave, voffA, voffW, 0);
         };
-        auto prefetch_bias = [&]() { load_bias6<BHOFF>(bias_next, g, c.n0 + wn * 64 + ecc); };
+        auto prefetch_bias = [&]() { if constexpr (!FOLD) load_bias6<BHOFF>(bias_next, g, c.n0 + wn * 64 + ecc); };
+        RowstatPartials sp;
+        auto prefetch_stat = [&](int half) {
+            if constexpr (FOLD) {
+                const int r = min(c.m0 + xrow, g.M - 1);
+                if (half == 0) sp.template issue<0, 8>(g.ex.statpart_in, g.ex.stat_slots, g.ex.stat_rows, r);
+                else sp.template issue<8, 8>(g.ex.statpart_in, g.ex.stat_slots, g.ex.stat_rows, r);
+            }
+        };
         if constexpr (RSTAT) epilogue6_resid<T>(acc, g, smem, wave, lane, row0, col0, bias, x0, rc, prefetch_dma, prefetch_bias, dbg_iter);
-        else epilogue6_park16<T, EPI>(acc, g, smem, wave, lane, row0, col0, bias, b23, cs, cs23, rsp, rrs, prefetch_dma, prefetch_bias, dbg_iter);
+        else epilogue6_park16<T, EPI, FOLD>(acc, g, smem, wave, lane, row0, col0, bias, b23, cs, cs23, rsp, rrs, xrows, prefetch_dma,
+                                            prefetch_bias, prefetch_stat, dbg_iter);
+        if constexpr (FOLD) {
+            float s1, s2;
+            sp.sum(g.ex.stat_slots, s1, s2);
+            rowstat_pair(s1, s2, g.ex.ln_eps, own.rstd, own.mrs);
+            if (more && c.n0 == 0 && tid < P6_BM && c.m0 + xrow < g.M) rowstat_alarm(g.ex.alarm, g.ex.alarm_sumsq, s2);
+        }
         PG_TS(g, dbg_iter, wave, 9);
         ++dbg_iter;
         if (!more) break;
-        pin_bias6(bias_next);
-        bias = bias_next;
+        if constexpr (!FOLD) {
+            pin_bias6(bias_next);
+            bias = bias_next;
+        }
         first = false;
     }
 }
 
-template <typename T, int EPI>
+template <typename T, int EPI, bool FOLD = false>
 int launch_pp6(const GemmArgs& g, int nblk, hipStream_t s) {
     static bool attr_set = false;
-    return launch_kernel(gemm_pp6_kernel<T, EPI>, attr_set, P6_LDS, dim3(nblk), dim3(512), g, s, "gemm_pp6", "gemm_pp6: set LDS attr");
+    return launch_kernel(gemm_pp6_kernel<T, EPI, FOLD>, attr_set, P6_LDS, dim3(nblk), dim3(512), g, s, "gemm_pp6", "gemm_pp6: set LDS attr");
 }
 
 }
@@ -443,15 +486,16 @@
     }
     const int cap = pg_gemm_grid_cus();
     const int nblk = g.ntiles < cap ? g.ntiles : cap;
-    if (epi_is_ln(epi) && (!g.ex.colsum || !g.ex.rowstat)) { pg_set_error("gemm_pp6: LN epilogue needs colsum / rowstat"); return PG_EINVAL; }
+    if (epi_is_ln(epi) && (!g.ex.colsum || (!g.ex.rowstat && !g.ex.statpart_in))) { pg_set_error("gemm_pp6: LN epilogue needs colsum and rowstat or statpart_in"); return PG_EINVAL; }
+    const bool fold = epi_is_ln(epi) && g.ex.statpart_in != nullptr;
     if (epi == EPI_RESID_STAT && (!g.ex.x16 || !g.ex.statpart || g.ex.ldx != g.ldc || !g.bias)) { pg_set_error("gemm_pp6: EPI_RESID_STAT needs bias, x16 / statpart and ldx == ldc"); return PG_EINVAL; }
 #define P6_DISPATCH(TT)                                                          \
     switch (epi) {                                                               \
         case EPI_QKV: return launch_pp6<TT, EPI_QKV>(g, nblk, s);                \
         case EPI_GELU: return launch_pp6<TT, EPI_GELU>(g, nblk, s);              \
-        case EPI_QKV_LN: return launch_pp6<TT, EPI_QKV_LN>(g, nblk, s);          \
+        case EPI_QKV_LN: return fold ? launch_pp6<TT, EPI_QKV_LN, true>(g, nblk, s) : launch_pp6<TT, EPI_QKV_LN>(g, nblk, s);   \
         case EPI_RESID_STAT: return launch_pp6<TT, EPI_RESID_STAT>(g, nblk, s);  \
-        default: return launch_pp6<TT, EPI_GELU_LN>(g, nblk, s);                 \
+        default: return fold ? launch_pp6<TT, EPI_GELU_LN, true>(g, nblk, s) : launch_pp6<TT, EPI_GELU_LN>(g, nblk, s);         \
     }
     if (dtype == PG_DTYPE_F16) { P6_DISPATCH(T_F16) }
     if (dtype == PG_DTYPE_BF16) { P6_DISPATCH(T_BF16) }
diff --git a/pigeon_amd/csrc/gemm_tail.hip b/pigeon_amd/csrc/gemm_tail.hip
--- a/pigeon_amd/csrc/gemm_tail.hip
+++ b/pigeon_amd/csrc/gemm_tail.hip
@@ -38,6 +38,10 @@
 #pragma unroll
     for (int j = 0; j < 4; ++j) vw[j] = (j * 16 + l15) * (int)g.ldw * 2 + lq * 16;
 
+    RowPair own = {0.f, 0.f};
+    if constexpr (epi_is_ln(EPI)) {
+        if (g.ex.statpart_in) own = tile_rowpair(g, row0 + (lane & 31), lane < 32, col0 == 0);
+    }
     const int nks = g.K / 32;
     FragTL<T> fr[TL_DEPTH];
 #pragma unroll
@@ -71,6 +75,9 @@
     for (int ib = 0; ib < 2; ++ib)
 #pragma unroll
         for (int j = 0; j < 4; ++j) *(f32x4*)(slab + (ib * 16 + l15) * EPI_SLAB_ROWPF + j * 16 + 4 * lq) = acc[ib][j];
+    if constexpr (LN) {
+        if (g.ex.statpart_in && lane < 32) { slab[lane * EPI_SLAB_ROWPF + 64] = own.rstd; slab[lane * EPI_SLAB_ROWPF + 65] = own.mrs; }
+    }
     wave_lds_fence();
 
     constexpr int HOFF = STAT ? 32 : 4;
@@ -92,7 +99,7 @@
         if constexpr (OUT16) {
             float rstd = 0.f, mrs = 0.f;
             if constexpr (LN) {
-                const u32x2 rs = *(const u32x2*)(g.ex.rowstat + (int64_t)row * 2);
+                const u32x2 rs = g.ex.statpart_in ? *(const u32x2*)(slab + r * EPI_SLAB_ROWPF + 64) : *(const u32x2*)(g.ex.rowstat + (int64_t)row * 2);
                 asm("v_mov_b32 %0, %1" : "=v"(rstd) : "v"(rs[0]));
                 asm("v_mov_b32 %0, %1" : "=v"(mrs) : "v"(rs[1]));
             }
diff --git a/pigeon_amd/csrc/pigeon_internal.h b/pigeon_amd/csrc/pigeon_internal.h
--- a/pigeon_amd/csrc/pigeon_internal.h
+++ b/pigeon_amd/csrc/pigeon_internal.h
@@ -13,6 +13,11 @@
     int64_t ldx = 0;
     float* statpart = nullptr;
     int64_t stat_rows = 0;
+    const float* statpart_in = nullptr;
+    int stat_slots = 0;
+    float ln_eps = 0.f;
+    unsigned long long* alarm = nullptr;
+    float alarm_sumsq = 0.f;
     int parts = 1;
     int64_t a_part = 0, w_part = 0, c_part = 0;
 };
@@ -23,6 +28,7 @@
 int pg_gemm_grid_cus();
 int pg_gemm_raster_gn();
 unsigned long long pg_tune_epoch();
+bool pg_rowstat_fold_pays(int epi, int M, int N, int K);
 int pg_gemm_precise_route(int M, int N, int Ktot, bool resid, const int* cand, int ncand);
 
 enum { PG_GEMM_V_ONE_TILE = 8, PG_GEMM_V_PP = 36, PG_GEMM_V_PP6 = 56, PG_GEMM_V_TAIL = 70, PG_GEMM_V_MID = 71 };
diff --git a/pigeon_amd/csrc/rowops.hip b/pigeon_amd/csrc/rowops.hip
--- a/pigeon_amd/csrc/rowops.hip
+++ b/pigeon_amd/csrc/rowops.hip
@@ -1,5 +1,6 @@
 #include "common.h"
 #include "pigeon_internal.h"
+#include "rowstat.h"
 
 template <int OUT>
 __global__ __launch_bounds__(256) void layernorm_kernel(const float* __restrict__ x, const float* __restrict__ gamma,
@@ -168,16 +169,12 @@
     const int64_t row = (int64_t)blockIdx.x * 256 + threadIdx.x;
     if (row >= rows) return;
     float s1 = 0.f, s2 = 0.f;
-    for (int i = 0; i < slots; ++i) {
-        const f32x2 v = *(const f32x2*)(part + ((int64_t)i * rows + row) * 2);
-        s1 += v[0]; s2 += v[1];
-    }
-    const float mean = s1 * (1.0f / VIT_HIDDEN);
-    const float var = fmaxf(s2 * (1.0f / VIT_HIDDEN) - mean * mean, 0.f);
-    const float rstd = 1.0f / sqrtf(var + eps);
+    for (int i = 0; i < slots; ++i) rowstat_add(s1, s2, *(const f32x2*)(part + ((int64_t)i * rows + row) * 2));
+    float rstd, mrs;
+    rowstat_pair(s1, s2, eps, rstd, mrs);
     rowstat[2 * row] = rstd;
-    rowstat[2 * row + 1] = mean * rstd;
-    if (alarm && !(s2 < alarm_sumsq)) atomicAdd(alarm, 1ull);
+    rowstat[2 * row + 1] = mrs;
+    rowstat_alarm(alarm, alarm_sumsq, s2);
 }
 
 int pg_rowstat_finalize_launch(const float* statpart, int slots, float* rowstat, int64_t rows, float eps, hipStream_t s,
diff --git a/pigeon_amd/csrc/rowstat.h b/pigeon_amd/csrc/rowstat.h
--- /dev/null
+++ b/pigeon_amd/csrc/rowstat.h
@@ -0,0 +1,38 @@
+#pragma once
+#include "common.h"
+
+constexpr int ROWSTAT_MAX_SLOTS = 16;
+
+__device__ __forceinline__ void rowstat_pair(float s1, float s2, float eps, float& rstd, float& mrs) {
+#pragma clang fp contract(off)
+    constexpr float inv_n = 1.0f / VIT_HIDDEN;
+    const float mean = s1 * inv_n;
+    const float mm = mean * mean;
+    const float var = fmaxf(__builtin_fmaf(s2, inv_n, -mm), 0.f);
+    rstd = 1.0f / sqrtf(var + eps);
+    mrs = mean * rstd;
+}
+
+__device__ __forceinline__ void rowstat_add(float& s1, float& s2, f32x2 v) { s1 += v[0]; s2 += v[1]; }
+
+struct RowstatPartials {
+    f32x2 v[ROWSTAT_MAX_SLOTS];
+    template <int FROM = 0, int CNT = ROWSTAT_MAX_SLOTS>
+    __device__ __forceinline__ void issue(const float* part, int slots, int64_t stat_rows, int64_t row) {
+#pragma unroll
+        for (int i = FROM; i < FROM + CNT; ++i) {
+            const int slot = i < slots ? i : slots - 1;
+            v[i] = *(const f32x2*)(part + ((int64_t)slot * stat_rows + row) * 2);
+        }
+    }
+    __device__ __forceinline__ void sum(int slots, float& s1, float& s2) const {
+        s1 = 0.f; s2 = 0.f;
+#pragma unroll
+        for (int i = 0; i < ROWSTAT_MAX_SLOTS; ++i)
+            if (i < slots) rowstat_add(s1, s2, v[i]);
+    }
+};
+
+__device__ __forceinline__ void rowstat_alarm(unsigned long long* alarm, float alarm_sumsq, float s2) {
+    if (alarm && !(s2 < alarm_sumsq)) atomicAdd(alarm, 1ull);
+}
diff --git a/pigeon_amd/csrc/vit.hip b/pigeon_amd/csrc/vit.hip
--- a/pigeon_amd/csrc/vit.hip
+++ b/pigeon_amd/csrc/vit.hip
@@ -35,15 +35,22 @@
     if (!h->ln_fold) { ProfScope p(h, s, PROF_LAYERNORM); RC(pg_preln_launch(X, h->cls, h->pos, h->preg, h->preb, M, eps, s)); }
     if (h->ln_fold) {
         uint16_t* Xn2 = (uint16_t*)(ws + w.Xn2);
-        float *statpart = (float*)(ws + w.statpart), *rsA = (float*)(ws + w.rsA), *rsB = (float*)(ws + w.rsB);
+        float *statpart = (float*)(ws + w.statpart), *rsA = (float*)(ws + w.rsA);
         const int slots = VIT_HIDDEN / 64;
+        const bool fold_qkv = pg_rowstat_fold_pays(EPI_QKV_LN, (int)M, 3 * D, D), fold_fc1 = pg_rowstat_fold_pays(EPI_GELU_LN, (int)M, F, D);
+        auto ln_extra = [&](const float* colsum, bool from_partials) {
+            PgGemmExtra e; e.colsum = colsum;
+            if (from_partials) { e.statpart_in = statpart; e.stat_slots = slots; e.ln_eps = eps; e.alarm = h->range_alarm; e.alarm_sumsq = h->range_alarm_sumsq; }
+            else e.rowstat = rsA;
+            return e;
+        };
         { ProfScope p(h, s, PROF_LAYERNORM); RC(pg_preln_launch(X, h->cls, h->pos, h->preg, h->preb, M, eps, s, Xn, dt, rsA)); }
         SAT(Xn, M, VIT_HIDDEN, VIT_HIDDEN);
         for (int l = 0; l < h->cfg.layers; ++l) {
             const LayerW& L = h->layers[l];
             const bool last = l + 1 == h->cfg.layers;
             PgGemmExtra ex;
-            { ProfScope p(h, s, PROF_GEMM_QKV); ex = PgGemmExtra(); ex.colsum = L.sqkv; ex.rowstat = rsA;
+            { ProfScope p(h, s, PROF_GEMM_QKV); ex = ln_extra(L.sqkv, fold_qkv && l > 0);
               RC(gemm(Xn, L.wqkv, L.bqkv, big, 3 * D, D, EPI_QKV_LN, &ex)); }
             SAT(big, M, 3 * VIT_HIDDEN, 3 * VIT_HIDDEN);
             { ProfScope p(h, s, PROF_ATTENTION); RC(pg_attention_launch(dt, big, Xn, n, s)); }
@@ -51,8 +58,8 @@
             { ProfScope p(h, s, PROF_GEMM_OUT); ex = PgGemmExtra(); ex.x16 = Xn2; ex.ldx = VIT_HIDDEN; ex.statpart = statpart;
               RC(gemm(Xn, L.wo, L.bo, X, D, D, EPI_RESID_STAT, &ex)); }
             SAT(Xn2, M, VIT_HIDDEN, VIT_HIDDEN);
-            { ProfScope p(h, s, PROF_LAYERNORM); RC(pg_rowstat_finalize_launch(statpart, slots, rsB, M, eps, s, h->range_alarm, h->range_alarm_sumsq)); }
-            { ProfScope p(h, s, PROF_GEMM_FC1); ex = PgGemmExtra(); ex.colsum = L.s1; ex.rowstat = rsB;
+            if (!fold_fc1) { ProfScope p(h, s, PROF_LAYERNORM); RC(pg_rowstat_finalize_launch(statpart, slots, rsA, M, eps, s, h->range_alarm, h->range_alarm_sumsq)); }
+            { ProfScope p(h, s, PROF_GEMM_FC1); ex = ln_extra(L.s1, fold_fc1);
               RC(gemm(Xn2, L.w1, L.b1, big, F, D, EPI_GELU_LN, &ex)); }
             SAT(big, M, VIT_MLP, VIT_MLP);
             { ProfScope p(h, s, PROF_GEMM_FC2);
@@ -60,7 +67,7 @@
               else { ex = PgGemmExtra(); ex.x16 = Xn; ex.ldx = VIT_HIDDEN; ex.statpart = statpart;
                      RC(gemm(big, L.w2, L.b2, X, D, F, EPI_RESID_STAT, &ex)); } }
             if (!last) SAT(Xn, M, VIT_HIDDEN, VIT_HIDDEN);
-            if (!last) { ProfScope p(h, s, PROF_LAYERNORM); RC(pg_rowstat_finalize_launch(statpart, slots, rsA, M, eps, s, h->range_alarm, h->range_alarm_sumsq)); }
+            if (!last && !fold_qkv) { ProfScope p(h, s, PROF_LAYERNORM); RC(pg_rowstat_finalize_launch(statpart, slots, rsA, M, eps, s, h->range_alarm, h->range_alarm_sumsq)); }
         }
     } else
     for (int l = 0; l < h->cfg.layers; ++l) {
diff --git a/pigeon_amd/hip_ops.py b/pigeon_amd/hip_ops.py
--- a/pigeon_amd/hip_ops.py
+++ b/pigeon_amd/hip_ops.py
@@ -122,6 +122,32 @@
     check(load().pg_op_gemm16_ln(_dt16(A), _p(A), A.stride(0), _p(W), W.stride(0), _p(bias), _p(colsum), _p(rowstat), _p(out),
                                  out.stride(0), M, N, K, epi, float(qscale), int(qcols), variant, _stream()), "pg_op_gemm16_ln")
     return out
+
+
+def rowstat_finalize_alarm(part: torch.Tensor, alarm: torch.Tensor, alarm_sumsq: float, eps: float = 1e-5) -> torch.Tensor:
+    slots, rows = part.shape[0], part.shape[1]
+    rs = torch.empty((rows, 2), dtype=torch.float32, device=part.device)
+    check(load().pg_op_rowstat_finalize_alarm(_p(part), slots, _p(rs), rows, float(eps), _p(alarm), float(alarm_sumsq), _stream()),
+          "pg_op_rowstat_finalize_alarm")
+    return rs
+
+
+def gemm16_ln_part(A: torch.Tensor, W: torch.Tensor, bias: torch.Tensor, colsum: torch.Tensor, part: torch.Tensor, epi: int,
+                   qscale: float = 1.0, qcols: int = 0, variant: int = 0, eps: float = 1e-5, alarm: Optional[torch.Tensor] = None,
+                   alarm_sumsq: float = 0.0) -> torch.Tensor:
+    M, K = A.shape
+    N = W.shape[0]
+    out = torch.empty((M, N), dtype=A.dtype, device=A.device)
+    check(load().pg_op_gemm16_ln_part(_dt16(A), _p(A), A.stride(0), _p(W), W.stride(0), _p(bias), _p(colsum), None, _p(part),
+                                      part.shape[0], part.shape[1], float(eps), None if alarm is None else _p(alarm), float(alarm_sumsq),
+                                      _p(out), out.stride(0), M, N, K, epi, float(qscale), int(qcols), variant, _stream()),
+          "pg_op_gemm16_ln_part")
+    return out
+
+
+def tune_rowstat_fold(on) -> None:
+    mode = 2 if (not isinstance(on, bool) and on == 2) else (1 if on else 0)
+    check(load().pg_tune_rowstat_fold(mode), "pg_tune_rowstat_fold")
 
 
 def layernorm(x: torch.Tensor, gamma: torch.Tensor, beta: torch.Tensor, eps: float = 1e-5,
```
